# choderalab/openmmtools

Hardware: AMD Instinct MI355X
Metric: REMD iterations/s (propagate+u_kl+mix), 24-replica AlanineDipeptideExplicit per GPU (higher is better)
Workload: dtype f32

## Files before the change

### openmmtools_amd/csrc/forces.hip

```cpp
#include "remd_internal.h"
#include "rng.h"
#include <cmath>
#include <algorithm>
#include <set>
#include <cstdlib>
#include <cstdio>

#define EP_EXT      0
#define EP_BOND     1
#define EP_ANGLE    2
#define EP_TORSION  3
#define EP_EXCEPT   4
#define EP_EXCLCORR 5
#define EP_PME      6
#define EP_CONST    7
#define EP_NB0      8

#include "pair_math.h"
#include "listed_terms.h"

#define MAX_EXCL_WORDS 8

struct nb_tables {
    nb_params p{};
    int method = NB_LJ_ONLY;
    bool has_alch = false;
    dev_array<float4> d_param;
    dev_array<unsigned long long> d_mask;
    int n_exc = 0; dev_array<int> d_exc_atoms; dev_array<float> d_exc_params;
    dev_array<int> d_exc_alch; dev_array<int> d_excl_alch;
    double lam_e_override = -1.0;
    double self_nn = 0, self_aa = 0, q_n = 0, q_a = 0;
    dev_array<double> d_probe; int probe_R = 0;
    int n_excl = 0; dev_array<int> d_excl_atoms; dev_array<float> d_excl_qq;
    dev_array<float> d_rep_lam;
    int rep_lam_R = 0;
    std::vector<double> state_lam_a, state_sc;
    dev_array<double> d_state_lam;
    dev_array<double> d_alch_ukl;
    dev_array<int> d_own;
    int alch_R = 0, alch_K = 0;
    double disp_coeff = 0.0;
    double self_energy = 0.0;
    double net_charge_term = 0.0;
    std::vector<double> charge;
    std::vector<char> is_alch;
    int n_groups = 0; dev_array<int> d_grp_first; dev_array<int> d_grp_size;
    dev_array<int> d_order;
    dev_array<float4> d_spos;
    dev_array<float4> d_sposi;
    dev_array<float4> d_lj_sposi;
    dev_array<float4> d_sparam;
    dev_array<unsigned long long> d_smask;
    dev_array<float4> d_tile_c; dev_array<float4> d_tile_h;
    dev_array<float4> d_partial;
    dev_array<float4> d_cl_c; dev_array<float4> d_cl_h;
    int cl_cap = 0; bool clusters = true;
    bool lj_split = false; int NL = 0, NLpad = 0, lj_words = 1, lj_cap = 0;
    dev_array<int> d_lj_ord;
    dev_array<unsigned long long> d_lj_mask;
    dev_array<int> d_lj_order; dev_array<float4> d_lj_spos; dev_array<float4> d_lj_sparam; dev_array<unsigned long long> d_lj_smask;
    dev_array<float4> d_lj_tile_c; dev_array<float4> d_lj_tile_h; dev_array<float4> d_lj_cl_c; dev_array<float4> d_lj_cl_h;
    int sci_split = 12;
    dev_array<unsigned int> d_sci_list; dev_array<int> d_sci_count; dev_array<unsigned long long> d_excl; int excl_W = 0;
    dev_array<long long> d_sforce; dev_array<long long> d_lj_sforce;
    dev_array<unsigned int> d_lj_sci_list; dev_array<int> d_lj_sci_count; dev_array<unsigned long long> d_lj_excl; int lj_excl_W = 0;
    int sort_R = 0; int evals_since_sort = 1 << 30; int resort_interval = 40; bool sorting = true;
    std::vector<float> rep_lam_host;
    dev_array<unsigned int> d_queue;
    struct tune_seg { int cand; hipEvent_t a, b; };
    int nb_prio = 0;
    std::vector<tune_seg> tune_segs; int tune_state = 0 , tune_left = 0, tune_next = 0;
    int nb_grid = 0;
    int sort_hbits = 0;
    dev_array<float4> d_ctab; bool use_table = false;
    dev_array<unsigned int> d_pair_done; unsigned int pair_done_target = 0;
    dev_array<int> d_tile_of_rank;
    dev_array<int> d_sort_scratch;
    ~nb_tables() { for (auto& sg : tune_segs) { if (sg.a) hipEventDestroy(sg.a); if (sg.b) hipEventDestroy(sg.b); } }
};
void remd_table_deleter::operator()(nb_tables* t) const { delete t; }

__global__ void remd_spin_wait_kernel(const unsigned int* flag, unsigned int seq, unsigned int* spin_out)
{
    if (threadIdx.x == 0) {
        long long n = 0;
        while ((int)(__hip_atomic_load(flag, __ATOMIC_RELAXED, __HIP_MEMORY_SCOPE_AGENT) - seq) < 0) {
            if ((n & 255) == 255 && __hip_atomic_load(spin_out, __ATOMIC_RELAXED, __HIP_MEMORY_SCOPE_AGENT) != 0u) break;
            __builtin_amdgcn_s_sleep(4);
            if (++n > (1ll << 25)) { atomicCAS(spin_out, 0u, 1u); break; }
        }
    }
    __builtin_amdgcn_fence(__ATOMIC_ACQUIRE, "agent");
}
void remd_launch_join_wait(remd_ctx* h)
{
    if (h->fold_pending) {
        hipEventRecord(h->ev_join, h->stream2);
        hipStreamWaitEvent(h->stream, h->ev_join, 0);
        h->fold_pending = false;
    }
    if (!h->join_deferred) return;
    hipLaunchKernelGGL(remd_spin_wait_kernel, dim3(1), dim3(64), 0, h->stream, h->d_sync + 1, h->join_deferred, h->d_sync + 2);
    h->join_deferred = 0;
}
__global__ void remd_signal_kernel(unsigned int* flag, unsigned int seq)
{
    if (threadIdx.x == 0) __hip_atomic_store(flag, seq, __ATOMIC_RELEASE, __HIP_MEMORY_SCOPE_AGENT);
}

__device__ __forceinline__ double wave_sum(double e)
{
    for (int off = 32; off > 0; off >>= 1) e += __shfl_xor(e, off);
    return e;
}

__device__ __forceinline__ double block_sum_256(double e, double* s_part)
{
    e = wave_sum(e);
    if ((threadIdx.x & 63) == 0) s_part[threadIdx.x >> 6] = e;
    __syncthreads();
    return s_part[0] + s_part[1] + s_part[2] + s_part[3];
}

template <bool ENERGY>
__global__ __launch_bounds__(64)
void ext_force_kernel(int n_ext, const int* __restrict__ ext_atoms, float K, float x0, double U0,
                      int Npad, const float4* __restrict__ pos, long long* __restrict__ force,
                      double* __restrict__ epart, int n_epart)
{
    const int r = blockIdx.x;
    double e = 0.0;
    for (int t = threadIdx.x; t < n_ext; t += 64) {
        const int i = ext_atoms[t];
        const float4 p = pos[(size_t)r * Npad + i];
        const float dx = p.x - x0;
        add_force(force + (size_t)r * 3 * Npad, Npad, i, -K * dx, -K * p.y, -K * p.z);
        if (ENERGY) e += 0.5 * (double)K * ((double)dx * dx + (double)p.y * p.y + (double)p.z * p.z) + U0;
    }
    if (ENERGY) {
        e = wave_sum(e);
        if (threadIdx.x == 0) epart[(size_t)r * n_epart + EP_EXT] = e;
    }
}

template <bool ENERGY>
__global__ __launch_bounds__(256)
void bond_kernel(int n, const int* __restrict__ atoms, const float* __restrict__ params, int Npad,
                 const float4* __restrict__ pos, long long* __restrict__ force, double* __restrict__ epart, int n_epart)
{
    __shared__ double s_part[4];
    const int r = blockIdx.x;
    const float4* P = pos + (size_t)r * Npad;
    long long* F = force + (size_t)r * 3 * Npad;
    double e = 0.0;
    for (int t = threadIdx.x; t < n; t += 256) {
        const int i = atoms[2 * t], j = atoms[2 * t + 1];
        const float r0 = params[2 * t], k = params[2 * t + 1];
        const float3 d = sub3(ld3(P, j), ld3(P, i));
        const float len = sqrtf(dotf(d, d));
        const float dl = len - r0;
        const float fs = k * dl / len;
        add_force(F, Npad, i, fs * d.x, fs * d.y, fs * d.z);
        add_force(F, Npad, j, -fs * d.x, -fs * d.y, -fs * d.z);
        if (ENERGY) e += 0.5 * (double)k * (double)dl * (double)dl;
    }
    if (ENERGY) { e = block_sum_256(e, s_part); if (threadIdx.x == 0) epart[(size_t)r * n_epart + EP_BOND] = e; }
}

template <bool ENERGY>
__global__ __launch_bounds__(256)
void angle_kernel(int n, const int* __restrict__ atoms, const float* __restrict__ params, int Npad,
                  const float4* __restrict__ pos, long long* __restrict__ force, double* __restrict__ epart, int n_epart)
{
    __shared__ double s_part[4];
    const int r = blockIdx.x;
    const float4* P = pos + (size_t)r * Npad;
    long long* F = force + (size_t)r * 3 * Npad;
    double e = 0.0;
    for (int t = threadIdx.x; t < n; t += 256) {
        const int a = atoms[3 * t], b = atoms[3 * t + 1], c = atoms[3 * t + 2];
        const float th0 = params[2 * t], k = params[2 * t + 1];
// ... 79 lines not shown
    unsigned k = 0u;
    for (int b = bits - 1; b >= 0; --b) {
#pragma unroll
        for (int i = 0; i < 3; ++i) k = (k << 1) | ((X[i] >> b) & 1u);
    }
    return k;
}

template <typename KEY>
__device__ __forceinline__
void sort_groups_body(int G, int N, int Npad, const int* __restrict__ grp_first, const int* __restrict__ grp_size,
                      const float4* __restrict__ pos, const float* __restrict__ box, int* __restrict__ order,
                      KEY* key, int* r_first, int* r_size, int* r_off, int* s_part, int hbits)
{
    const int r = blockIdx.x, tid = threadIdx.x;
    const float Lx = box[4 * r], Ly = box[4 * r + 1], Lz = box[4 * r + 2];
    const int nc = 1 << hbits;
    constexpr int GBITS = sizeof(KEY) == 8 ? 32 : 13;
    for (int g = tid; g < G; g += 1024) {
        const float4 x = pos[(size_t)r * Npad + grp_first[g]];
        float fx = x.x / Lx, fy = x.y / Ly, fz = x.z / Lz;
        fx -= floorf(fx); fy -= floorf(fy); fz -= floorf(fz);
        const unsigned cx = min(nc - 1, (int)(fx * nc)), cy = min(nc - 1, (int)(fy * nc)), cz = min(nc - 1, (int)(fz * nc));
        key[g] = ((KEY)hilbert3(cx, cy, cz, hbits) << GBITS) | (KEY)(unsigned)g;
    }
    __syncthreads();
    for (int g = tid; g < G; g += 1024) {
        const KEY k = key[g];
        int rank = 0;
        for (int o = 0; o < G; ++o) rank += (key[o] < k) ? 1 : 0;
        r_first[rank] = grp_first[g];
        r_size[rank] = grp_size[g];
    }
    __syncthreads();
    const int per = (G + 1023) / 1024;
    const int b = min(G, tid * per), e = min(G, b + per);
    int sum = 0;
    for (int k = b; k < e; ++k) sum += r_size[k];
    s_part[tid] = sum;
    __syncthreads();
    for (int off = 1; off < 1024; off <<= 1) {
        const int v = (tid >= off) ? s_part[tid - off] : 0;
        __syncthreads();
        s_part[tid] += v;
        __syncthreads();
    }
    int run = (tid > 0) ? s_part[tid - 1] : 0;
    for (int k = b; k < e; ++k) { r_off[k] = run; run += r_size[k]; }
    __syncthreads();
    int* O = order + (size_t)r * Npad;
    for (int k = tid; k < G; k += 1024) {
        const int st = r_off[k], f = r_first[k], n = r_size[k];
        for (int a = 0; a < n; ++a) O[st + a] = f + a;
    }
    for (int k = N + tid; k < Npad; k += 1024) O[k] = -1;
}

__global__ __launch_bounds__(1024)
void sort_groups_kernel(int G, int N, int Npad, const int* __restrict__ grp_first, const int* __restrict__ grp_size,
                        const float4* __restrict__ pos, const float* __restrict__ box, int* __restrict__ order, int hbits)
{
    extern __shared__ __attribute__((aligned(16))) char smem[];
    unsigned* key = reinterpret_cast<unsigned*>(smem);
    int* r_first = reinterpret_cast<int*>(key + G);
    __shared__ int s_part[1024];
    sort_groups_body<unsigned>(G, N, Npad, grp_first, grp_size, pos, box, order, key, r_first, r_first + G, r_first + 2 * G, s_part, hbits);
}

__global__ __launch_bounds__(1024)
void sort_groups_large_kernel(int G, int N, int Npad, const int* __restrict__ grp_first, const int* __restrict__ grp_size,
                              const float4* __restrict__ pos, const float* __restrict__ box, int* __restrict__ order,
                              int* __restrict__ scratch, int hbits)
{
    __shared__ int s_part[1024];
    int* base = scratch + (size_t)blockIdx.x * 5 * G;
    unsigned long long* key = reinterpret_cast<unsigned long long*>(base);
    int* r_first = base + 2 * G;
    sort_groups_body<unsigned long long>(G, N, Npad, grp_first, grp_size, pos, box, order, key, r_first, r_first + G, r_first + 2 * G, s_part, hbits);
}

__global__ __launch_bounds__(256)
void gather_params_kernel(int Npad, int words, const int* __restrict__ order, const float4* __restrict__ param,
                          const unsigned long long* __restrict__ mask, float4* __restrict__ sparam,
                          unsigned long long* __restrict__ smask)
{
    const int k = blockIdx.x * blockDim.x + threadIdx.x, r = blockIdx.y;
    if (k >= Npad) return;
    const int o = order[(size_t)r * Npad + k];
    sparam[(size_t)r * Npad + k] = (o >= 0) ? param[o] : make_float4(0.f, 0.f, 0.f, 0.f);
    for (int w = 0; w < words; ++w)
        smask[((size_t)r * Npad + k) * words + w] = (o >= 0) ? mask[(size_t)o * words + w] : 0ull;
}

__global__ __launch_bounds__(1024)
void compact_lj_kernel(int N, int Npad, int NL, int NLpad, int words, const int* __restrict__ order, const int* __restrict__ lj_ord,
                       const float4* __restrict__ param, const unsigned long long* __restrict__ lj_mask,
                       int* __restrict__ lj_order, float4* __restrict__ lj_sparam, unsigned long long* __restrict__ lj_smask)
{
    __shared__ int s_part[1024];
    const int r = blockIdx.x, tid = threadIdx.x;
    const int* O = order + (size_t)r * Npad;
    const int per = (N + 1023) / 1024;
    const int b = min(N, tid * per), e = min(N, b + per);
    int cnt = 0;
    for (int k = b; k < e; ++k) cnt += (lj_ord[O[k]] >= 0) ? 1 : 0;
    s_part[tid] = cnt;
    __syncthreads();
    for (int off = 1; off < 1024; off <<= 1) {
        const int v = (tid >= off) ? s_part[tid - off] : 0;
        __syncthreads();
        s_part[tid] += v;
        __syncthreads();
    }
    int slot = (tid > 0) ? s_part[tid - 1] : 0;
    for (int k = b; k < e; ++k) {
        const int a = O[k];
        const int ord = lj_ord[a];
        if (ord >= 0) {
            lj_order[(size_t)r * NLpad + slot] = a;
            lj_sparam[(size_t)r * NLpad + slot] = param[a];
            for (int w = 0; w < words; ++w) lj_smask[((size_t)r * NLpad + slot) * words + w] = lj_mask[(size_t)ord * words + w];
            ++slot;
        }
    }
    for (int k = NL + tid; k < NLpad; k += 1024) {
        lj_order[(size_t)r * NLpad + k] = -1;
        lj_sparam[(size_t)r * NLpad + k] = make_float4(0.f, 0.f, 0.f, 0.f);
        for (int w = 0; w < words; ++w) lj_smask[((size_t)r * NLpad + k) * words + w] = 0ull;
    }
}

__device__ __forceinline__
void gather_positions_body(int tile, int nt, int r, int lane, int Npad, int Npad_pos, const int* __restrict__ order,
                           const float4* __restrict__ pos, const float* __restrict__ box, float4* __restrict__ spos,
                           float4* __restrict__ tile_c, float4* __restrict__ tile_h, float4* __restrict__ cl_c,
                           float4* __restrict__ cl_h, const float4* __restrict__ sparam = nullptr, float4* __restrict__ sposi = nullptr)
{
    const int k = tile * 64 + lane;
    const int o = order[(size_t)r * Npad + k];
    float4 x = (o >= 0) ? pos[(size_t)r * Npad_pos + o] : make_float4(0.f, 0.f, 0.f, 0.f);
    if (sparam) x.w = sparam[(size_t)r * Npad + k].x;
    spos[(size_t)r * Npad + k] = x;
    const float Lx = box[4 * r], Ly = box[4 * r + 1], Lz = box[4 * r + 2];
    if (sposi) {
        auto frac = [](float v, float L) { float f = v / L; f -= floorf(f); return (unsigned int)(f * 4294967296.f); };
        const unsigned int fx = frac(x.x, Lx), fy = frac(x.y, Ly), fz = frac(x.z, Lz);
        sposi[(size_t)r * Npad + k] = make_float4(__uint_as_float(fx), __uint_as_float(fy), __uint_as_float(fz), x.w);
    }
    const float x0 = __shfl(x.x, 0), y0 = __shfl(x.y, 0), z0 = __shfl(x.z, 0);
    float dx = x.x - x0, dy = x.y - y0, dz = x.z - z0;
    dx -= Lx * rintf(dx / Lx); dy -= Ly * rintf(dy / Ly); dz -= Lz * rintf(dz / Lz);
    if (o < 0) { dx = dy = dz = 0.f; }
    float lox = dx, hix = dx, loy = dy, hiy = dy, loz = dz, hiz = dz;
    for (int off = 32; off > 0; off >>= 1) {
        lox = fminf(lox, __shfl_xor(lox, off)); hix = fmaxf(hix, __shfl_xor(hix, off));
        loy = fminf(loy, __shfl_xor(loy, off)); hiy = fmaxf(hiy, __shfl_xor(hiy, off));
        loz = fminf(loz, __shfl_xor(loz, off)); hiz = fmaxf(hiz, __shfl_xor(hiz, off));
    }
    if (lane == 0) {
        tile_c[(size_t)r * nt + tile] = make_float4(x0 + 0.5f * (lox + hix), y0 + 0.5f * (loy + hiy), z0 + 0.5f * (loz + hiz), 0.f);
        tile_h[(size_t)r * nt + tile] = make_float4(0.5f * (hix - lox), 0.5f * (hiy - loy), 0.5f * (hiz - loz), 0.f);
    }
    if (cl_c) {
        const int g0 = lane & ~7;
        const float cx0 = __shfl(x.x, g0), cy0 = __shfl(x.y, g0), cz0 = __shfl(x.z, g0);
        const int o0 = __shfl(o, g0);
        float ex = x.x - cx0, ey = x.y - cy0, ez = x.z - cz0;
        ex -= Lx * rintf(ex / Lx); ey -= Ly * rintf(ey / Ly); ez -= Lz * rintf(ez / Lz);
        if (o < 0) { ex = ey = ez = 0.f; }
        float ax = ex, bx2 = ex, ay = ey, by2 = ey, az = ez, bz2 = ez;
        for (int off = 4; off > 0; off >>= 1) {
            ax = fminf(ax, __shfl_xor(ax, off)); bx2 = fmaxf(bx2, __shfl_xor(bx2, off));
            ay = fminf(ay, __shfl_xor(ay, off)); by2 = fmaxf(by2, __shfl_xor(by2, off));
            az = fminf(az, __shfl_xor(az, off)); bz2 = fmaxf(bz2, __shfl_xor(bz2, off));
        }
        if ((lane & 7) == 0) {
            const int ncl = nt * 8;
            const int c = tile * 8 + (lane >> 3);
            cl_c[(size_t)r * ncl + c] = (o0 >= 0) ? make_float4(cx0 + 0.5f * (ax + bx2), cy0 + 0.5f * (ay + by2), cz0 + 0.5f * (az + bz2), 0.f)
                                                  : make_float4(0.f, 0.f, 0.f, 0.f);
            cl_h[(size_t)r * ncl + c] = (o0 >= 0) ? make_float4(0.5f * (bx2 - ax), 0.5f * (by2 - ay), 0.5f * (bz2 - az), 0.f)
                                                  : make_float4(-1e9f, -1e9f, -1e9f, 0.f);
        }
    }
}

__global__ __launch_bounds__(64)
void gather_positions_kernel(int Npad, int Npad_pos, const int* __restrict__ order, const float4* __restrict__ pos,
                             const float* __restrict__ box, float4* __restrict__ spos, float4* __restrict__ tile_c,
                             float4* __restrict__ tile_h, float4* __restrict__ cl_c, float4* __restrict__ cl_h)
{
    gather_positions_body(blockIdx.x, gridDim.x, blockIdx.y, threadIdx.x, Npad, Npad_pos, order, pos, box, spos, tile_c, tile_h, cl_c, cl_h);
}

struct gather_args { int Npad; const int* order; float4* spos; float4* tile_c; float4* tile_h; float4* cl_c; float4* cl_h; const float4* sparam; float4* sposi; };
__global__ __launch_bounds__(64)
void gather_positions2_kernel(int nt_a, gather_args a, gather_args b, int Npad_pos, const float4* __restrict__ pos,
                              const float* __restrict__ box)
{
    const bool second = (int)blockIdx.x >= nt_a;
    const gather_args& g = second ? b : a;
    gather_positions_body(second ? blockIdx.x - nt_a : blockIdx.x, second ? gridDim.x - nt_a : nt_a, blockIdx.y, threadIdx.x, g.Npad, Npad_pos,
                          g.order, pos, box, g.spos, g.tile_c, g.tile_h, g.cl_c, g.cl_h, g.sparam, g.sposi);
}


__device__ __forceinline__
void scatter_sorted_forces_body(int Npad_a, const int* __restrict__ order_a, long long* __restrict__ sforce_a,
                                int Npad_b, const int* __restrict__ order_b, long long* __restrict__ sforce_b,
                                long long* __restrict__ force, int Npad_force, int k, int r)
{
    const bool second = k >= Npad_a;
    if (second) k -= Npad_a;
    const int Npad_s = second ? Npad_b : Npad_a;
    if (k >= Npad_s) return;
    long long* S = (second ? sforce_b : sforce_a) + (size_t)r * 3 * Npad_s;
    const int o = (second ? order_b : order_a)[(size_t)r * Npad_s + k];
    unsigned long long* U = reinterpret_cast<unsigned long long*>(force + (size_t)r * 3 * Npad_force);
#pragma unroll
    for (int c = 0; c < 3; ++c) {
        const long long v = S[(size_t)c * Npad_s + k];
        if (v != 0) { S[(size_t)c * Npad_s + k] = 0; if (o >= 0) atomicAdd(&U[(size_t)c * Npad_force + o], (unsigned long long)v); }
    }
}

__global__ __launch_bounds__(256)
void scatter_sorted_forces_kernel(int Npad_a, const int* __restrict__ order_a, long long* __restrict__ sforce_a,
                                  int Npad_b, const int* __restrict__ order_b, long long* __restrict__ sforce_b,
                                  long long* __restrict__ force, int Npad_force, unsigned int* __restrict__ done = nullptr)
{
    scatter_sorted_forces_body(Npad_a, order_a, sforce_a, Npad_b, order_b, sforce_b, force, Npad_force, blockIdx.x * 256 + threadIdx.x, blockIdx.y);
    if (done) {
        asm volatile("s_waitcnt vmcnt(0)" ::: "memory");
        __syncthreads();
        if (threadIdx.x == 0) __hip_atomic_fetch_add(done + 16 * blockIdx.y, 1u, __ATOMIC_RELAXED, __HIP_MEMORY_SCOPE_AGENT);
    }
}

#define SCI_LANE_II(lane) ((lane) & 7)
#define SCI_LANE_JJ(lane) ((lane) >> 3)
#define SCI_LANE_OF(ii, jj) ((jj) * 8 + (ii))

__global__ __launch_bounds__(64)
void build_excl_kernel(int Npad, int ncl, int W, int words, const unsigned long long* __restrict__ smask,
                       unsigned long long* __restrict__ excl)
{
    const int ic = blockIdx.x, r = blockIdx.y, lane = threadIdx.x;
    const int ii = SCI_LANE_II(lane), jj = SCI_LANE_JJ(lane);
    const int half = 32 * words;
    const int i = ic * 8 + ii;
    for (int dj = 0; dj < W; ++dj) {
        const int j = (ic + dj) * 8 + jj;
        const int d = j - i + half;
        bool ex = (dj == 0 && jj <= ii);
        if (d >= 0 && d < 2 * half) ex = ex || ((smask[((size_t)r * Npad + i) * words + (d >> 6)] >> (d & 63)) & 1ull);
        const unsigned long long m = __ballot(ex);
        if (lane == 0) excl[((size_t)r * ncl + ic) * W + dj] = m;
    }
}

__device__ __forceinline__
void build_sci_list_body(int T, int r, int lane, int ncl, int cap, float rc2, const float4* __restrict__ cl_c,
                         const float4* __restrict__ cl_h, const float4* __restrict__ tile_c, const float4* __restrict__ tile_h,
                         const float* __restrict__ box, unsigned int* __restrict__ list, int* __restrict__ count)
{
    __shared__ int s_tiles[64];
    __shared__ float4 s_ci[8], s_hi[8];
    const int ntile = ncl >> 3;
    const float Lx = box[4 * r], Ly = box[4 * r + 1], Lz = box[4 * r + 2];
    const float iLx = 1.f / Lx, iLy = 1.f / Ly, iLz = 1.f / Lz;
    if (lane < 8) { s_ci[lane] = cl_c[(size_t)r * ncl + T * 8 + lane]; s_hi[lane] = cl_h[(size_t)r * ncl + T * 8 + lane]; }
    const float4 ct = tile_c[(size_t)r * ntile + T], ht = tile_h[(size_t)r * ntile + T];
    auto near = [&](const float4 ci, const float4 hi, const float4 cj, const float4 hj) {
        float bx = cj.x - ci.x, by = cj.y - ci.y, bz = cj.z - ci.z;
        bx -= Lx * rintf(bx * iLx); by -= Ly * rintf(by * iLy); bz -= Lz * rintf(bz * iLz);
        bx = fmaxf(0.f, fabsf(bx) - hi.x - hj.x); by = fmaxf(0.f, fabsf(by) - hi.y - hj.y); bz = fmaxf(0.f, fabsf(bz) - hi.z - hj.z);
        return (hi.x >= 0.f) && (bx * bx + by * by + bz * bz <= rc2);
    };
    unsigned int* L = list + ((size_t)r * ntile + T) * cap;
    int n = 0;
    for (int tbase = T; tbase < ntile; tbase += 64) {
        const int jt = tbase + lane;
        const bool thit = (jt < ntile) && near(ct, ht, tile_c[(size_t)r * ntile + jt], tile_h[(size_t)r * ntile + jt]);
        const unsigned long long tm = __ballot(thit);
        const int nhit = __popcll(tm);
        __syncthreads();
        if (thit) s_tiles[__popcll(tm & ((1ull << lane) - 1ull))] = jt;
        __syncthreads();
        for (int q = 0; q < nhit; q += 8) {
            const int g = q + (lane >> 3);
            unsigned int imask = 0u;
            int jc = 0;
            if (g < nhit) {
                jc = s_tiles[g] * 8 + (lane & 7);
                const float4 cj = cl_c[(size_t)r * ncl + jc], hj = cl_h[(size_t)r * ncl + jc];
#pragma unroll
                for (int s = 0; s < 8; ++s)
                    if (jc >= T * 8 + s && near(s_ci[s], s_hi[s], cj, hj)) imask |= 1u << s;
            }
            const unsigned long long m = __ballot(imask != 0u);
            if (imask != 0u) {
                const int slot = n + __popcll(m & ((1ull << lane) - 1ull));
                if (slot < cap) L[slot] = (unsigned int)jc | (imask << 16);
            }
            n += __popcll(m);
        }
    }
    if (lane == 0) count[(size_t)r * ntile + T] = n;
}

__global__ __launch_bounds__(256)
void rank_tiles_kernel(int ntile, const int* __restrict__ count, int* __restrict__ tile_of_rank)
{
    const int r = blockIdx.y;
    const int* c = count + (size_t)r * ntile;
    for (int t = blockIdx.x * 256 + threadIdx.x; t < ntile; t += gridDim.x * 256) {
        const int mine = c[t];
        int rank = 0;
        for (int q = 0; q < ntile; ++q) { const int o = c[q]; rank += (o > mine || (o == mine && q < t)) ? 1 : 0; }
// ... 187 lines not shown
                fr = keep_where(in, fr);
                const sci_v2f dxy = { dx, dy }, fr2 = { fr, fr };
                fixy[s] = __builtin_elementwise_fma(dxy, fr2, fixy[s]);
                fjxy = __builtin_elementwise_fma(-dxy, fr2, fjxy);
                fiz[s] = fmaf(dz, fr, fiz[s]);
                fjz = fmaf(-dz, fr, fjz);
                if (ENERGY) e += ((in >> lane) & 1ull) ? (double)ee : 0.0;
            }
            fjx = fjxy.x; fjy = fjxy.y;
            if (touched) {
                asm("s_nop 1\n\t"
                    "v_add_f32_dpp %0, %0, %0 quad_perm:[1,0,3,2] row_mask:0xf bank_mask:0xf\n\t"
                    "v_add_f32_dpp %1, %1, %1 quad_perm:[1,0,3,2] row_mask:0xf bank_mask:0xf\n\t"
                    "v_add_f32_dpp %2, %2, %2 quad_perm:[1,0,3,2] row_mask:0xf bank_mask:0xf\n\t"
                    "v_add_f32_dpp %0, %0, %0 quad_perm:[2,3,0,1] row_mask:0xf bank_mask:0xf\n\t"
                    "v_add_f32_dpp %1, %1, %1 quad_perm:[2,3,0,1] row_mask:0xf bank_mask:0xf\n\t"
                    "v_add_f32_dpp %2, %2, %2 quad_perm:[2,3,0,1] row_mask:0xf bank_mask:0xf\n\t"
                    "v_add_f32_dpp %0, %0, %0 row_half_mirror row_mask:0xf bank_mask:0xf\n\t"
                    "v_add_f32_dpp %1, %1, %1 row_half_mirror row_mask:0xf bank_mask:0xf\n\t"
                    "v_add_f32_dpp %2, %2, %2 row_half_mirror row_mask:0xf bank_mask:0xf"
                    : "+v"(fjx), "+v"(fjy), "+v"(fjz));
            }
            const int eb = k & 7;
            if (ii == eb) { qfx = fjx; qfy = fjy; qfz = fjz; qj = j; }
            if (eb == 7 || k + 1 == cnt) {
                if (ii <= eb) add_force(force + (size_t)r * 3 * Npad_force, Npad_force, qj, qfx, qfy, qfz);
            }
        }
    }
    auto reduce_scatter = [&](float (&v)[8]) {
        float a[4], b[2];
#pragma unroll
        for (int q = 0; q < 4; ++q) {
            const float send = (jj & 4) ? v[q] : v[q + 4], keep = (jj & 4) ? v[q + 4] : v[q];
            a[q] = keep + __shfl_xor(send, 32);
        }
#pragma unroll
        for (int q = 0; q < 2; ++q) {
            const float send = (jj & 2) ? a[q] : a[q + 2], keep = (jj & 2) ? a[q + 2] : a[q];
            b[q] = keep + __shfl_xor(send, 16);
        }
        const float send = (jj & 1) ? b[0] : b[1], keep = (jj & 1) ? b[1] : b[0];
        return keep + __shfl_xor(send, 8);
    };
    float fix[8], fiy[8];
#pragma unroll
    for (int s = 0; s < 8; ++s) { fix[s] = fixy[s].x; fiy[s] = fixy[s].y; }
    float fx = reduce_scatter(fix), fy = reduce_scatter(fiy), fz = reduce_scatter(fiz);
    if (NW > 1) {
        __shared__ float s_f[NW][3][64];
        s_f[wv][0][lane] = fx; s_f[wv][1][lane] = fy; s_f[wv][2][lane] = fz;
        __syncthreads();
        if (wv == 0) {
            fx = s_f[0][0][lane]; fy = s_f[0][1][lane]; fz = s_f[0][2][lane];
#pragma unroll
            for (int w = 1; w < NW; ++w) { fx += s_f[w][0][lane]; fy += s_f[w][1][lane]; fz += s_f[w][2][lane]; }
        }
    }
    if (wv == 0) add_force(force + (size_t)r * 3 * Npad_force, Npad_force, (T * 8 + jj) * 8 + ii, fx, fy, fz);
    if (ENERGY) {
        e = wave_sum(e);
        if (lane == 0) epart[(size_t)r * n_epart + EP_NB0 + ep_off + T * nsplit + zsl] = e;
    }
}

#define SCI_RELAXED(M) (M == NB_RF || M == NB_EWALD || (M == NB_LJ_ONLY && ALCH))
extern __shared__ __attribute__((aligned(16))) float4 s_ctab[];
__device__ __forceinline__ void stage_coulomb_table(const nb_params& p, const float4* __restrict__ ctab_g, int nthreads)
{
    for (int k = threadIdx.x; k < p.ctab_n; k += nthreads) s_ctab[k] = ctab_g[k];
    __syncthreads();
}

template <int METHOD, bool ENERGY, bool ALCH, int NW, bool TABLE>
__global__ __launch_bounds__(64 * NW) __attribute__((amdgpu_waves_per_eu(SCI_RELAXED(METHOD) ? 2 : 4, SCI_RELAXED(METHOD) ? 3 : 4)))
void nonbonded_sci_kernel(nb_params p, sci_args a, const float* __restrict__ box, const float* __restrict__ rep_lam,
                          double* __restrict__ epart, int n_epart, int R, const float4* __restrict__ ctab_g)
{
    constexpr bool TAB = TABLE && !ENERGY && SCI_EWALD(METHOD);
    if (TAB) stage_coulomb_table(p, ctab_g, 64 * NW);
    nonbonded_sci_body<METHOD, ENERGY, ALCH, NW, TAB>(p, a, blockIdx.x, box, rep_lam, epart, n_epart, R, s_ctab - p.ctab_key0);
}

template <int METHOD_A, int METHOD_B, bool ENERGY, bool ALCH, int NW, bool TABLE>
__global__ __launch_bounds__(64 * NW)
__attribute__((amdgpu_waves_per_eu((SCI_RELAXED(METHOD_A) || SCI_RELAXED(METHOD_B)) ? 2 : 4, (SCI_RELAXED(METHOD_A) || SCI_RELAXED(METHOD_B)) ? 3 : 4)))
void nonbonded_sci2_kernel(nb_params p, sci_args a, sci_args b, int n_items_a, int n_items, unsigned int* queue, const float* __restrict__ box,
                           const float* __restrict__ rep_lam, double* __restrict__ epart, int n_epart, int R, const float4* __restrict__ ctab_g)
{
    constexpr bool TAB = TABLE && !ENERGY && SCI_EWALD(METHOD_A);
    if (p.prio) __builtin_amdgcn_s_setprio(3);
    if (!queue) {
        if ((int)blockIdx.x < n_items_a) {
            if (TAB) stage_coulomb_table(p, ctab_g, 64 * NW);
            nonbonded_sci_body<METHOD_A, ENERGY, ALCH, NW, TAB>(p, a, blockIdx.x, box, rep_lam, epart, n_epart, R, s_ctab - p.ctab_key0);
        }
        else nonbonded_sci_body<METHOD_B, ENERGY, ALCH, NW, false, true>(p, b, blockIdx.x - n_items_a, box, rep_lam, epart, n_epart, R);
        return;
    }
    if (TAB) stage_coulomb_table(p, ctab_g, 64 * NW);
    __shared__ int s_item;
    for (;;) {
        if (threadIdx.x == 0) s_item = (int)atomicAdd(&queue[0], 1u);
        __syncthreads();
        const int item = s_item;
        if (item >= n_items_a) break;
        nonbonded_sci_body<METHOD_A, ENERGY, ALCH, NW, TAB>(p, a, item, box, rep_lam, epart, n_epart, R, s_ctab - p.ctab_key0);
        __syncthreads();
    }
    __syncthreads();
    for (;;) {
        if (threadIdx.x == 0) s_item = (int)atomicAdd(&queue[1], 1u);
        __syncthreads();
        const int item = s_item;
        if (item >= n_items - n_items_a) break;
        nonbonded_sci_body<METHOD_B, ENERGY, ALCH, NW, false, true>(p, b, item, box, rep_lam, epart, n_epart, R);
        __syncthreads();
    }
    if (threadIdx.x == 0 && atomicAdd(&queue[2], 1u) == gridDim.x - 1) { queue[0] = 0u; queue[1] = 0u; queue[2] = 0u; }
}

#define NB_CHUNK 128
#define NB_WAVES 4
template <int METHOD, bool ENERGY, bool ALCH>
__global__ __launch_bounds__(64 * NB_WAVES)
void nonbonded_kernel(nb_params p, int N, int Npad, const float4* __restrict__ pos,
                      const float4* __restrict__ param_all, const unsigned long long* __restrict__ mask_all,
                      const int* __restrict__ order, const float4* __restrict__ tile_c, const float4* __restrict__ tile_h,
                      const float* __restrict__ box, const float* __restrict__ rep_lam,
                      float4* __restrict__ partial, double* __restrict__ epart, int n_epart, int ntile)
{
    __shared__ float4 s_pos[NB_CHUNK];
    __shared__ float4 s_prm[NB_CHUNK];
    const int tid = threadIdx.x;
    const int lane = tid & 63, wave = tid >> 6;
    const int itile = blockIdx.x * NB_WAVES + wave;
    const int i0 = itile * 64;
    const int i = i0 + lane;
    const int js = blockIdx.y;
    const int r = blockIdx.z;
    const float4* __restrict__ P = pos + (size_t)r * Npad;
    const float4* __restrict__ param = order ? param_all + (size_t)r * Npad : param_all;
    const unsigned long long* __restrict__ mask = order ? mask_all + (size_t)r * Npad * p.excl_words : mask_all;
    const float Lx = box[4 * r], Ly = box[4 * r + 1], Lz = box[4 * r + 2];
    const float iLx = 1.f / Lx, iLy = 1.f / Ly, iLz = 1.f / Lz;
    float lam_a = 1.f, sc = 0.f, lam_e = 1.f;
    if (ALCH) { lam_a = rep_lam[4 * r]; sc = rep_lam[4 * r + 1]; lam_e = rep_lam[4 * r + 2]; }
    const bool active = (itile < ntile) && (i < N);
    const float4 xi = P[active ? i : 0];
    float4 pi = param[active ? i : 0];
    if (ALCH && pi.w != 0.f) pi.x *= lam_e;
    unsigned long long mk[MAX_EXCL_WORDS];
#pragma unroll
    for (int w = 0; w < MAX_EXCL_WORDS; ++w) mk[w] = (w < p.excl_words) ? mask[(size_t)(active ? i : 0) * p.excl_words + w] : 0ull;
    const int half = 32 * p.excl_words;

    const int tps = (ntile + p.n_jsplit - 1) / p.n_jsplit;
    const int t0 = js * tps, t1 = min(ntile, t0 + tps);
    const int jbeg = t0 * 64, jend = min(t1 * 64, N);
    float4 ci = make_float4(0.f, 0.f, 0.f, 0.f), hi = ci;
    const bool cull = order != nullptr && itile < ntile;
    if (cull) { ci = tile_c[(size_t)r * ntile + itile]; hi = tile_h[(size_t)r * ntile + itile]; }
    float fx = 0.f, fy = 0.f, fz = 0.f;
    double e = 0.0;
    const float rcut2 = SCI_EWALD(METHOD) ? p.rcc2 : p.rc2;
    for (int cb = jbeg; cb < jend; cb += NB_CHUNK) {
        __syncthreads();
        {
            const int jj = min(cb + (tid & (NB_CHUNK - 1)), jend - 1);
            if (tid < NB_CHUNK) s_pos[tid] = P[jj]; else s_prm[tid - NB_CHUNK] = param[jj];
        }
        __syncthreads();
        const int cn = min(NB_CHUNK, jend - cb);
        for (int tb = 0; tb < cn; tb += 64) {
            const int jb = cb + tb;
            const int tn = min(64, cn - tb);
            const bool near = (jb + 63 >= i0 - half) && (jb <= i0 + 63 + half);
            if (cull) {
                const int jt = jb >> 6;
                const float4 cj = tile_c[(size_t)r * ntile + jt], hj = tile_h[(size_t)r * ntile + jt];
                float bx = cj.x - ci.x, by = cj.y - ci.y, bz = cj.z - ci.z;
                bx -= Lx * rintf(bx * iLx); by -= Ly * rintf(by * iLy); bz -= Lz * rintf(bz * iLz);
                bx = fmaxf(0.f, fabsf(bx) - hi.x - hj.x); by = fmaxf(0.f, fabsf(by) - hi.y - hj.y); bz = fmaxf(0.f, fabsf(bz) - hi.z - hj.z);
                if (bx * bx + by * by + bz * bz > rcut2) continue;
            }
#pragma unroll 4
            for (int u = 0; u < tn; ++u) {
                const int j = jb + u;
                const float4 xj = s_pos[tb + u];
                float4 pj = s_prm[tb + u];
                float dx = xj.x - xi.x, dy = xj.y - xi.y, dz = xj.z - xi.z;
                dx -= Lx * rintf(dx * iLx); dy -= Ly * rintf(dy * iLy); dz -= Lz * rintf(dz * iLz);
                const float r2 = dx * dx + dy * dy + dz * dz;
                bool in = active && (r2 < rcut2);
                if (near) {
                    const int d = j - i + half;
                    if (d >= 0 && d < 2 * half) in = in && !((mk[d >> 6] >> (d & 63)) & 1ull);
                }
                if (in) {
// ... 426 lines not shown
        for (int i = 0; i < N; ++i) if (d->epsilon[i] != 0.0) ord[i] = NL++;
        t.lj_split = any_charge && NL > 0 && NL * 10 <= N * 6;
        if (t.lj_split) {
            t.NL = NL; t.NLpad = (NL + 63) / 64 * 64;
            int maxd_lj = 0;
            for (int e = 0; e < d->n_exceptions; ++e) {
                const int a = ord[d->exception_atoms[2 * e]], b2 = ord[d->exception_atoms[2 * e + 1]];
                if (a >= 0 && b2 >= 0) maxd_lj = std::max(maxd_lj, std::abs(a - b2));
            }
            t.lj_words = std::max(1, (maxd_lj + 32) / 32);
            if (t.lj_words > MAX_EXCL_WORDS) t.lj_split = false;
        }
        if (t.lj_split) {
            std::vector<unsigned long long> lm((size_t)t.NLpad * t.lj_words, 0ull);
            auto setb = [&](int a, int b2) { const int dd = b2 - a + 32 * t.lj_words; lm[(size_t)a * t.lj_words + (dd >> 6)] |= 1ull << (dd & 63); };
            for (int a = 0; a < t.NL; ++a) setb(a, a);
            for (int e = 0; e < d->n_exceptions; ++e) {
                const int a = ord[d->exception_atoms[2 * e]], b2 = ord[d->exception_atoms[2 * e + 1]];
                if (a >= 0 && b2 >= 0) { setb(a, b2); setb(b2, a); }
            }
            if ((rc = t.d_lj_ord.upload(h, ord)) || (rc = t.d_lj_mask.upload(h, lm))) return rc;
        }
    }

    t.disp_coeff = 0.0;
    if (d->use_dispersion_correction) {
        std::vector<double> sg(d->sigma, d->sigma + N), ep(d->epsilon, d->epsilon + N);
        for (int i = 0; i < N; ++i) if (t.is_alch[i]) ep[i] = 0.0;
        t.disp_coeff = dispersion_coefficient(N, sg, ep, d->cutoff, p.rs >= 0 ? d->switch_distance : -1.0);
    }
    t.self_energy = 0.0; t.net_charge_term = 0.0; t.self_nn = t.self_aa = t.q_n = t.q_a = 0.0;
    if (t.method == NB_EWALD) {
        double q2n = 0, q2a = 0;
        for (int i = 0; i < N; ++i) {
            if (t.is_alch[i]) { q2a += d->charge[i] * d->charge[i]; t.q_a += d->charge[i]; }
            else { q2n += d->charge[i] * d->charge[i]; t.q_n += d->charge[i]; }
        }
        const double pref = -REMD_ONE_4PI_EPS0 * d->ewald_alpha / sqrt(M_PI);
        t.self_nn = pref * q2n; t.self_aa = pref * q2a;
        t.self_energy = t.self_nn + t.self_aa;
        t.net_charge_term = -REMD_ONE_4PI_EPS0 * M_PI / (2.0 * d->ewald_alpha * d->ewald_alpha);
    }
    return 0;
}

static int update_replica_lambdas(remd_ctx* h, nb_tables& t)
{
    if (!t.has_alch) return 0;
    if (t.rep_lam_R != h->R) { t.d_rep_lam.reset(); REMD_TRY(t.d_rep_lam.alloc(h, 4 * h->R)); t.rep_lam_R = h->R; t.rep_lam_host.clear(); }
    std::vector<float> rl(4 * (size_t)h->R, 0.f);
    for (int r = 0; r < h->R; ++r) {
        const int64_t k = h->labels.empty() ? 0 : h->labels[h->r_begin + r];
        const double ls = h->lam_s.empty() ? 1.0 : h->lam_s[k];
        const double le = t.lam_e_override >= 0.0 ? t.lam_e_override : (h->lam_e.empty() ? 1.0 : h->lam_e[k]);
        rl[4 * r] = (float)pow(ls, h->sc_a);
        rl[4 * r + 1] = (float)(h->sc_alpha * pow(1.0 - ls, h->sc_b));
        rl[4 * r + 2] = (float)le;
    }
    if (rl == t.rep_lam_host) return 0;
    REMD_CHECK(h, hipMemcpyAsync(t.d_rep_lam, rl.data(), sizeof(float) * rl.size(), hipMemcpyHostToDevice, h->stream));
    REMD_CHECK(h, hipStreamSynchronize(h->stream));
    t.rep_lam_host = rl;
    return 0;
}

static void launch_list_build(remd_ctx* h, nb_tables& t, bool lj)
{
    const int ncl = lj ? t.NLpad / 8 : ((h->N + 63) / 64) * 8;
    hipLaunchKernelGGL(build_sci_list_kernel, dim3(ncl / 8, h->R), dim3(64), 0, h->stream, ncl, lj ? t.lj_cap : t.cl_cap,
                       (!lj && t.method == NB_EWALD) ? t.p.rcc2 : t.p.rc2,
                       lj ? t.d_lj_cl_c : t.d_cl_c, lj ? t.d_lj_cl_h : t.d_cl_h, lj ? t.d_lj_tile_c : t.d_tile_c, lj ? t.d_lj_tile_h : t.d_tile_h,
                       h->d_box, lj ? t.d_lj_sci_list : t.d_sci_list, lj ? t.d_lj_sci_count : t.d_sci_count);
}

static int ensure_sorted(remd_ctx* h, nb_tables& t)
{
    if (!t.sorting || t.n_groups <= 0) return 0;
    const int ntile = (h->N + 63) / 64;
    const bool cl = t.clusters && ntile * 8 < 65536;
    if (t.sort_R != h->R) {
        t.d_order.reset(); t.d_spos.reset(); t.d_sparam.reset(); t.d_smask.reset(); t.d_tile_c.reset(); t.d_tile_h.reset();
        const size_t n = (size_t)h->R * h->Npad;
        REMD_TRY(t.d_order.alloc(h, n));
        REMD_TRY(t.d_spos.alloc(h, n));
        t.d_sposi.reset();
        REMD_TRY(t.d_sposi.alloc(h, n));
        REMD_TRY(t.d_sparam.alloc(h, n));
        REMD_TRY(t.d_smask.alloc(h, n * t.p.excl_words));
        REMD_TRY(t.d_tile_c.alloc(h, (size_t)h->R * ntile));
        REMD_TRY(t.d_tile_h.alloc(h, (size_t)h->R * ntile));
        t.d_pair_done.reset();
        REMD_TRY(t.d_pair_done.alloc(h, 16 * h->R));
        REMD_CHECK(h, hipMemsetAsync(t.d_pair_done, 0, sizeof(unsigned int) * 16 * h->R, h->stream));
        t.pair_done_target = 0;
        t.d_cl_c.reset(); t.d_cl_h.reset();
        t.d_sci_list.reset(); t.d_sci_count.reset(); t.d_excl.reset(); t.d_sforce.reset(); t.d_lj_sforce.reset();
        t.d_lj_sci_list.reset(); t.d_lj_sci_count.reset(); t.d_lj_excl.reset();
        const int ncl = ntile * 8;
        t.cl_cap = std::min(ncl, 4096);
        if (cl) {
            REMD_TRY(t.d_cl_c.alloc(h, (size_t)h->R * ncl));
            REMD_TRY(t.d_cl_h.alloc(h, (size_t)h->R * ncl));
            t.excl_W = 4 * t.p.excl_words + 1;
            REMD_TRY(t.d_sci_list.alloc(h, (size_t)h->R * ntile * t.cl_cap));
            REMD_TRY(t.d_sci_count.alloc(h, (size_t)h->R * ntile));
            t.d_tile_of_rank.reset();
            REMD_TRY(t.d_tile_of_rank.alloc(h, (size_t)h->R * ntile));
            REMD_TRY(t.d_excl.alloc(h, (size_t)h->R * ncl * t.excl_W));
            REMD_TRY(t.d_sforce.alloc(h, n * 3));
            REMD_CHECK(h, hipMemsetAsync(t.d_sforce, 0, sizeof(long long) * n * 3, h->stream));
            if (!t.d_queue) {
                REMD_TRY(t.d_queue.alloc(h, 4));
                REMD_CHECK(h, hipMemsetAsync(t.d_queue, 0, 4 * sizeof(unsigned int), h->stream));
            }
        }
        if (cl && t.lj_split) {
            t.d_lj_order.reset(); t.d_lj_spos.reset(); t.d_lj_sparam.reset(); t.d_lj_smask.reset(); t.d_lj_tile_c.reset(); t.d_lj_tile_h.reset();
            t.d_lj_cl_c.reset(); t.d_lj_cl_h.reset();
            const size_t nl = (size_t)h->R * t.NLpad;
            const int ncl_lj = t.NLpad / 8;
            t.lj_cap = std::min(ncl_lj, 4096);
            REMD_TRY(t.d_lj_order.alloc(h, nl));
            REMD_TRY(t.d_lj_spos.alloc(h, nl));
            t.d_lj_sposi.reset();
            REMD_TRY(t.d_lj_sposi.alloc(h, nl));
            REMD_TRY(t.d_lj_sparam.alloc(h, nl));
            REMD_TRY(t.d_lj_smask.alloc(h, nl * t.lj_words));
            REMD_TRY(t.d_lj_tile_c.alloc(h, (size_t)h->R * (t.NLpad / 64)));
            REMD_TRY(t.d_lj_tile_h.alloc(h, (size_t)h->R * (t.NLpad / 64)));
            REMD_TRY(t.d_lj_cl_c.alloc(h, (size_t)h->R * ncl_lj));
            REMD_TRY(t.d_lj_cl_h.alloc(h, (size_t)h->R * ncl_lj));
            t.lj_excl_W = 4 * t.lj_words + 1;
            REMD_TRY(t.d_lj_sci_list.alloc(h, (size_t)h->R * (ncl_lj / 8) * t.lj_cap));
            REMD_TRY(t.d_lj_sci_count.alloc(h, (size_t)h->R * (ncl_lj / 8)));
            REMD_TRY(t.d_lj_excl.alloc(h, (size_t)h->R * ncl_lj * t.lj_excl_W));
            REMD_TRY(t.d_lj_sforce.alloc(h, nl * 3));
            REMD_CHECK(h, hipMemsetAsync(t.d_lj_sforce, 0, sizeof(long long) * nl * 3, h->stream));
        }
        t.sort_R = h->R; t.evals_since_sort = 1 << 30;
    }
    const bool split = cl && t.lj_split;
    if (t.evals_since_sort >= t.resort_interval) {
        remd_prof_scope ps(h, "nb_sort");
        if (t.sort_hbits == 0) {
            double lmax = 0.0;
            for (int k = 0; k < 3 && (size_t)k < h->box_host.size(); ++k) lmax = std::max(lmax, h->box_host[k]);
            t.sort_hbits = lmax > 0.0 ? std::max(1, std::min(6, (int)lround(log2(lmax / 0.11)))) : 4;
        }
        if (t.n_groups < 8192) {
            const size_t lds = sizeof(int) * 4 * (size_t)t.n_groups;
            hipLaunchKernelGGL(sort_groups_kernel, dim3(h->R), dim3(1024), lds, h->stream, t.n_groups, h->N, h->Npad, t.d_grp_first,
                               t.d_grp_size, h->d_pos, h->d_box, t.d_order, t.sort_hbits);
        } else {
            const size_t need = (size_t)h->R * 5 * t.n_groups;
            REMD_TRY(t.d_sort_scratch.grow(h, need));
            hipLaunchKernelGGL(sort_groups_large_kernel, dim3(h->R), dim3(1024), 0, h->stream, t.n_groups, h->N, h->Npad, t.d_grp_first,
                               t.d_grp_size, h->d_pos, h->d_box, t.d_order, t.d_sort_scratch, t.sort_hbits);
        }
        hipLaunchKernelGGL(gather_params_kernel, dim3((h->Npad + 255) / 256, h->R), dim3(256), 0, h->stream, h->Npad, t.p.excl_words,
                           t.d_order, t.d_param, t.d_mask, t.d_sparam, t.d_smask);
        if (split)
            hipLaunchKernelGGL(compact_lj_kernel, dim3(h->R), dim3(1024), 0, h->stream, h->N, h->Npad, t.NL, t.NLpad, t.lj_words, t.d_order,
                               t.d_lj_ord, t.d_param, t.d_lj_mask, t.d_lj_order, t.d_lj_sparam, t.d_lj_smask);
        if (cl) {
            hipLaunchKernelGGL(build_excl_kernel, dim3(ntile * 8, h->R), dim3(64), 0, h->stream, h->Npad, ntile * 8, t.excl_W, t.p.excl_words,
                               t.d_smask, t.d_excl);
            if (split)
                hipLaunchKernelGGL(build_excl_kernel, dim3(t.NLpad / 8, h->R), dim3(64), 0, h->stream, t.NLpad, t.NLpad / 8, t.lj_excl_W,
                                   t.lj_words, t.d_lj_smask, t.d_lj_excl);
        }
        t.evals_since_sort = 0;
    }
    t.evals_since_sort++;
    remd_prof_scope ps(h, "nb_gather");
    if (split) {
        const int ntile_lj = t.NLpad / 64;
        gather_args ga{h->Npad, t.d_order, t.d_spos, t.d_tile_c, t.d_tile_h, t.d_cl_c, t.d_cl_h, t.d_sparam, t.d_sposi};
        gather_args gb{t.NLpad, t.d_lj_order, t.d_lj_spos, t.d_lj_tile_c, t.d_lj_tile_h, t.d_lj_cl_c, t.d_lj_cl_h, nullptr, t.d_lj_sposi};
        sci_list_args la{ntile * 8, t.cl_cap, t.d_cl_c, t.d_cl_h, t.d_tile_c, t.d_tile_h, t.d_sci_list, t.d_sci_count};
        sci_list_args lb{t.NLpad / 8, t.lj_cap, t.d_lj_cl_c, t.d_lj_cl_h, t.d_lj_tile_c, t.d_lj_tile_h, t.d_lj_sci_list, t.d_lj_sci_count};
        const float rc2_main = t.method == NB_EWALD ? t.p.rcc2 : t.p.rc2;
        hipLaunchKernelGGL(gather_positions2_kernel, dim3(ntile + ntile_lj, h->R), dim3(64), 0, h->stream, ntile, ga, gb, h->Npad, h->d_pos, h->d_box);
        hipLaunchKernelGGL(build_sci_list2_kernel, dim3(ntile + ntile_lj, h->R), dim3(64), 0, h->stream, ntile, la, lb, rc2_main, t.p.rc2, h->d_box);
        if (t.evals_since_sort == 1 && t.d_tile_of_rank && ntile <= 2048)
            hipLaunchKernelGGL(rank_tiles_kernel, dim3((ntile + 255) / 256, h->R), dim3(256), 0, h->stream, ntile, t.d_sci_count, t.d_tile_of_rank);
    } else {
        hipLaunchKernelGGL(gather_positions_kernel, dim3(ntile, h->R), dim3(64), 0, h->stream, h->Npad, h->Npad, t.d_order, h->d_pos, h->d_box,
                           t.d_spos, t.d_tile_c, t.d_tile_h, cl ? t.d_cl_c : (float4*)nullptr, cl ? t.d_cl_h : (float4*)nullptr);
        if (cl) launch_list_build(h, t, false);
    }
    const bool debug = h->sw.debug;
    if (cl && t.evals_since_sort == 1 && (t.cl_cap < ntile * 8 || debug)) {
        std::vector<int> cnt((size_t)h->R * ntile);
        REMD_CHECK(h, hipMemcpyAsync(cnt.data(), t.d_sci_count, sizeof(int) * cnt.size(), hipMemcpyDeviceToHost, h->stream));
        REMD_CHECK(h, hipStreamSynchronize(h->stream));
        int mx = 0; for (int c : cnt) mx = std::max(mx, c);
        if (debug) {
            std::vector<unsigned int> ll((size_t)ntile * t.cl_cap);
            hipMemcpy(ll.data(), t.d_sci_list, sizeof(unsigned int) * ll.size(), hipMemcpyDeviceToHost);
            double ne = 0, nb = 0;
            for (int T = 0; T < ntile; ++T) for (int k = 0; k < std::min(cnt[T], t.cl_cap); ++k) { ne += 1; nb += __builtin_popcount(ll[(size_t)T * t.cl_cap + k] >> 16); }
            fprintf(stderr, "[remd] sci list (replica 0): %d tiles, %.1f entries per tile (max %d, cap %d), %.2f i clusters per entry\n",
                    ntile, ne / ntile, mx, t.cl_cap, nb / std::max(1.0, ne));
        }
        if (mx > t.cl_cap) t.clusters = false;
    }
    return 0;
}

template <int METHOD, bool ENERGY>
static int launch_nb(remd_ctx* h, nb_tables& t)
{
    const int ntile = (h->N + 63) / 64;
    if (t.sorting && t.clusters && t.d_order && t.d_sci_list && t.n_groups > 0 && ntile * 8 < 65536) {
        const int ncl = ntile * 8;
        const float* rl = t.has_alch ? t.d_rep_lam : (const float*)nullptr;
        const bool split = t.lj_split && t.d_lj_sci_list && (METHOD == NB_EWALD || METHOD == NB_RF);
        constexpr int MAIN = (METHOD == NB_EWALD) ? NB_EWALD_NOLJ : (METHOD == NB_RF) ? NB_RF_NOLJ : METHOD;
        const int ssplit = std::max(SCI_NW, std::min(16, t.sci_split / SCI_NW * SCI_NW));
        const bool ranked = (ntile >= 64 || h->parent != nullptr) && ntile <= 2048 && t.lj_split && t.d_lj_sci_list && t.d_tile_of_rank && (METHOD == NB_EWALD || METHOD == NB_RF);
        sci_args sa{h->N, h->Npad, ncl, t.cl_cap, t.excl_W, h->Npad, 0, ssplit, t.d_spos, t.d_sparam, t.d_excl, t.d_sci_list, t.d_sci_count, t.d_sforce,
                    t.d_sposi, ranked ? t.d_tile_of_rank : (const int*)nullptr};
        const int items_a = ntile * h->R * (ssplit / SCI_NW);
        if (split) {
            sci_args sb{t.NL, t.NLpad, t.NLpad / 8, t.lj_cap, t.lj_excl_W, t.NLpad, ncl * 4, ssplit, t.d_lj_spos, t.d_lj_sparam, t.d_lj_excl,
                        t.d_lj_sci_list, t.d_lj_sci_count, t.d_lj_sforce, t.d_lj_sposi, nullptr};
            const int items = items_a + (t.NLpad / 64) * h->R * (ssplit / SCI_NW);
            const int persist_grid = h->sw.nb_persist_grid >= 0 ? h->sw.nb_persist_grid : t.nb_grid;
            const int grid = (h->pme_concurrent && persist_grid > 0) ? std::min(items, persist_grid) : items;
            const bool fold = h->fold_pending && !ENERGY && t.d_pair_done;
            if (h->fold_pending && !fold) h->fold_pending = false;
            const bool tab = t.use_table && !ENERGY && SCI_EWALD(MAIN);
            const size_t tab_lds = tab ? sizeof(float4) * (size_t)t.p.ctab_n : 0;
#define LAUNCH_SCI2(ALCHF, TABF) hipLaunchKernelGGL((nonbonded_sci2_kernel<MAIN, NB_LJ_ONLY, ENERGY, ALCHF, SCI_NW, TABF>), dim3(grid), dim3(64 * SCI_NW), \
            tab_lds, h->stream, t.p, sa, sb, items_a, items, grid < items ? t.d_queue : (unsigned int*)nullptr, h->d_box, rl, h->d_epart, h->n_epart, h->R, \
            (const float4*)t.d_ctab)
            if (t.has_alch) { if (tab) LAUNCH_SCI2(true, true); else LAUNCH_SCI2(true, false); }
            else { if (tab) LAUNCH_SCI2(false, true); else LAUNCH_SCI2(false, false); }
#undef LAUNCH_SCI2
            const dim3 sgrid((h->Npad + t.NLpad + 255) / 256, h->R);
            if (fold) {
                t.pair_done_target += sgrid.x;
                h->fold.done = t.d_pair_done; h->fold.target = t.pair_done_target;
            }
            hipLaunchKernelGGL(scatter_sorted_forces_kernel, sgrid, dim3(256), 0, h->stream, h->Npad,
                               t.d_order, t.d_sforce, t.NLpad, t.d_lj_order, t.d_lj_sforce, h->d_force, h->Npad, fold ? t.d_pair_done : (unsigned int*)nullptr);
            return 0;
        }
        const bool tab1 = t.use_table && !ENERGY && SCI_EWALD(METHOD);
        const size_t tab1_lds = tab1 ? sizeof(float4) * (size_t)t.p.ctab_n : 0;
#define LAUNCH_SCI(ALCHF, TABF) hipLaunchKernelGGL((nonbonded_sci_kernel<METHOD, ENERGY, ALCHF, SCI_NW, TABF>), dim3(items_a), dim3(64 * SCI_NW), tab1_lds, \
            h->stream, t.p, sa, h->d_box, rl, h->d_epart, h->n_epart, h->R, (const float4*)t.d_ctab)
        if (t.has_alch) { if (tab1) LAUNCH_SCI(true, true); else LAUNCH_SCI(true, false); }
        else { if (tab1) LAUNCH_SCI(false, true); else LAUNCH_SCI(false, false); }
#undef LAUNCH_SCI
        hipLaunchKernelGGL(scatter_sorted_forces_kernel, dim3((h->Npad + 255) / 256, h->R), dim3(256), 0, h->stream, h->Npad, t.d_order,
                           t.d_sforce, 0, (const int*)nullptr, (long long*)nullptr, h->d_force, h->Npad);
        return 0;
    }
    dim3 grid((ntile + NB_WAVES - 1) / NB_WAVES, t.p.n_jsplit, h->R);
    const size_t need = (size_t)h->R * t.p.n_jsplit * h->Npad;
    REMD_TRY(t.d_partial.grow(h, need));
    const bool sorted = t.sorting && t.d_order && t.n_groups > 0;
    const float4* P = sorted ? t.d_spos : h->d_pos;
    const float4* prm = sorted ? t.d_sparam : t.d_param;
    const unsigned long long* mk = sorted ? t.d_smask : t.d_mask;
    const int* ord = sorted ? t.d_order : nullptr;
    if (t.has_alch)
        hipLaunchKernelGGL((nonbonded_kernel<METHOD, ENERGY, true>), grid, dim3(64 * NB_WAVES), 0, h->stream, t.p, h->N, h->Npad, P,
                           prm, mk, ord, t.d_tile_c, t.d_tile_h, h->d_box, t.d_rep_lam, t.d_partial, h->d_epart, h->n_epart, ntile);
    else
        hipLaunchKernelGGL((nonbonded_kernel<METHOD, ENERGY, false>), grid, dim3(64 * NB_WAVES), 0, h->stream, t.p, h->N, h->Npad, P,
                           prm, mk, ord, t.d_tile_c, t.d_tile_h, h->d_box, (const float*)nullptr, t.d_partial, h->d_epart, h->n_epart, ntile);
    hipLaunchKernelGGL(nb_reduce_kernel, dim3((h->N + 255) / 256, h->R), dim3(256), 0, h->stream, h->N, h->Npad, t.p.n_jsplit,
                       t.d_partial, h->d_force);
    return 0;
}

void remd_nb_reset_accumulators(remd_ctx* h)
{
    nb_tables* t = h->nb.get();
    h->fold_pending = false;
    if (!t || h->R <= 0) return;
    if (t->d_sforce) hipMemsetAsync(t->d_sforce, 0, sizeof(long long) * 3 * (size_t)h->R * h->Npad, h->stream);
    if (t->d_lj_sforce) hipMemsetAsync(t->d_lj_sforce, 0, sizeof(long long) * 3 * (size_t)h->R * t->NLpad, h->stream);
}

int remd_nb_molecules(remd_ctx* h, const int** first, const int** size)
{
    nb_tables* it = h->nb.get();
    if (!it || it->n_groups <= 0) return 0;
    *first = it->d_grp_first; *size = it->d_grp_size;
    return it->n_groups;
}

const float* remd_nb_rep_lam(remd_ctx* h)
{
    if (h->regions_exact) {
        const float4* prm; const float* le;
        if (remd_regions_pme_tables(h, &prm, &le)) return le;
    }
    nb_tables* it = h->nb.get();
    return (it && it->has_alch) ? it->d_rep_lam : nullptr;
}
const float4* remd_nb_param(remd_ctx* h)
{
    if (h->regions_exact) {
        const float4* prm; const float* le;
        if (remd_regions_pme_tables(h, &prm, &le)) return prm;
    }
    return remd_table_of(h->nb).d_param;
}

int remd_nb_required_epart(remd_ctx* h)
{
    const int ntile = (h->Npad + 63) / 64;
    return EP_NB0 + ntile * 8 * 4 + 8 + ntile * 8 * 4 + 2;
}

#define TUNE_SEG 40
#define TUNE_NC 6
struct tune_cand { int grid, prio_pair; };
static const tune_cand g_tune_cands[TUNE_NC] = {{0, 1}, {0, 0}, {768, 0}, {640, 0}, {576, 0}, {512, 0}};
void remd_nb_tune_step(remd_ctx* h, int steps_left_in_call)
{
    nb_tables* tp = h->nb.get();
    if (!tp || h->nb_method == REMD_NB_NONE) return;
    nb_tables& t = *tp;
    if (h->sw.nb_persist_grid >= 0 || t.tune_state != 0 || !h->pme_concurrent || h->profiling == 2) return;
    if (t.tune_left == 0) {
        hipEvent_t boundary = nullptr;
        if (!t.tune_segs.empty() && !t.tune_segs.back().b) {
            hipEventCreate(&boundary); hipEventRecord(boundary, h->stream);
            t.tune_segs.back().b = boundary;
        }
        if (t.tune_next == 2 * TUNE_NC) { t.tune_state = 1; t.nb_grid = 0; return; }
        if (steps_left_in_call < TUNE_SEG) { t.nb_grid = 0; return; }
        nb_tables::tune_seg sg{t.tune_next % TUNE_NC, nullptr, nullptr};
        hipEventCreate(&sg.a); hipEventRecord(sg.a, h->stream);
        t.tune_segs.push_back(sg);
        t.nb_grid = g_tune_cands[sg.cand].grid; t.nb_prio = g_tune_cands[sg.cand].prio_pair;
        t.tune_next++;
        t.tune_left = TUNE_SEG;
    }
    t.tune_left--;
}
void remd_nb_tune_resolve(remd_ctx* h)
{
    nb_tables* tp = h->nb.get();
    if (!tp || tp->tune_state != 1) return;
    nb_tables& t = *tp;
    double ms[TUNE_NC] = {0};
    bool ok = true;
    for (auto& sg : t.tune_segs) {
        float e = 0.f;
        if (!sg.a || !sg.b || hipEventElapsedTime(&e, sg.a, sg.b) != hipSuccess) { ok = false; (void)hipGetLastError(); }
        ms[sg.cand] += e;
        if (sg.a) hipEventDestroy(sg.a);
        if (sg.b) hipEventDestroy(sg.b);
    }
    t.tune_segs.clear();
    int best = 0;
    for (int c = 1; c < TUNE_NC; ++c) if (ok && ms[c] < ms[best] * 0.995) best = c;
    t.nb_grid = ok ? g_tune_cands[best].grid : 0; t.nb_prio = ok ? g_tune_cands[best].prio_pair : 0;
    t.tune_state = 2;
    if (h->sw.nb_tune_verbose)
    {
        fprintf(stderr, "[remd] pair-kernel residency, ms per %d steps:", 2 * TUNE_SEG);
        for (int c = 0; c < TUNE_NC; ++c) fprintf(stderr, " %d%s: %.2f", g_tune_cands[c].grid, g_tune_cands[c].prio_pair ? "p" : "", ms[c]);
        fprintf(stderr, " -> %d workgroups\n", t.nb_grid);
    }
}
void remd_nb_invalidate_sort(remd_ctx* h)
{
    nb_tables* t = h->nb.get();
    if (t) t->evals_since_sort = 1 << 30;
}
int remd_nb_resident_info(remd_ctx* h, int* ok, int* method, int* has_alch, nb_params* p, const float4** param, const float** rep_lam)
{
    *ok = 0; *method = -1; *has_alch = 0; *param = nullptr; *rep_lam = nullptr;
    if (h->nb_method == REMD_NB_NONE) { *ok = h->nocutoff ? 0 : 1; return 0; }
    if (h->n_regions > 0) return 0;
    nb_tables* t = h->nb.get();
    if (!t || t->method != NB_LJ_ONLY || t->n_exc != 0 || t->n_excl != 0 || h->n_exceptions != 0) return 0;
    int rc = update_replica_lambdas(h, *t);
    if (rc) return rc;
    *ok = 1; *method = t->method; *has_alch = t->has_alch ? 1 : 0; *p = t->p; *param = t->d_param;
    *rep_lam = t->has_alch ? t->d_rep_lam : nullptr;
    return 0;
}

int remd_compute_forces(remd_ctx* h, bool with_energy, unsigned class_mask)
{
    if (with_energy && (class_mask & 63u) != 63u) return remd_fail(h, -1, "energies need every force class");
    const bool do_ext = (class_mask >> REMD_FG_EXTERNAL) & 1u, do_bond = (class_mask >> REMD_FG_BOND) & 1u;
    const bool do_angle = (class_mask >> REMD_FG_ANGLE) & 1u, do_torsion = (class_mask >> REMD_FG_TORSION) & 1u;
    const bool do_nb = (class_mask >> REMD_FG_NONBONDED) & 1u, do_recip = (class_mask >> REMD_FG_RECIPROCAL) & 1u;
    const bool do_rst = h->n_restraints > 0 && ((class_mask >> REMD_FG_RESTRAINT) & 1u);
    if (!h->force_zeroed)
        REMD_CHECK(h, hipMemsetAsync(h->d_force, 0, sizeof(long long) * 3 * (size_t)h->Npad * h->R, h->stream));
    h->force_zeroed = false;
    if (with_energy)
        REMD_CHECK(h, hipMemsetAsync(h->d_epart, 0, sizeof(double) * (size_t)h->n_epart * h->R, h->stream));
    const int R = h->R;
#define LAUNCH_E(kern, ...) do { if (with_energy) hipLaunchKernelGGL(kern<true>, __VA_ARGS__); else hipLaunchKernelGGL(kern<false>, __VA_ARGS__); } while (0)
    if (h->n_regions > 0 && do_nb) { int rcr = remd_regions_forces(h, with_energy, h->n_epart - 2); if (rcr) return rcr; }
    if (h->nocutoff && do_nb) { int rcn = remd_nocutoff_forces(h, with_energy, EP_NB0); if (rcn) return rcn; }
    if (h->gbsa && do_nb) { int rcg = remd_gbsa_forces(h, with_energy, EP_NB0 + 1); if (rcg) return rcg; }
    if (h->n_ext > 0 && do_ext) {
        remd_prof_scope ps(h, "ext_force");
        LAUNCH_E(ext_force_kernel, dim3(R), dim3(64), 0, h->stream, h->n_ext, h->d_ext_atoms, (float)h->ext_K, (float)h->ext_x0,
                 h->ext_U0, h->Npad, h->d_pos, h->d_force, h->d_epart, h->n_epart);
    }
    bool forked = false, swapped = false;
    struct unswap { remd_ctx* h; bool* on; ~unswap() { if (*on) std::swap(h->stream, h->stream2); } } guard{h, &swapped};
    auto listed_terms = [&](int& total) {
        listed_tables T{};
        T.n_bonds = do_bond ? h->n_bonds : 0; T.n_angles = do_angle ? h->n_angles : 0; T.n_torsions = do_torsion ? h->n_torsions : 0;
        T.bond_atoms = h->d_bond_atoms; T.bond_params = h->d_bond_params;
        T.angle_atoms = h->d_angle_atoms; T.angle_params = h->d_angle_params;
        T.torsion_atoms = h->d_torsion_atoms; T.torsion_params = h->d_torsion_params;
        nb_tables* it = h->nb.get();
        if (it && h->nb_method != REMD_NB_NONE && do_nb) {
            nb_tables& t = *it;
            T.n_exc = t.n_exc; T.exc_atoms = t.d_exc_atoms; T.exc_params = t.d_exc_params;
            T.n_excl = t.n_excl; T.excl_atoms = t.d_excl_atoms; T.excl_qq = t.d_excl_qq;
            T.alpha = t.p.alpha; T.two_alpha_sqrtpi = t.p.two_alpha_sqrtpi;
            T.exc_alch = t.d_exc_alch; T.excl_alch = t.d_excl_alch; T.rep_lam = t.has_alch ? t.d_rep_lam : nullptr;
        }
        total = T.n_bonds + T.n_angles + T.n_torsions + T.n_exc + T.n_excl;
        T.n_aterm = 0; T.aterm = nullptr;
        if (h->sw.listed_atoms && total > 0 && h->d_aterm && h->n_aterm > 0) { T.aterm = h->d_aterm; T.n_aterm = h->n_aterm; total = h->n_aterm; }
        return T;
    };
    bool listed_rode = false;
    if (h->nb_method != REMD_NB_NONE) {
        nb_tables& t0 = remd_table_of(h->nb);
        int rc0 = update_replica_lambdas(h, t0);
        if (rc0) return rc0;
        if (t0.method == NB_EWALD && h->sw.overlap && h->stream2 && do_nb && do_recip) {
            t0.p.prio = h->sw.nb_prio >= 0 ? h->sw.nb_prio : t0.nb_prio;
            h->mesh_prio_hi = !t0.p.prio;
            if (!h->sync_events) {
                h->fork_seq_pending = ++h->sync_seq;
                hipLaunchKernelGGL(remd_spin_wait_kernel, dim3(1), dim3(64), 0, h->stream2, h->d_sync, h->sync_seq, h->d_sync + 2);
            } else {
                hipEventRecord(h->ev_fork, h->stream);
                hipStreamWaitEvent(h->stream2, h->ev_fork, 0);
            }
            h->mesh_listed_total = 0;
            if (h->sw.listed_main && h->sw.listed_ride && !with_energy && !h->sync_events && t0.p.prio != 0) {
                int total = 0;
                h->mesh_listed = listed_terms(total);
                h->mesh_listed_total = total;
                listed_rode = total > 0;
            }
            rc0 = remd_pme_forces(h, with_energy, h->stream, 1);
            if (rc0) return rc0;
            std::swap(h->stream, h->stream2);
            swapped = true; forked = true;
        }
    }
    h->pme_concurrent = forked;
    if (!forked) { h->mesh_prio_hi = true; if (h->nb_method != REMD_NB_NONE) remd_table_of(h->nb).p.prio = 0; }
    const bool merged = !with_energy;
    if (!merged && h->n_bonds > 0) {
        remd_prof_scope ps(h, "bonded");
        LAUNCH_E(bond_kernel, dim3(R), dim3(256), 0, h->stream, h->n_bonds, h->d_bond_atoms, h->d_bond_params, h->Npad,
                 h->d_pos, h->d_force, h->d_epart, h->n_epart);
    }
    if (!merged && h->n_angles > 0) {
        remd_prof_scope ps(h, "bonded");
        LAUNCH_E(angle_kernel, dim3(R), dim3(256), 0, h->stream, h->n_angles, h->d_angle_atoms, h->d_angle_params, h->Npad,
                 h->d_pos, h->d_force, h->d_epart, h->n_epart);
    }
    if (!merged && h->n_torsions > 0) {
        remd_prof_scope ps(h, "bonded");
        LAUNCH_E(torsion_kernel, dim3(R), dim3(256), 0, h->stream, h->n_torsions, h->d_torsion_atoms, h->d_torsion_params, h->Npad,
                 h->d_pos, h->d_force, h->d_epart, h->n_epart);
    }
    if (!merged && do_rst) { int rcr = remd_restraints_forces(h, with_energy, h->n_epart - 1, h->stream); if (rcr) return rcr; }
    const bool listed_main = h->sw.listed_main && forked && !with_energy && !h->sync_events && h->nb_method != REMD_NB_NONE && remd_table_of(h->nb).p.prio != 0;
    int rc_rst = 0;
    auto launch_listed = [&](hipStream_t lst) {
        if (do_rst && !rc_rst) rc_rst = remd_restraints_forces(h, with_energy, h->n_epart - 1, lst);
        if (listed_rode) return;
        int total = 0;
        const listed_tables T = listed_terms(total);
        if (total > 0) {
            remd_prof_scope ps(h, "bonded");
            hipLaunchKernelGGL(listed_forces_kernel, dim3((total + 255) / 256, R), dim3(256), 0, lst, T, h->Npad, h->d_pos,
                               h->d_box, h->d_force);
        }
    };
    if (h->nb_method == REMD_NB_NONE) {
        if (merged) launch_listed(h->stream);
    } else {
        nb_tables& t = remd_table_of(h->nb);
        int rc = do_nb ? ensure_sorted(h, t) : 0;
        if (rc) return rc;
        if (merged && listed_main) launch_listed(h->stream2);
        h->fold_pending = h->sw.nb_fold && listed_main && merged && h->defer_join_ok && do_nb && (class_mask & 63u) == 63u && t.sorting && t.clusters &&
                          t.lj_split && t.d_lj_sci_list && t.d_sci_list && h->profiling != 2;
        h->fold.done = nullptr;
        if (do_nb) {
            remd_prof_scope ps(h, "nonbonded");
            if (with_energy) {
                if (t.method == NB_LJ_ONLY) rc = launch_nb<NB_LJ_ONLY, true>(h, t);
                else if (t.method == NB_RF) rc = launch_nb<NB_RF, true>(h, t);
                else rc = launch_nb<NB_EWALD, true>(h, t);
            } else {
                if (t.method == NB_LJ_ONLY) rc = launch_nb<NB_LJ_ONLY, false>(h, t);
                else if (t.method == NB_RF) rc = launch_nb<NB_RF, false>(h, t);
                else rc = launch_nb<NB_EWALD, false>(h, t);
            }
            if (rc) return rc;
        }
        h->fold_pending = h->fold_pending && h->fold.done != nullptr;
        if (merged && !listed_main) launch_listed(h->stream);
        if (!merged && t.n_exc > 0) {
            remd_prof_scope ps(h, "exceptions");
            LAUNCH_E(exception_kernel, dim3(R), dim3(256), 0, h->stream, t.n_exc, t.d_exc_atoms, t.d_exc_params, t.d_exc_alch,
                     t.has_alch ? t.d_rep_lam : (const float*)nullptr, h->Npad,
                     h->d_pos, h->d_box, h->d_force, h->d_epart, h->n_epart);
        }
        if (!merged && t.n_excl > 0) {
            remd_prof_scope ps(h, "exceptions");
            LAUNCH_E(ewald_exclusion_kernel, dim3(R), dim3(256), 0, h->stream, t.n_excl, t.d_excl_atoms, t.d_excl_qq, t.d_excl_alch,
                     t.has_alch ? t.d_rep_lam : (const float*)nullptr, t.p.alpha,
                     t.p.two_alpha_sqrtpi, h->Npad, h->d_pos, h->d_box, h->d_force, h->d_epart, h->n_epart);
        }
        if (t.method == NB_EWALD) {
            if (forked) {
                if (h->fold_pending) {
                    std::swap(h->stream, h->stream2); swapped = false;
                } else if (!h->sync_events) {
                    hipLaunchKernelGGL(remd_signal_kernel, dim3(1), dim3(64), 0, h->stream, h->d_sync + 1, h->sync_seq);
                    std::swap(h->stream, h->stream2); swapped = false;
                    if (h->defer_join_ok && !with_energy) h->join_deferred = h->sync_seq;
                    else hipLaunchKernelGGL(remd_spin_wait_kernel, dim3(1), dim3(64), 0, h->stream, h->d_sync + 1, h->sync_seq, h->d_sync + 2);
                } else {
                    hipEventRecord(h->ev_join, h->stream);
                    std::swap(h->stream, h->stream2); swapped = false;
                    hipStreamWaitEvent(h->stream, h->ev_join, 0);
                }
                rc = remd_pme_forces(h, with_energy, h->stream, 2); if (rc) return rc;
            }
            else if (do_recip) { rc = remd_pme_forces(h, with_energy, h->stream); if (rc) return rc; }
        }
        if (with_energy)
            hipLaunchKernelGGL(const_energy_kernel, dim3((R + 63) / 64), dim3(64), 0, h->stream, R, t.disp_coeff, t.self_nn, t.self_aa,
                               t.q_n, t.q_a, t.net_charge_term, t.has_alch ? t.d_rep_lam : (const float*)nullptr, h->d_box,
                               h->d_epart, h->n_epart);
    }
#undef LAUNCH_E
    if (rc_rst) return rc_rst;
    if (with_energy)
        hipLaunchKernelGGL(reduce_energy_kernel, dim3(R), dim3(64), 0, h->stream, h->n_epart, h->d_epart, h->d_potential);
    REMD_CHECK(h, hipGetLastError());
    h->forces_valid = true;
    return 0;
}

__global__ void assemble_ukl_poly_kernel(int R, int K, const double* __restrict__ probe ,
                                         const double* __restrict__ beta, const double* __restrict__ econst,
                                         const double* __restrict__ lam_e, const double* __restrict__ alch, const int* __restrict__ own,
                                         const double* __restrict__ pressure , const float* __restrict__ box,
                                         double econst_vref, double* __restrict__ ukl_rows, double* __restrict__ potential)
{
    const int t = blockIdx.x * blockDim.x + threadIdx.x;
    if (t >= R * K) return;
    const int r = t / K, l = t % K;
    const double P0 = probe[r], Ph = probe[R + r], P1 = probe[2 * R + r];
    const double c = 2.0 * (P1 - P0) - 4.0 * (Ph - P0);
    const double b = (P1 - P0) - c;
    const double le = lam_e[l];
    const double V = (double)box[4 * r] * (double)box[4 * r + 1] * (double)box[4 * r + 2];
    if (l == own[r]) potential[r] = P0 + b * le + c * le * le;
    double U = P0 + b * le + c * le * le + econst[l] * ((econst_vref > 0.0 && V > 0.0) ? econst_vref / V : 1.0);
    if (alch) U += alch[t] - alch[(size_t)r * K + own[r]];
    if (pressure) U += pressure[l] * V;
    ukl_rows[t] = beta[l] * U;
}

__global__ void assemble_ukl_quad_kernel(int R, int K, int n, const double* __restrict__ probe ,
                                         const double* __restrict__ beta, const double* __restrict__ econst,
                                         const float* __restrict__ state_le , const double* __restrict__ alch, const int* __restrict__ own,
                                         const double* __restrict__ pressure , const float* __restrict__ box,
                                         double econst_vref, double* __restrict__ ukl_rows, double* __restrict__ potential)
{
    const int t = blockIdx.x * blockDim.x + threadIdx.x;
    if (t >= R * K) return;
    const int r = t / K, l = t % K;
    const double c0 = probe[r];
    double lin[4], a[4], b[4], le[4];
    for (int x = 0; x < n; ++x) {
        const double Ph = probe[(size_t)(1 + 2 * x) * R + r] - c0, P1 = probe[(size_t)(2 + 2 * x) * R + r] - c0;
        a[x] = 2.0 * P1 - 4.0 * Ph; b[x] = P1 - a[x]; lin[x] = P1;
        le[x] = (double)state_le[4 * l + x];
    }
    double U = c0;
    for (int x = 0; x < n; ++x) U += b[x] * le[x] + a[x] * le[x] * le[x];
    int p = 1 + 2 * n;
    for (int x = 0; x < n; ++x) for (int y = x + 1; y < n; ++y, ++p)
        U += (probe[(size_t)p * R + r] - c0 - lin[x] - lin[y]) * le[x] * le[y];
    const double V = (double)box[4 * r] * (double)box[4 * r + 1] * (double)box[4 * r + 2];
    if (l == own[r]) potential[r] = U;
    U += econst[l] * ((econst_vref > 0.0 && V > 0.0) ? econst_vref / V : 1.0);
    if (alch) U += alch[t] - alch[(size_t)r * K + own[r]];
    if (pressure) U += pressure[l] * V;
    ukl_rows[t] = beta[l] * U;
}

static int assemble_ukl_rows(remd_ctx* h, double* d_rows)
{
    const int n = h->R * h->K;
    const double* alch = nullptr;
    nb_tables* it = h->nb.get();
    bool poly = false;
    const int* d_own_states = nullptr;
    if (h->n_regions > 0 && (h->nb_method != REMD_NB_NONE || h->nocutoff)) {
        nb_tables& t = remd_table_of(h->nb);
        it = &t;
        if (t.alch_R != h->R || t.alch_K != h->K) {
            t.d_alch_ukl.reset(); t.d_state_lam.reset(); t.d_own.reset();
            REMD_TRY(t.d_alch_ukl.alloc(h, (size_t)n));
            t.alch_R = h->R; t.alch_K = h->K;
// ... 89 lines not shown
```

### openmmtools_amd/csrc/integrate.hip

```cpp
#include "remd_internal.h"
#include "rng.h"
#include <set>
#include "pair_math.h"
#include "listed_terms.h"
#include "nocutoff_pair.h"

#define UNIT_FREE   0
#define UNIT_SETTLE 1
#define UNIT_SHAKE  2
#define MAX_TOK 24
#define CHAIN_BIN_COLS 256

struct chain_prog {
    int n;
    char tok[MAX_TOK];
    int o_index[MAX_TOK];
    long long step[MAX_TOK];
    float hV, hR;
    float hVg[4];
    const long long* Fg[4];
    float a, b;
    int nO;
    int accumulate_momentum;
    int cmm_w, cmm_r;
// ... 243 lines not shown
        } else if (tok == 'V' || (tok >= '0' && tok <= '3')) {
            const long long* Ft = tok == 'V' ? F : prog.Fg[tok - '0'] + (size_t)r * 3 * Npad;
            const float hv = tok == 'V' ? prog.hV : prog.hVg[tok - '0'];
#pragma unroll
            for (int k = 0; k < NAT; ++k) {
                const float s = hv * im[k] * (1.0f / 4294967296.0f);
                v[k].x += s * (float)Ft[idx[k]];
                v[k].y += s * (float)Ft[Npad + idx[k]];
                v[k].z += s * (float)Ft[2 * Npad + idx[k]];
            }
#ifdef CHAIN_STAMPS
            if (S.stamps && t == 0) { asm volatile("s_waitcnt vmcnt(0) lgkmcnt(0)" ::: "memory"); const unsigned long long now = wall_clock64(); atomicAdd(&S.stamps[1 + 22], now - S.t_last); S.t_last = now; }
#endif
            constrain_v<TYPE, NAT>(sc, im, tol, v, x);
        } else if (tok == 'R') {
            if (TYPE == UNIT_FREE) {
#pragma unroll
                for (int k = 0; k < NAT; ++k) x[k] = x[k] + v[k] * prog.hR;
            } else {
                float3 p0[NAT], p1[NAT], q[NAT];
#pragma unroll
                for (int k = 0; k < NAT; ++k) {
                    p0[k] = x[k] - x[0];
                    p1[k] = p0[k] + v[k] * prog.hR;
                    q[k] = p1[k];
                }
                if (TYPE == UNIT_SETTLE) settle_positions(sc, p0, p1);
                else S.shake_it = max(S.shake_it, shake_positions<NAT>(im, dist, tol, p0, p1));
                const float ih = frcp(prog.hR);
                const float3 org = x[0];
#pragma unroll
                for (int k = 0; k < NAT; ++k) {
                    v[k] = v[k] + (p1[k] - q[k]) * ih;
                    x[k] = org + p1[k];
                }
                constrain_v<TYPE, NAT>(sc, im, tol, v, x);
            }
        } else if (tok == 'O') {
            const uint64_t cnt = (uint64_t)prog.step[t] * (uint64_t)prog.nO + (uint64_t)prog.o_index[t];
#pragma unroll
            for (int k = 0; k < NAT; ++k) {
                const float3 xi = gaussian3(seed, REMD_STREAM_OU, (uint32_t)idx[k], rg, cnt);
                const float sig = prog.b * fsqrt(kT * im[k]);
                v[k].x = prog.a * v[k].x + sig * xi.x;
                v[k].y = prog.a * v[k].y + sig * xi.y;
                v[k].z = prog.a * v[k].z + sig * xi.z;
            }
            constrain_v<TYPE, NAT>(sc, im, tol, v, x);
        } else if (tok == 'C') {
            float sx, sy, sz;
            if (S.have_cm) { sx = S.cmx; sy = S.cmy; sz = S.cmz; }
            else {
                sx = (float)__hip_atomic_load(&cmm_r[0], __ATOMIC_RELAXED, __HIP_MEMORY_SCOPE_AGENT) * (1.0f / 4294967296.0f) * inv_total_mass;
                sy = (float)__hip_atomic_load(&cmm_r[1], __ATOMIC_RELAXED, __HIP_MEMORY_SCOPE_AGENT) * (1.0f / 4294967296.0f) * inv_total_mass;
                sz = (float)__hip_atomic_load(&cmm_r[2], __ATOMIC_RELAXED, __HIP_MEMORY_SCOPE_AGENT) * (1.0f / 4294967296.0f) * inv_total_mass;
            }
#pragma unroll
            for (int k = 0; k < NAT; ++k) { v[k].x -= sx; v[k].y -= sy; v[k].z -= sz; }
        }
#ifdef CHAIN_STAMPS
        if (S.stamps) { const unsigned long long now = wall_clock64(); atomicAdd(&S.stamps[1 + min(t, 33)], now - S.t_last); S.t_last = now; }
#endif
        if ((prog.measure & 1) && tok == 'O') S.heat += unit_ke() - ke0;
        if ((prog.measure & 2) && (is_v || tok == 'R')) S.shadow += unit_ke() - ke0;
    }
    float3 mom = f3(0, 0, 0);
    if (!last) return mom;
#pragma unroll
    for (int k = 0; k < NAT; ++k) {
        P[idx[k]] = make_float4(x[k].x, x[k].y, x[k].z, 0.f);
        V[idx[k]] = make_float4(v[k].x, v[k].y, v[k].z, 0.f);
        mom = mom + v[k] * frcp(im[k]);
        if (prog.zero_force) { Fw[idx[k]] = 0; Fw[Npad + idx[k]] = 0; Fw[2 * Npad + idx[k]] = 0; }
        if (bins.count) {
            float u; int kx;
            remd_pme_scaled1(x[k].x, bins.box[4 * r], bins.nx, u, kx);
            if (kx >= bins.nx) kx -= bins.nx;
            const int slot = atomicAdd(&bins.count[(size_t)r * bins.nx + kx], 1);
            if (slot < bins.cap) {
                const size_t e = ((size_t)r * bins.nx + kx) * bins.cap + slot;
                bins.atoms[e] = make_float4(x[k].x, x[k].y, x[k].z, __int_as_float(idx[k]));
                if (bins.q) bins.q[e] = bins.param[idx[k]].x;
            } else atomicCAS(bins.err, 0u, 2u);
        }
#ifdef CHAIN_STAMPS
        if (S.stamps) { asm volatile("s_waitcnt vmcnt(0) lgkmcnt(0)" ::: "memory"); const unsigned long long now = wall_clock64(); atomicAdd(&S.stamps[1 + 24 + k], now - S.t_last); S.t_last = now; }
#endif
    }
#ifdef CHAIN_STAMPS
    if (S.stamps) { const unsigned long long now = wall_clock64(); atomicAdd(&S.stamps[35], now - S.t_last); S.t_last = now; }
#endif
    return mom;
}

__device__ __forceinline__ void integrate_chain_body(chain_prog prog, int n_units, const int4* __restrict__ unit_atoms,
                            const unsigned char* __restrict__ unit_type, const float* __restrict__ shake_dist,
                            settle_const sc, float tol,
                            int Npad, float4* __restrict__ pos, float4* __restrict__ vel,
                            long long* force, const float* __restrict__ invmass,
                            const int64_t* __restrict__ labels, const double* __restrict__ beta,
                            int r_begin, uint64_t seed, long long* __restrict__ cmm, float inv_total_mass,
                            unsigned int* join_flag, unsigned int join_seq, remd_chain_bins bins,
                            unsigned long long* chain_slots, unsigned int* chain_sync_err,
                            unsigned long long* own_time, long long* __restrict__ work, float4* __restrict__ xold, float4* __restrict__ vold,
                            remd_fold_args fold, const unsigned int* __restrict__ noise_id)
{
    const int uidx = blockIdx.x * blockDim.x + threadIdx.x;
    const int r = blockIdx.y;
    int4 a4 = make_int4(-1, -1, -1, -1);
    int type = UNIT_FREE;
    float dist[3] = { 0.f, 0.f, 0.f };
    float kT = 0.f;
    uint32_t rg = 0u;
    unit_regs S;
    S.have_cm = 0; S.shake_it = 0;
    {
        if (uidx < n_units) {
            a4 = unit_atoms[uidx]; type = (int)unit_type[uidx];
            dist[0] = shake_dist[uidx * 3]; dist[1] = shake_dist[uidx * 3 + 1]; dist[2] = shake_dist[uidx * 3 + 2];
        }
        kT = frcp((float)beta[labels[r_begin + r]]);
        rg = noise_id ? noise_id[r] : (uint32_t)(r_begin + r);
        const int e_idx[4] = { a4.x, a4.y, a4.z, a4.w };
        const float4* Pe = pos + (size_t)r * Npad;
        const float4* Ve = vel + (size_t)r * Npad;
#pragma unroll
        for (int k = 0; k < 4; ++k) {
            if (e_idx[k] >= 0) {
                const float4 p = Pe[e_idx[k]], w = Ve[e_idx[k]];
                S.x[k] = f3(p.x, p.y, p.z); S.v[k] = f3(w.x, w.y, w.z); S.im[k] = invmass[e_idx[k]];
            }
        }
    }
    if (fold.done) {
        if (threadIdx.x == 0) {
            const unsigned int* word = fold.done + 16 * blockIdx.y;
            long long n = 0;
            while ((int)(__hip_atomic_load(word, __ATOMIC_RELAXED, __HIP_MEMORY_SCOPE_AGENT) - fold.target) < 0) {
                if ((n & 255) == 255 && __hip_atomic_load(chain_sync_err, __ATOMIC_RELAXED, __HIP_MEMORY_SCOPE_AGENT) != 0u) break;
                __builtin_amdgcn_s_sleep(2);
                if (++n > (1ll << 25)) { atomicCAS(chain_sync_err, 0u, 1u); break; }
            }
        }
        __syncthreads();
        __builtin_amdgcn_fence(__ATOMIC_ACQUIRE, "agent");
    }
    if (join_flag) {
        if (threadIdx.x == 0) {
            long long n = 0;
            while ((int)(__hip_atomic_load(join_flag, __ATOMIC_RELAXED, __HIP_MEMORY_SCOPE_AGENT) - join_seq) < 0) {
                if ((n & 255) == 255 && __hip_atomic_load(join_flag + 1, __ATOMIC_RELAXED, __HIP_MEMORY_SCOPE_AGENT) != 0u) break;
                __builtin_amdgcn_s_sleep(2);
                if (++n > (1ll << 25)) { atomicCAS(join_flag + 1, 0u, 1u); break; }
            }
        }
        __syncthreads();
        __builtin_amdgcn_fence(__ATOMIC_ACQUIRE, "agent");
    }
    const unsigned long long own_t0 = own_time ? wall_clock64() : 0ull;
    float3 mom = f3(0, 0, 0);
    const int cmm_r_eff = prog.cmm_r, cmm_w_eff = prog.cmm_w;
    if (uidx == 0 && cmm_r_eff >= 0) {
        long long* o = cmm + ((size_t)(1 - cmm_r_eff) * gridDim.y + r) * 4;
        o[0] = 0; o[1] = 0; o[2] = 0;
    }
    const bool active = a4.x >= 0;
    if (!active) type = UNIT_FREE;
    const int idx[4] = { a4.x, a4.y, a4.z, a4.w };
    float4* P = pos + (size_t)r * Npad;
    float4* V = vel + (size_t)r * Npad;
    const long long* F = force + (size_t)r * 3 * Npad;
    long long* Fw = force + (size_t)r * 3 * Npad;
    const long long* cr = cmm + ((size_t)max(cmm_r_eff, 0) * gridDim.y + r) * 4;
#ifdef CHAIN_STAMPS
    S.stamps = (own_time && blockIdx.x == 0 && blockIdx.y == 0 && threadIdx.x == 0) ? own_time + 2 : nullptr;
    S.t_last = own_t0;
#endif
    const bool wg_bins = bins.count != nullptr && bins.nx <= CHAIN_BIN_COLS;
    remd_chain_bins unit_bins = bins;
    if (wg_bins) unit_bins.count = nullptr;
#ifdef CHAIN_STAMPS
    if (S.stamps) { asm volatile("s_waitcnt vmcnt(0) lgkmcnt(0)" ::: "memory"); const unsigned long long now = wall_clock64(); atomicAdd(&S.stamps[1 + 20], now - S.t_last); S.t_last = now; }
#endif
    for (int t0 = 0;;) {
        int t1 = t0;
        while (t1 < prog.n && chain_tok(prog, t1) != 'M') ++t1;
        const bool first = t0 == 0, last = t1 == prog.n;
        if (active) {
#define RUN(TY, NA) mom = run_unit<TY, NA>(prog, idx, dist, sc, tol, Npad, P, V, F, Fw, invmass, kT, rg, seed, cr, inv_total_mass, unit_bins, r, S, t0, t1, first, last, xold ? xold + (size_t)r * Npad : nullptr, vold ? vold + (size_t)r * Npad : nullptr)
            if (type == UNIT_SETTLE) RUN(UNIT_SETTLE, 3);
            else if (type == UNIT_FREE) { if (a4.y < 0) RUN(UNIT_FREE, 1); else RUN(UNIT_FREE, 4); }
            else if (a4.z < 0) RUN(UNIT_SHAKE, 2);
            else if (a4.w < 0) RUN(UNIT_SHAKE, 3);
            else RUN(UNIT_SHAKE, 4);
#undef RUN
        }
        if (last) break;
        {
            __shared__ long long s_pm[4][3];
            __shared__ unsigned long long s_tot[3];
            float3 pm = f3(0, 0, 0);
            if (active) {
#pragma unroll
                for (int k = 0; k < 4; ++k) if (idx[k] >= 0) pm = pm + S.v[k] * frcp(S.im[k]);
            }
            for (int off = 32; off > 0; off >>= 1) {
                pm.x += __shfl_xor(pm.x, off); pm.y += __shfl_xor(pm.y, off); pm.z += __shfl_xor(pm.z, off);
            }
            if ((threadIdx.x & 63) == 0) {
                long long* w = s_pm[threadIdx.x >> 6];
                w[0] = (long long)((double)pm.x * 4294967296.0); w[1] = (long long)((double)pm.y * 4294967296.0); w[2] = (long long)((double)pm.z * 4294967296.0);
            }
            if (threadIdx.x < 3) s_tot[threadIdx.x] = 0ull;
            __syncthreads();
            const unsigned long long tag = (unsigned long long)(prog.m_epoch & 0xffffu);
            unsigned long long* slots = chain_slots + ((size_t)(prog.m_epoch & 1u) * gridDim.y + r) * gridDim.x * 3;
            if (threadIdx.x < 3) {
                const long long t = s_pm[0][threadIdx.x] + s_pm[1][threadIdx.x] + s_pm[2][threadIdx.x] + s_pm[3][threadIdx.x];
                if (t >= (1ll << 46) || t < -(1ll << 46)) atomicCAS(chain_sync_err, 0u, 7u);
                __hip_atomic_store(&slots[blockIdx.x * 3 + threadIdx.x], ((unsigned long long)t << 16) | tag, __ATOMIC_RELAXED, __HIP_MEMORY_SCOPE_AGENT);
            }
            const int n_words = 3 * (int)gridDim.x;
            if (threadIdx.x < 255 && (int)threadIdx.x < n_words) {
                long long part = 0;
                for (int q = threadIdx.x; q < n_words; q += 255) {
                    unsigned long long w;
                    long long n = 0;
                    while (((w = __hip_atomic_load(&slots[q], __ATOMIC_RELAXED, __HIP_MEMORY_SCOPE_AGENT)) & 0xffffull) != tag) {
                        if ((n & 255) == 255 && __hip_atomic_load(chain_sync_err, __ATOMIC_RELAXED, __HIP_MEMORY_SCOPE_AGENT) != 0u) break;
                        __builtin_amdgcn_s_sleep(1);
                        if (++n > (1ll << 25)) { atomicCAS(chain_sync_err, 0u, 3u); break; }
                    }
                    part += (long long)w >> 16;
                }
                atomicAdd(&s_tot[threadIdx.x % 3], (unsigned long long)part);
            }
            __syncthreads();
            S.cmx = (float)(long long)s_tot[0] * (1.0f / 4294967296.0f) * inv_total_mass;
            S.cmy = (float)(long long)s_tot[1] * (1.0f / 4294967296.0f) * inv_total_mass;
            S.cmz = (float)(long long)s_tot[2] * (1.0f / 4294967296.0f) * inv_total_mass;
            S.have_cm = 1;
            __syncthreads();
#ifdef CHAIN_STAMPS
            if (S.stamps) { const unsigned long long now = wall_clock64(); atomicAdd(&S.stamps[1 + min(t1, 33)], now - S.t_last); S.t_last = now; }
#endif
        }
        t0 = t1 + 1;
    }
    if (wg_bins) {
        __shared__ int s_bin_cnt[CHAIN_BIN_COLS], s_bin_base[CHAIN_BIN_COLS];
        for (int c = threadIdx.x; c < bins.nx; c += blockDim.x) s_bin_cnt[c] = 0;
        __syncthreads();
        int col[4] = { 0, 0, 0, 0 }, rank[4] = { 0, 0, 0, 0 };
        if (active) {
#pragma unroll
            for (int k = 0; k < 4; ++k) {
                if (idx[k] >= 0) {
                    float u; int kx;
                    remd_pme_scaled1(S.x[k].x, bins.box[4 * r], bins.nx, u, kx);
                    if (kx >= bins.nx) kx -= bins.nx;
                    col[k] = kx; rank[k] = atomicAdd(&s_bin_cnt[kx], 1);
                }
            }
        }
        __syncthreads();
        for (int c = threadIdx.x; c < bins.nx; c += blockDim.x) {
            const int n = s_bin_cnt[c];
            if (n > 0) s_bin_base[c] = atomicAdd(&bins.count[(size_t)r * bins.nx + c], n);
        }
        __syncthreads();
        if (active) {
#pragma unroll
            for (int k = 0; k < 4; ++k) {
                if (idx[k] >= 0) {
                    const int slot = s_bin_base[col[k]] + rank[k];
                    if (slot < bins.cap) {
                        const size_t e = ((size_t)r * bins.nx + col[k]) * bins.cap + slot;
                        bins.atoms[e] = make_float4(S.x[k].x, S.x[k].y, S.x[k].z, __int_as_float(idx[k]));
                        if (bins.q) bins.q[e] = bins.param[idx[k]].x;
                    } else atomicCAS(bins.err, 0u, 2u);
                }
            }
        }
#ifdef CHAIN_STAMPS
        if (S.stamps) { const unsigned long long now = wall_clock64(); atomicAdd(&S.stamps[1 + 27], now - S.t_last); S.t_last = now; }
#endif
    }
    if (prog.accumulate_momentum) {
        for (int off = 32; off > 0; off >>= 1) {
            mom.x += __shfl_xor(mom.x, off); mom.y += __shfl_xor(mom.y, off); mom.z += __shfl_xor(mom.z, off);
        }
        if ((threadIdx.x & 63) == 0) {
            unsigned long long* c = reinterpret_cast<unsigned long long*>(cmm + ((size_t)cmm_w_eff * gridDim.y + r) * 4);
            atomicAdd(&c[0], (unsigned long long)(long long)((double)mom.x * 4294967296.0));
            atomicAdd(&c[1], (unsigned long long)(long long)((double)mom.y * 4294967296.0));
            atomicAdd(&c[2], (unsigned long long)(long long)((double)mom.z * 4294967296.0));
        }
    }
    if (prog.measure && work) {
        float hq = active ? S.heat : 0.f, sw = active ? S.shadow : 0.f;
        for (int off = 32; off > 0; off >>= 1) { hq += __shfl_xor(hq, off); sw += __shfl_xor(sw, off); }
        if ((threadIdx.x & 63) == 0) {
            unsigned long long* w = reinterpret_cast<unsigned long long*>(work + 4 * (size_t)r);
            if (prog.measure & 1) atomicAdd(&w[0], (unsigned long long)(long long)((double)hq * 16777216.0));
            if (prog.measure & 2) atomicAdd(&w[1], (unsigned long long)(long long)((double)sw * 16777216.0));
        }
    }
    if (type == UNIT_SHAKE && S.shake_it > 0 &&
        (unsigned int)S.shake_it > __hip_atomic_load(chain_sync_err + 1, __ATOMIC_RELAXED, __HIP_MEMORY_SCOPE_AGENT))
        atomicMax(chain_sync_err + 1, (unsigned int)S.shake_it);
    if (own_time && blockIdx.x == 0 && blockIdx.y == 0 && threadIdx.x == 0) {
        atomicAdd(&own_time[0], wall_clock64() - own_t0);
        atomicAdd(&own_time[1], 1ull);
    }
}

__global__ __launch_bounds__(256)
void integrate_chain_kernel(chain_prog prog, int n_units, const int4* __restrict__ unit_atoms, const unsigned char* __restrict__ unit_type,
                            const float* __restrict__ shake_dist, settle_const sc, float tol, int Npad, float4* __restrict__ pos,
                            float4* __restrict__ vel, long long* force, const float* __restrict__ invmass, const int64_t* __restrict__ labels,
                            const double* __restrict__ beta, int r_begin, uint64_t seed, long long* __restrict__ cmm, float inv_total_mass,
                            unsigned int* join_flag, unsigned int join_seq, remd_chain_bins bins, unsigned long long* chain_slots,
                            unsigned int* chain_sync_err, unsigned long long* own_time, long long* __restrict__ work, float4* __restrict__ xold,
                            float4* __restrict__ vold, remd_fold_args fold, const unsigned int* __restrict__ noise_id)
{
    integrate_chain_body(prog, n_units, unit_atoms, unit_type, shake_dist, sc, tol, Npad, pos, vel, force, invmass, labels, beta, r_begin, seed,
                         cmm, inv_total_mass, join_flag, join_seq, bins, chain_slots, chain_sync_err, own_time, work, xold, vold, fold, noise_id);
}

template <int TYPE, int NAT>
__device__ __forceinline__ void assign_unit(const int* idx, const settle_const& sc, float tol, const float4* __restrict__ P,
                                            float4* __restrict__ V, const float* __restrict__ invmass, float kT, uint32_t rg,
                                            uint64_t seed, int64_t iteration)
{
    float3 x[NAT], v[NAT];
    float im[NAT];
#pragma unroll
    for (int k = 0; k < NAT; ++k) {
        const float4 p = P[idx[k]];
        x[k] = f3(p.x, p.y, p.z);
        im[k] = invmass[idx[k]];
        const float3 xi = gaussian3(seed, REMD_STREAM_VELOCITY, (uint32_t)idx[k], rg, (uint64_t)iteration);
        const float sig = fsqrt(kT * im[k]);
        v[k] = xi * sig;
    }
    constrain_v<TYPE, NAT>(sc, im, tol, v, x);
#pragma unroll
    for (int k = 0; k < NAT; ++k) V[idx[k]] = make_float4(v[k].x, v[k].y, v[k].z, 0.f);
}

__global__ __launch_bounds__(256)
void assign_velocities_kernel(int n_units, const int4* __restrict__ unit_atoms,
                              const unsigned char* __restrict__ unit_type, settle_const sc, float tol,
                              int Npad, const float4* __restrict__ pos, float4* __restrict__ vel,
                              const float* __restrict__ invmass, const int64_t* __restrict__ labels,
                              const double* __restrict__ beta, int r_begin, uint64_t seed, int64_t iteration,
                              const unsigned int* __restrict__ noise_id)
{
    const int uidx = blockIdx.x * blockDim.x + threadIdx.x;
    const int r = blockIdx.y;
    if (uidx >= n_units) return;
    const int4 a4 = unit_atoms[uidx];
    if (a4.x < 0) return;
// ... 79 lines not shown
            dist.push_back(0); dist.push_back(0); dist.push_back(0);
        }
        for (; q < fr.size(); ++q) {
            atoms.push_back(make_int4(fr[q], -1, -1, -1)); type.push_back(UNIT_FREE);
            dist.push_back(0); dist.push_back(0); dist.push_back(0);
        }
    }
    ut.n_units = (int)atoms.size();
    REMD_TRY(ut.d_atoms.upload(h, atoms));
    REMD_TRY(ut.d_type.upload(h, type));
    REMD_TRY(ut.d_dist.upload(h, dist));
    h->n_settle = d->n_settle; h->n_shake = d->n_shake;
    int n_con = 3 * d->n_settle;
    for (int s = 0; s < d->n_shake; ++s) for (int k = 1; k < 4; ++k) if (d->shake_atoms[4 * s + k] >= 0) n_con++;
    h->n_dof = 3 * N - n_con - (d->cmm_frequency > 0 ? 3 : 0);
    if (d->n_settle > 0) {
        const int* a = d->settle_atoms;
        const double mO = d->mass[a[0]], mH = d->mass[a[1]];
        const double rc = 0.5 * d->settle_dHH;
        const double t = sqrt(d->settle_dOH * d->settle_dOH - rc * rc);
        const double ra = 2.0 * mH * t / (mO + 2.0 * mH);
        ut.sc.mO = (float)mO; ut.sc.mH = (float)mH; ut.sc.ra = (float)ra; ut.sc.rb = (float)(t - ra);
        ut.sc.rc = (float)rc; ut.sc.dOH = (float)d->settle_dOH; ut.sc.dHH = (float)d->settle_dHH;
    }
    return 0;
}

int remd_parse_splitting(remd_ctx* h, const char* splitting, std::vector<char>& tokens, int& nV, int& nR, int& nO, int* nVg)
{
    tokens.clear(); nV = nR = nO = 0;
    std::string s(splitting ? splitting : "");
    std::vector<int> vgroup;
    size_t i = 0;
    while (i < s.size()) {
        while (i < s.size() && s[i] == ' ') ++i;
        if (i >= s.size()) break;
        size_t j = i; while (j < s.size() && s[j] != ' ') ++j;
        std::string tok = s.substr(i, j - i);
        for (auto& c : tok) c = (char)toupper(c);
        if (tok[0] == 'V' && tok.find_first_not_of("0123456789", 1) == std::string::npos) {
            int g = -1;
            if (tok.size() > 1) {
                if (tok.size() > 3) return remd_fail(h, -3, "force group of '" + tok + "' out of range");
                g = atoi(tok.c_str() + 1);
                if (g > 31) return remd_fail(h, -3, "OpenMM only allows up to 32 force groups (integrators.py:1346-1347)");
            }
            tokens.push_back('V'); vgroup.push_back(g); nV++;
        }
        else if (tok == "R") { tokens.push_back('R'); nR++; }
        else if (tok == "O") { tokens.push_back('O'); nO++; }
        else if (tok == "{" || tok == "}") tokens.push_back(tok[0]);
        else return remd_fail(h, -3, "unsupported splitting token '" + tok + "' (supported: V V<group> R O { })");
        i = j;
    }
    {
        std::set<int> groups;
        for (int g : vgroup) if (g >= 0) groups.insert(g);
        int counts[4] = {0, 0, 0, 0};
        if (groups.size() > 1) {
            if (!nVg) return remd_fail(h, -3, "multiple-time-step splittings are set with remd_set_integrator");
            size_t v = 0;
            for (auto& c : tokens) if (c == 'V') {
                const int g = vgroup[v++];
                if (g < 0) return remd_fail(h, -3, "a multiple-time-step splitting must name the force group of every V (integrators.py:1527-1529)");
                if (g > 3) return remd_fail(h, -3, "force groups above 3 are not supported in multiple-time-step splittings");
                c = (char)('0' + g); counts[g]++;
            }
        }
        if (nVg) for (int g = 0; g < 4; ++g) nVg[g] = counts[g];
    }
    if (tokens.empty()) return remd_fail(h, -3, "empty splitting string");
    if (nR == 0 || nV == 0) return remd_fail(h, -3, "splitting needs at least one R and one V (integrators.py:1376-1385)");
    int depth = 0;
    for (char c : tokens) {
        if (c == '{') { if (++depth > 1) return remd_fail(h, -3, "nested '{' in the splitting string"); }
        else if (c == '}') { if (--depth < 0) return remd_fail(h, -3, "'}' without '{' in the splitting string"); }
        else if (c == 'O' && depth > 0) return remd_fail(h, -3, "O substeps cannot be Metropolized (integrators.py:1387-1401)");
    }
    if (depth != 0) return remd_fail(h, -3, "'{' without '}' in the splitting string");
    return 0;
}

remd_chain_bins remd_pme_chain_bins(remd_ctx* h);
static void launch_chain(remd_ctx* h, const unit_tables& ut, const chain_prog& prog, bool bin_for_pme = false)
{
    const bool chain_bins = h->sw.pme_chainbin >= 0 ? h->sw.pme_chainbin != 0
                                                    : (h->parent == nullptr || (long long)((ut.n_units + 255) / 256) * h->R > 1024);
    const remd_chain_bins bins = (bin_for_pme && chain_bins) ? remd_pme_chain_bins(h) : remd_chain_bins();
    remd_prof_scope ps(h, "integrate_chain");
    dim3 grid((ut.n_units + 255) / 256, h->R);
    hipLaunchKernelGGL(integrate_chain_kernel, grid, dim3(256), 0, h->stream, prog, ut.n_units, ut.d_atoms, ut.d_type,
                       ut.d_dist, ut.sc, (float)fmax(h->constraint_tol, REMD_CONSTRAINT_TOL_FLOOR), h->Npad, h->d_pos, h->d_vel, h->d_force,
                       h->d_invmass, h->d_labels, h->d_beta, h->r_begin, h->seed, h->d_cmm,
                       (float)(h->total_mass > 0 ? 1.0 / h->total_mass : 0.0),
                       h->join_deferred ? h->d_sync + 1 : (unsigned int*)nullptr, h->join_deferred, bins, h->d_chain_sync, h->d_sync + 2,
                       (h->profiling == 2 || (h->profiling == 1 && h->prof_filter.find("integrate_chain") != std::string::npos)) ? h->d_chain_own : (unsigned long long*)nullptr,
                       h->d_work, h->d_xold, h->d_vold, h->fold_pending ? h->fold : remd_fold_args(), h->d_noise_id);
    h->join_deferred = 0; h->fold_pending = false;
    if (bins.count) h->cbins_ready = true;
}

#define WORK_SCALE 16777216.0
__global__ void work_pe_kernel(int R, const double* __restrict__ U, double* __restrict__ pe_prev, long long* __restrict__ work, int accumulate)
{
    const int r = blockIdx.x * blockDim.x + threadIdx.x;
    if (r >= R) return;
    if (accumulate) work[4 * r + 1] += (long long)((U[r] - pe_prev[r]) * WORK_SCALE);
    pe_prev[r] = U[r];
}
__global__ void metropolis_kernel(int R, int r_begin, uint64_t seed, long long gstep, int brace, const int64_t* __restrict__ labels,
                                  const double* __restrict__ beta, long long* __restrict__ work, int* __restrict__ accept,
                                  const unsigned int* __restrict__ noise_id)
{
    const int r = blockIdx.x * blockDim.x + threadIdx.x;
    if (r >= R) return;
    const double sw = (double)work[4 * r + 1] / WORK_SCALE;
    const philox4 w = remd_philox(seed, REMD_STREAM_METROPOLIS, (uint32_t)brace, noise_id ? noise_id[r] : (uint32_t)(r_begin + r), (uint64_t)gstep);
    const double u = remd_u53(w.w[2], w.w[3]);
    const int acc = (exp(-sw * beta[labels[r_begin + r]]) - u >= 0.0) ? 1 : 0;
    accept[r] = acc;
    work[4 * r + 2] += 1;
    if (!acc) work[4 * r + 3] += 1;
    work[4 * r + 1] = 0;
}
__global__ __launch_bounds__(256)
void metropolis_restore_kernel(int N, int Npad, const int* __restrict__ accept, float4* __restrict__ pos, float4* __restrict__ vel,
                               const float4* __restrict__ xold, const float4* __restrict__ vold)
{
    const int i = blockIdx.x * blockDim.x + threadIdx.x, r = blockIdx.y;
    if (i >= N || accept[r]) return;
    const size_t o = (size_t)r * Npad + i;
    pos[o] = xold[o];
    const float4 v = vold[o];
    vel[o] = make_float4(-v.x, -v.y, -v.z, 0.f);
}
int remd_work_buffers(remd_ctx* h)
{
    if (h->d_work.size() == 4 * (size_t)h->R) return 0;
    REMD_TRY(h->d_work.alloc(h, 4 * (size_t)h->R));
    REMD_TRY(h->d_pe_prev.alloc(h, h->R));
    REMD_TRY(h->d_xold.alloc(h, (size_t)h->R * h->Npad));
    REMD_TRY(h->d_vold.alloc(h, (size_t)h->R * h->Npad));
    REMD_TRY(h->d_accept.alloc(h, h->R));
    REMD_CHECK(h, hipMemsetAsync(h->d_work, 0, sizeof(long long) * 4 * h->R, h->stream));
    return 0;
}

struct resident_prog {
    int n; char tok[MAX_TOK]; int o_index[MAX_TOK];
    float hV, hR, a, b; int nO;
    int n_steps, cmm_frequency; long long gstep0, first_step;
};
struct resident_sys {
    int N, Npad, method, alch, n_ext, list_cap;
    nb_params p;
    float skin, ext_K, ext_x0, inv_total_mass;
    const float4* param; const float* rep_lam; const int* ext_atoms; const float* invmass; const float* box;
    const int64_t* labels; const double* beta; int r_begin; uint64_t seed; const unsigned int* noise_id;
    unsigned int* err;
};

#ifndef RES_UNROLL
#define RES_UNROLL 2
#endif
#define RES_FSCALE 8192.f

template <bool ALCH>
__device__ __forceinline__ float resident_pair(const nb_params& p, float r2, float4 pi, float4 pj, float lam_a, float sc)
{
    const float inv_r = __builtin_amdgcn_rsqf(r2), r = r2 * inv_r;
    const float sig = pi.y + pj.y, eps4 = pi.z * pj.z;
    const bool soft = ALCH && ((pi.w != pj.w) || pi.w > 1.5f);
    const float lam = soft ? lam_a : 1.f, s0 = soft ? sc : 0.f;
    const float is2 = __builtin_amdgcn_rcpf(sig * sig);
    const float q2 = r2 * is2, t = q2 * q2 * q2;
    const float x = __builtin_amdgcn_rcpf(s0 + t);
    float U = lam * eps4 * x * (x - 1.f);
    float dUdr = lam * eps4 * (2.f * x - 1.f) * (-x * x * 6.f * t * inv_r);
    const float xs = fminf(fmaxf((r - p.rs) * p.inv_sw, 0.f), 1.f);
    const float Sw = 1.f + xs * xs * xs * (-10.f + xs * (15.f - 6.f * xs));
// ... 984 lines not shown
```

### openmmtools_amd/csrc/pme.hip

```cpp
#include "remd_internal.h"
#include "listed_terms.h"
#include "pme_pow2.h"
#include <cmath>
#include <vector>
#include <type_traits>

#ifndef PME_PRIO
#define PME_PRIO 3
#endif
#define PME_ORDER 5
#define FFT_B 8
#define FFT_T 32
#define PME_FIXED_SCALE 68719476736.0

struct fft_sched { const uint2* tab; int off[8]; };

struct pme_state {
    bool prio_hi = true;
    int n[4] = {0, 0, 0, 0};
    int R = 0;
    size_t npts = 0;
    bool ready = false;
    dev_array<float2> d_grid;
    hipStream_t stream = nullptr;
    int nzc = 0; size_t nspec = 0; size_t xy_lds = 0; bool xy_fused = false; int xy_threads = 512;
    int xy_pow2 = 0;
    dev_array<int> d_col_count; dev_array<int> d_col_start; dev_array<int> d_cursor; dev_array<int> d_atom_col; dev_array<int> d_col_atoms;
    dev_array<float2> d_tw[4];
    dev_array<float> d_bmod[3];
    int nrad[4] = {0, 0, 0, 0}; int radix[4][8];
    int xs_sw = 0;
    int ys_sh = 0;
    dev_array<float> d_infl; int infl_version = -1;
    int infl_rep = 0;
    bool z_half = false;
    dev_array<double> d_energy;
    int n_eblk = 0;
    fft_sched sch_x, sch_y, sch_z;
    dev_array<uint2> d_sched[3];
    int sch_nl = 0, sch_zt = 0;
    dev_array<float> d_cbin_q;
    dev_array<unsigned long long> d_fbin; size_t fbin_P = 0;
    dev_array<int> d_cbin_count; dev_array<float4> d_cbin_atoms; int cbin_cap = 0, cbin_parity = 0; bool cbin_use = false;
};

__device__ __forceinline__ float2 cmul(float2 a, float2 b) { return make_float2(a.x * b.x - a.y * b.y, a.x * b.y + a.y * b.x); }
__device__ __forceinline__ float2 cadd(float2 a, float2 b) { return make_float2(a.x + b.x, a.y + b.y); }
__device__ __forceinline__ float2 csub(float2 a, float2 b) { return make_float2(a.x - b.x, a.y - b.y); }

struct fft_plan { int n; int nrad; int radix[8]; unsigned mnb[8]; unsigned mNs[8]; int prio;  };
__host__ __device__ __forceinline__ unsigned fft_magic(unsigned d) { return (unsigned)((0x100000000ull + d - 1) / d); }
__device__ __forceinline__ int fft_div(int x, unsigned magic, int d) { return d == 1 ? x : (int)__umulhi((unsigned)x, magic); }

template <int SIGN>
__device__ __forceinline__ void bfly2(float2* v) { const float2 a = v[0], b = v[1]; v[0] = cadd(a, b); v[1] = csub(a, b); }
template <int SIGN>
__device__ __forceinline__ void bfly3(float2* v)
{
    const float c = -0.5f, s = SIGN * 0.86602540378443865f;
    const float2 t1 = cadd(v[1], v[2]);
    const float2 t2 = make_float2(v[0].x + c * t1.x, v[0].y + c * t1.y);
    const float2 d = csub(v[1], v[2]);
    const float2 t3 = make_float2(-s * d.y, s * d.x);
    v[0] = cadd(v[0], t1); v[1] = cadd(t2, t3); v[2] = csub(t2, t3);
}
template <int SIGN>
__device__ __forceinline__ void bfly4(float2* v)
{
    const float2 a = cadd(v[0], v[2]), b = csub(v[0], v[2]), c = cadd(v[1], v[3]), d = csub(v[1], v[3]);
    const float2 id = make_float2(-SIGN * d.y, SIGN * d.x);
    v[0] = cadd(a, c); v[2] = csub(a, c); v[1] = cadd(b, id); v[3] = csub(b, id);
}
template <int SIGN>
__device__ __forceinline__ void bfly8(float2* v)
{
    float2 e[4] = { v[0], v[2], v[4], v[6] }, o[4] = { v[1], v[3], v[5], v[7] };
    bfly4<SIGN>(e); bfly4<SIGN>(o);
    const float h = 0.70710678118654752f;
    const float2 o1 = make_float2((o[1].x - SIGN * o[1].y) * h, (o[1].y + SIGN * o[1].x) * h);
    const float2 o2 = make_float2(-SIGN * o[2].y, SIGN * o[2].x);
    const float2 o3 = make_float2((-o[3].x - SIGN * o[3].y) * h, (-o[3].y + SIGN * o[3].x) * h);
    v[0] = cadd(e[0], o[0]); v[4] = csub(e[0], o[0]);
    v[1] = cadd(e[1], o1);   v[5] = csub(e[1], o1);
    v[2] = cadd(e[2], o2);   v[6] = csub(e[2], o2);
    v[3] = cadd(e[3], o3);   v[7] = csub(e[3], o3);
}
template <int SIGN>
__device__ __forceinline__ void bfly5(float2* v)
{
    const float c1 = 0.30901699437494745f, c2 = -0.80901699437494745f;
    const float s1 = SIGN * 0.95105651629515353f, s2 = SIGN * 0.58778525229247314f;
    const float2 a1 = cadd(v[1], v[4]), a2 = cadd(v[2], v[3]), b1 = csub(v[1], v[4]), b2 = csub(v[2], v[3]);
    const float2 x0 = v[0];
    v[0] = make_float2(x0.x + a1.x + a2.x, x0.y + a1.y + a2.y);
    const float2 p1 = make_float2(x0.x + c1 * a1.x + c2 * a2.x, x0.y + c1 * a1.y + c2 * a2.y);
    const float2 p2 = make_float2(x0.x + c2 * a1.x + c1 * a2.x, x0.y + c2 * a1.y + c1 * a2.y);
    const float2 q1 = make_float2(s1 * b1.x + s2 * b2.x, s1 * b1.y + s2 * b2.y);
    const float2 q2 = make_float2(s2 * b1.x - s1 * b2.x, s2 * b1.y - s1 * b2.y);
    v[1] = make_float2(p1.x - q1.y, p1.y + q1.x); v[4] = make_float2(p1.x + q1.y, p1.y - q1.x);
    v[2] = make_float2(p2.x - q2.y, p2.y + q2.x); v[3] = make_float2(p2.x + q2.y, p2.y - q2.x);
}

template <int SIGN>
__device__ float2* fft_lines_lds(const fft_plan& pl, float2* src, float2* dst, int nlines, int ls, int es,
                                 const float2* __restrict__ tw, int tid, int nthreads, bool lines_fastest = false)
{
    const int n = pl.n;
    const unsigned mlines = fft_magic((unsigned)nlines);
    int Ns = 1;
    for (int s = 0; s < pl.nrad; ++s) {
        const int Rx = pl.radix[s];
        const int nb = n / Rx;
        const int total = nlines * nb;
        const int tstride = n / (Ns * Rx);
        const unsigned mnb = pl.mnb[s], mNs = pl.mNs[s];
        for (int idx = tid; idx < total; idx += nthreads) {
            int l, j;
            if (ls == 1 || lines_fastest) { j = fft_div(idx, mlines, nlines); l = idx - j * nlines; }
            else { l = fft_div(idx, mnb, nb); j = idx - l * nb; }
            const int jq = fft_div(j, mNs, Ns);
            const int k = j - jq * Ns;
            const int tstep = k * tstride;
            const float2* S = src + l * ls;
            float2 v[8];
#pragma unroll
// ... 79 lines not shown
        Ns *= Rx;
    }
}

#define PME_MESH_SCALE 16777216.0f

__device__ __forceinline__ void bspline5(float f, float* w, float* d)
{
    float a[5] = { f, 1.f - f, 0.f, 0.f, 0.f };
#pragma unroll
    for (int m = 3; m <= 4; ++m) {
        const float div = 1.f / (m - 1);
#pragma unroll
        for (int j = 4; j >= 0; --j) if (j < m) {
            const float prev = (j > 0) ? a[j - 1] : 0.f;
            const float cur = (j < m - 1) ? a[j] : 0.f;
            a[j] = div * ((f + j) * cur + (m - f - j) * prev);
        }
    }
#pragma unroll
    for (int j = 0; j < 5; ++j) {
        const float prev = (j > 0) ? a[j - 1] : 0.f;
        const float cur = (j < 4) ? a[j] : 0.f;
        d[j] = cur - prev;
        w[j] = 0.25f * ((f + j) * cur + (5.f - f - j) * prev);
    }
}

__device__ __forceinline__ void pme_scaled(const float4 x, const float* __restrict__ box4, int nx, int ny, int nz,
                                           float& ux, float& uy, float& uz, int& kx, int& ky, int& kz)
{
    remd_pme_scaled1(x.x, box4[0], nx, ux, kx);
    remd_pme_scaled1(x.y, box4[1], ny, uy, ky);
    remd_pme_scaled1(x.z, box4[2], nz, uz, kz);
}

struct pme_cand { int n[5]; int base[5]; int ntot; };
__device__ __forceinline__ pme_cand pme_candidates(const int* __restrict__ cs, int x, int nx, int cap)
{
    pme_cand c;
    if (cap > 0) {
        c.ntot = 0;
#pragma unroll
        for (int b = 0; b < 5; ++b) {
            int kx = x + b; if (kx >= nx) kx -= nx;
            c.n[b] = min(cs[kx], cap); c.base[b] = kx * cap; c.ntot += c.n[b];
        }
    } else {
        const int xe = x + 5;
        const int beg0 = cs[x], end0 = cs[xe <= nx ? xe : nx];
        const int beg1 = cs[0], end1 = (xe <= nx) ? beg1 : cs[xe - nx];
        c.n[0] = end0 - beg0; c.base[0] = beg0; c.n[1] = end1 - beg1; c.base[1] = beg1;
        c.n[2] = c.n[3] = c.n[4] = 0; c.base[2] = c.base[3] = c.base[4] = 0;
        c.ntot = c.n[0] + c.n[1];
    }
    return c;
}
__device__ __forceinline__ int pme_cand_atom(const pme_cand& c, const int* __restrict__ ca, int t, bool capped,
                                             const float4* __restrict__ P, float4& xi, const float* __restrict__ cq,
                                             const float4* __restrict__ param, const float* __restrict__ rep_lam, int r, float& q, int* flat = nullptr)
{
    int base = c.base[0];
#pragma unroll
    for (int b = 0; b < 4; ++b) if (t >= c.n[b]) { t -= c.n[b]; base = c.base[b + 1]; } else break;
    if (flat) *flat = base + t;
    int i;
    if (capped) {
        xi = reinterpret_cast<const float4*>(ca)[base + t];
        i = __float_as_int(xi.w);
        if (cq) { q = cq[base + t]; return i; }
    } else {
        i = ca[base + t];
        xi = P[i];
    }
    const float4 pr = param[i];
    q = pr.x;
    if (rep_lam && pr.w != 0.f) q *= rep_lam[4 * r + (pr.w >= 8.f ? (int)pr.w - 8 : 2)];
    return i;
}

__global__ __launch_bounds__(1024)
void pme_bin_kernel(int N, int Npad, int nx, int ny, int nz, const float4* __restrict__ pos, const float* __restrict__ box,
                    int* __restrict__ bin_start , int* __restrict__ bin_atoms ,
                    unsigned int* fork_flag, unsigned int fork_seq)
{
    if (fork_flag && blockIdx.x == 0 && threadIdx.x == 0) __hip_atomic_store(fork_flag, fork_seq, __ATOMIC_RELEASE, __HIP_MEMORY_SCOPE_AGENT);
    __builtin_amdgcn_s_setprio(PME_PRIO);
    __shared__ int s_cnt[257], s_start[257], s_cur[256];
    const int r = blockIdx.x, tid = threadIdx.x;
    for (int k = tid; k <= nx; k += 1024) s_cnt[k] = 0;
    __syncthreads();
    for (int i = tid; i < N; i += 1024) {
        float ux, uy, uz; int kx, ky, kz;
        pme_scaled(pos[(size_t)r * Npad + i], box + 4 * r, nx, ny, nz, ux, uy, uz, kx, ky, kz);
        if (kx >= nx) kx -= nx;
        atomicAdd(&s_cnt[kx], 1);
    }
    __syncthreads();
    if (tid == 0) {
        int run = 0;
        for (int k = 0; k < nx; ++k) { s_start[k] = run; s_cur[k] = run; run += s_cnt[k]; }
        s_start[nx] = run;
    }
    __syncthreads();
    for (int i = tid; i < N; i += 1024) {
        float ux, uy, uz; int kx, ky, kz;
        pme_scaled(pos[(size_t)r * Npad + i], box + 4 * r, nx, ny, nz, ux, uy, uz, kx, ky, kz);
        if (kx >= nx) kx -= nx;
        const int slot = atomicAdd(&s_cur[kx], 1);
        bin_atoms[(size_t)r * Npad + slot] = i;
    }
    for (int k = tid; k <= nx; k += 1024) bin_start[(size_t)r * (nx + 1) + k] = s_start[k];
}

#define Z_PPT 12

template <int Z_THREADS, bool HALF>
__global__ __launch_bounds__(Z_THREADS)
void pme_spread_zfwd_kernel(fft_plan pl, fft_sched sc, int nl, int nx, int ny, int Npad, const float4* __restrict__ pos,
                            const float4* __restrict__ param, const float* __restrict__ box, const float* __restrict__ rep_lam,
                            const int* __restrict__ col_start, const int* __restrict__ col_atoms,
                            float2* __restrict__ spec, const float2* tw, const float2* tw_half,
                            int bin_cap, int* __restrict__ zero_count, unsigned int* fork_flag, unsigned int fork_seq,
                            const float* __restrict__ bin_q, listed_tables LT, int n_mesh_blocks, long long* __restrict__ force)
{
    if ((int)blockIdx.x >= n_mesh_blocks) {
        listed_forces_body(LT, Npad, pos, box, force, ((int)blockIdx.x - n_mesh_blocks) * Z_THREADS + (int)threadIdx.x, blockIdx.y);
        return;
    }
    if (pl.prio) __builtin_amdgcn_s_setprio(PME_PRIO);
    extern __shared__ __attribute__((aligned(16))) char smem[];
    const int M = pl.n;
    const int nz = HALF ? 2 * M : M, nzc = nz / 2 + 1, PZ = HALF ? ((M + 1) | 1) : (nz | 1);
    float2* buf = reinterpret_cast<float2*>(smem);
    float2* s_tw = buf + nl * PZ;
    float2* s_twh = s_tw + nz;
    int* acc = reinterpret_cast<int*>(buf);
    const int r = blockIdx.y, tid = threadIdx.x;
    const int nbpr = (ny + nl - 1) / nl;
    const int x = blockIdx.x / nbpr, y0 = (blockIdx.x - x * nbpr) * nl;
    for (int idx = tid; idx < nl * nz; idx += Z_THREADS) acc[idx] = 0;
    for (int idx = tid; idx < nz; idx += Z_THREADS) s_tw[idx] = tw[idx];
    if (HALF) for (int idx = tid; idx < M; idx += Z_THREADS) s_twh[idx] = tw_half[idx];
    __syncthreads();
    const int* cs = col_start + (size_t)r * (bin_cap > 0 ? nx : nx + 1);
    const int* ca = col_atoms + (size_t)r * (bin_cap > 0 ? (size_t)nx * bin_cap * 4 : (size_t)Npad);
    const float4* P = pos + (size_t)r * Npad;
    if (zero_count && blockIdx.x == 0) for (int k = tid; k < nx; k += Z_THREADS) zero_count[(size_t)r * nx + k] = 0;
    if (fork_flag && blockIdx.x == 0 && blockIdx.y == 0 && tid == 0)
        __hip_atomic_store(fork_flag, fork_seq, __ATOMIC_RELEASE, __HIP_MEMORY_SCOPE_AGENT);
    {
        const pme_cand cnd = pme_candidates(cs, x, nx, bin_cap);
        const int ntot = cnd.ntot;
        for (int t = tid; t < ntot; t += Z_THREADS) {
            float4 xi; float q;
            pme_cand_atom(cnd, ca, t, bin_cap > 0, P, xi, bin_q ? bin_q + (size_t)r * nx * bin_cap : (const float*)nullptr, param, rep_lam, r, q);
            if (q == 0.f) continue;
            float ux, uy, uz; int kx, ky, kz;
            pme_scaled(xi, box + 4 * r, nx, ny, nz, ux, uy, uz, kx, ky, kz);
            float wx[5], wy[5], wz[5], dx[5], dy[5], dz[5];
            bspline5(ux - kx, wx, dx); bspline5(uy - ky, wy, dy); bspline5(uz - kz, wz, dz);
            if (kx >= nx) kx -= nx; if (ky >= ny) ky -= ny; if (kz >= nz) kz -= nz;
            int a = kx - x; if (a < 0) a += nx;
            float wa = 0.f;
#pragma unroll
            for (int k = 0; k < 5; ++k) if (k == a) wa = wx[k];
            const float qa = q * wa * PME_MESH_SCALE;
#pragma unroll
            for (int b = 0; b < 5; ++b) {
                int iy = ky - b; if (iy < 0) iy += ny;
                const int lb = iy - y0;
                if (lb < 0 || lb >= nl) continue;
                const float qab = qa * wy[b];
#pragma unroll
                for (int c = 0; c < 5; ++c) {
                    int iz = kz - c; if (iz < 0) iz += nz;
                    atomicAdd(&acc[lb * nz + iz], __float2int_rn(qab * wz[c]));
                }
            }
        }
    }
    __syncthreads();
    const unsigned mM = fft_magic((unsigned)M);
    {
        float2 val[Z_PPT];
#pragma unroll
        for (int q = 0; q < Z_PPT; ++q) {
            const int idx = tid + q * Z_THREADS;
            val[q] = make_float2(0.f, 0.f);
            if (idx < nl * M) {
                if (HALF) { const int2 w = reinterpret_cast<const int2*>(acc)[idx]; val[q] = make_float2((float)w.x * (1.0f / PME_MESH_SCALE), (float)w.y * (1.0f / PME_MESH_SCALE)); }
                else val[q].x = (float)acc[idx] * (1.0f / PME_MESH_SCALE);
            }
// ... 615 lines not shown
    int e = 0;
    while (m % 2 == 0) { ++e; m /= 2; }
    const int st = (e + 2) / 3;
    for (int k = 0, left = e; k < st; ++k) { const int b = (left + (st - k) - 1) / (st - k); radix[nrad++] = 1 << b; left -= b; }
    while (m % 3 == 0) { radix[nrad++] = 3; m /= 3; }
    while (m % 5 == 0) { radix[nrad++] = 5; m /= 5; }
    return m == 1 && nrad <= 8;
}

static double bspline_M(int order, double u)
{
    if (order == 2) return (u < 0 || u > 2) ? 0.0 : 1.0 - fabs(u - 1.0);
    return u / (order - 1) * bspline_M(order - 1, u) + (order - u) / (order - 1) * bspline_M(order - 1, u - 1.0);
}

void remd_table_deleter::operator()(pme_state* s) const { delete s; }

static fft_plan make_plan(pme_state* s, int axis)
{
    fft_plan pl; pl.n = s->n[axis]; pl.nrad = s->nrad[axis]; pl.prio = s->prio_hi ? 1 : 0;
    int Ns = 1;
    for (int k = 0; k < 8; ++k) {
        pl.radix[k] = s->radix[axis][k];
        pl.mnb[k] = pl.mNs[k] = 0;
        if (k < pl.nrad) { pl.mnb[k] = fft_magic((unsigned)(pl.n / pl.radix[k])); pl.mNs[k] = fft_magic((unsigned)Ns); Ns *= pl.radix[k]; }
    }
    return pl;
}

static int build_sched(remd_ctx* h, pme_state* s, int axis, int nlines, int ls, int es, int nthreads, int ppt,
                       fft_sched* out, dev_array<uint2>& d_tab)
{
    const int n = s->n[axis];
    std::vector<uint2> tab;
    int Ns = 1;
    for (int st = 0; st < s->nrad[axis]; ++st) {
        const int Rx = s->radix[axis][st];
        const int NB = (ppt + Rx - 1) / Rx;
        const int nb = n / Rx, total = nlines * nb, tstride = n / (Ns * Rx);
        if ((long long)NB * nthreads < total) return remd_fail(h, -3, "PME FFT pass does not fit the workgroup registers");
        out->off[st] = (int)tab.size();
        const size_t base = tab.size();
        tab.resize(base + (size_t)NB * nthreads, make_uint2(0xffffffffu, 0u));
        if ((nlines - 1) * ls + (n - 1) * es > 0xffff) return remd_fail(h, -3, "PME plane too large for the FFT schedule");
        for (int b = 0; b < NB; ++b)
            for (int t = 0; t < nthreads; ++t) {
                const int idx = t + b * nthreads;
                if (idx >= total) continue;
                const int l = idx % nlines, j = idx / nlines;
                const int jq = j / Ns, k = j % Ns;
                const int src = l * ls + j * es, dst = l * ls + (jq * Ns * Rx + k) * es;
                tab[base + (size_t)b * nthreads + t] = make_uint2((unsigned)src | ((unsigned)dst << 16), (unsigned)(k * tstride));
            }
        Ns *= Rx;
    }
    REMD_TRY(d_tab.upload(h, tab));
    out->tab = d_tab;
    return 0;
}

static int pme_setup_impl(remd_ctx* h, bool full_complex)
{
    h->pme.reset(new pme_state());
    pme_state* s = h->pme.get();
    for (int k = 0; k < 3; ++k) {
        s->n[k] = h->grid[k];
        if (s->n[k] < 6 || s->n[k] > 256 || !factorize(s->n[k], s->radix[k], s->nrad[k]))
            return remd_fail(h, -3, "PME mesh sizes must be products of 2, 3, 5 between 6 and 256");
    }
    s->n[3] = s->n[2] / 2;
    s->z_half = (s->n[2] % 2 == 0) && s->n[3] >= 3 && factorize(s->n[3], s->radix[3], s->nrad[3]) &&
                true;
    s->R = h->R;
    s->npts = (size_t)s->n[0] * s->n[1] * s->n[2];
    s->nzc = s->n[2] / 2 + 1;
    s->nspec = (size_t)s->nzc * s->n[0] * s->n[1];
    if (full_complex) {
        REMD_TRY(s->d_grid.alloc(h, s->npts * s->R));
    } else {
        s->ready = true;
        REMD_TRY(s->d_grid.alloc(h, s->nspec * s->R));
        REMD_TRY(s->d_col_start.alloc(h, (size_t)(s->n[0] + 1) * s->R));
        REMD_TRY(s->d_col_atoms.alloc(h, (size_t)h->Npad * s->R));
        if (!full_complex && h->sw.pme_chainbin != 0) {
            s->cbin_cap = std::min(h->Npad, std::max(64, 4 * ((h->N + s->n[0] - 1) / s->n[0])));
            if (h->sw.pme_cbin_cap) s->cbin_cap = h->sw.pme_cbin_cap;
            REMD_TRY(s->d_cbin_count.alloc(h, 2 * (size_t)s->R * s->n[0]));
            REMD_CHECK(h, hipMemset(s->d_cbin_count, 0, sizeof(int) * 2 * (size_t)s->R * s->n[0]));
            REMD_TRY(s->d_cbin_atoms.alloc(h, (size_t)s->R * s->n[0] * s->cbin_cap));
            REMD_TRY(s->d_cbin_q.alloc(h, (size_t)s->R * s->n[0] * s->cbin_cap));
        }
    }
    if (s->z_half) {
        const int n = s->n[3];
        std::vector<float2> tw(n);
        for (int j = 0; j < n; ++j) tw[j] = make_float2((float)cos(2.0 * M_PI * j / n), (float)(-sin(2.0 * M_PI * j / n)));
        REMD_TRY(s->d_tw[3].alloc(h, n));
        REMD_CHECK(h, hipMemcpy(s->d_tw[3], tw.data(), sizeof(float2) * n, hipMemcpyHostToDevice));
    }
    for (int k = 0; k < 3; ++k) {
        const int n = s->n[k];
        std::vector<float2> tw(n);
        for (int j = 0; j < n; ++j) tw[j] = make_float2((float)cos(2.0 * M_PI * j / n), (float)(-sin(2.0 * M_PI * j / n)));
        REMD_TRY(s->d_tw[k].alloc(h, n));
        REMD_CHECK(h, hipMemcpy(s->d_tw[k], tw.data(), sizeof(float2) * n, hipMemcpyHostToDevice));
        std::vector<float> bm(n);
        for (int m = 0; m < n; ++m) {
            double re = 0, im = 0;
            for (int k2 = 0; k2 <= PME_ORDER - 2; ++k2) {
                const double w = bspline_M(PME_ORDER, k2 + 1.0), arg = 2.0 * M_PI * m * k2 / n;
                re += w * cos(arg); im += w * sin(arg);
            }
            bm[m] = (float)(re * re + im * im);
        }
        for (int m = 0; m < n; ++m)
            if (bm[m] < 1e-7f) bm[m] = 0.5f * (bm[(m + n - 1) % n] + bm[(m + 1) % n]);
        REMD_TRY(s->d_bmod[k].alloc(h, n));
        REMD_CHECK(h, hipMemcpy(s->d_bmod[k], bm.data(), sizeof(float) * n, hipMemcpyHostToDevice));
    }
    s->n_eblk = s->nzc;
    REMD_TRY(s->d_energy.alloc(h, (size_t)s->n_eblk * s->R));
    s->xy_lds = sizeof(float2) * ((size_t)s->n[0] * (s->n[1] | 1) + s->n[0] + s->n[1]) + 128;
    {
        const long long np = (long long)s->n[0] * s->n[1];
        long long best_cost = -1; int best_t = 0;
        const int xy_cands[4] = {512, 256, 768, 1024};
        for (int tc = 0; tc < 4; ++tc) {
            const int t = xy_cands[tc];
            long long cost = 0; bool ok = true;
            for (int ax = 0; ax < 2 && ok; ++ax)
                for (int st = 0; st < s->nrad[ax]; ++st) {
                    const int rx = s->radix[ax][st];
                    const long long slots = (np / rx + t - 1) / t;
                    if (slots > (XY_PPT + rx - 1) / rx) ok = false;
                    cost += slots * t * rx;
                }
            if (ok && (best_cost < 0 || cost < best_cost)) { best_cost = cost; best_t = t; }
        }
        s->xy_threads = best_t > 0 ? best_t : 1024;
        s->xy_fused = best_t > 0 && s->xy_lds <= 160 * 1024;
    }
    if (!s->xy_fused && !full_complex) {
        for (int c = 1; c <= s->n[1]; ++c)
            if (s->n[1] % c == 0 && (long long)s->n[0] * c <= (long long)XY_PPT * XS_THREADS && (size_t)s->n[0] * (c | 1) * 8 <= 40 * 1024) s->xs_sw = c;
        if (s->xs_sw > 0) {
            int rc = build_sched(h, s, 0, s->xs_sw, 1, s->xs_sw | 1, XS_THREADS, XY_PPT, &s->sch_x, s->d_sched[0]);
            if (rc) return rc;
            s->n_eblk = s->nzc * (s->n[1] / s->xs_sw);
            REMD_TRY(s->d_energy.alloc(h, (size_t)s->n_eblk * s->R));
            REMD_CHECK(h, hipFuncSetAttribute((const void*)pme_x_fused_kernel, hipFuncAttributeMaxDynamicSharedMemorySize, 64 * 1024));
            for (int c = 1; c <= s->n[0]; ++c)
                if (s->n[0] % c == 0 && (long long)s->n[1] * c <= (long long)XY_PPT * XS_THREADS && (size_t)c * (s->n[1] | 1) * 8 <= 40 * 1024) s->ys_sh = c;
            if (s->ys_sh > 0) {
                rc = build_sched(h, s, 1, s->ys_sh, s->n[1] | 1, 1, XS_THREADS, XY_PPT, &s->sch_y, s->d_sched[1]);
                if (rc) return rc;
                REMD_CHECK(h, hipFuncSetAttribute((const void*)pme_y_slab_kernel<-1>, hipFuncAttributeMaxDynamicSharedMemorySize, 64 * 1024));
                REMD_CHECK(h, hipFuncSetAttribute((const void*)pme_y_slab_kernel<+1>, hipFuncAttributeMaxDynamicSharedMemorySize, 64 * 1024));
            }
        }
    }
    if (s->xy_fused && !full_complex && s->n[0] == s->n[1] && (s->n[0] == 64 || s->n[0] == 128) &&
        (h->sw.pme_pow2 & 1)) {
        s->xy_pow2 = s->n[0];
        s->xy_threads = s->n[0] == 64 ? 512 : 1024;
        s->xy_lds = sizeof(float2) * ((size_t)s->n[0] * (s->n[0] + 8) + s->n[0]) + sizeof(double) * 16;
        REMD_CHECK(h, hipFuncSetAttribute((const void*)pme_xy_pow2_kernel<64, 8, false>, hipFuncAttributeMaxDynamicSharedMemorySize, 64 * 1024));
        REMD_CHECK(h, hipFuncSetAttribute((const void*)pme_xy_pow2_kernel<64, 8, true>, hipFuncAttributeMaxDynamicSharedMemorySize, 64 * 1024));
        REMD_CHECK(h, hipFuncSetAttribute((const void*)pme_xy_pow2_kernel<128, 16, false>, hipFuncAttributeMaxDynamicSharedMemorySize, 160 * 1024));
        REMD_CHECK(h, hipFuncSetAttribute((const void*)pme_xy_pow2_kernel<128, 16, true>, hipFuncAttributeMaxDynamicSharedMemorySize, 160 * 1024));
    }
    if (s->xy_fused && !full_complex && !s->xy_pow2) {
        REMD_CHECK(h, hipFuncSetAttribute((const void*)pme_xy_fused_kernel, hipFuncAttributeMaxDynamicSharedMemorySize, (int)s->xy_lds));
        const int PS = s->n[1] | 1;
        int rc = build_sched(h, s, 1, s->n[0], PS, 1, s->xy_threads, XY_PPT, &s->sch_y, s->d_sched[1]);
        if (!rc) rc = build_sched(h, s, 0, s->n[1], 1, PS, s->xy_threads, XY_PPT, &s->sch_x, s->d_sched[0]);
        if (rc) return rc;
    }
#define Z_LDS_ATTR(ZT, HF) \
    REMD_CHECK(h, hipFuncSetAttribute((const void*)pme_spread_zfwd_kernel<ZT, HF>, hipFuncAttributeMaxDynamicSharedMemorySize, 160 * 1024)); \
    REMD_CHECK(h, hipFuncSetAttribute((const void*)pme_zinv_gather_kernel<ZT, HF>, hipFuncAttributeMaxDynamicSharedMemorySize, 160 * 1024));
    Z_LDS_ATTR(512, false) Z_LDS_ATTR(256, false) Z_LDS_ATTR(512, true) Z_LDS_ATTR(256, true)
#undef Z_LDS_ATTR
    REMD_CHECK(h, hipDeviceSynchronize());
    return 0;
}

int remd_pme_setup(remd_ctx* h) { return pme_setup_impl(h, false); }

template <int SIGN>
static void launch_pass(remd_ctx* h, pme_state* s, float2* data, size_t rep_stride, int axis_n_index, int es, int lines,
                        int line_div, size_t hi, int contiguous)
{
    fft_plan pl = make_plan(s, axis_n_index);
    dim3 grid((lines + FFT_B - 1) / FFT_B, s->R);
    const size_t lds = sizeof(float2) * 2 * FFT_B * pl.n;
    hipLaunchKernelGGL((fft_pass_kernel<SIGN, 0>), grid, dim3(FFT_B * FFT_T), lds, s->stream ? s->stream : h->stream, pl, data, rep_stride, es, lines,
                       line_div, hi, contiguous, s->d_tw[axis_n_index]);
}

const float* remd_nb_rep_lam(remd_ctx* h);
const float4* remd_nb_param(remd_ctx* h);

int remd_pme_forces(remd_ctx* h, bool with_energy, hipStream_t st, int part)
{
    pme_state* s = h->pme.get();
    if (!s || s->R != h->R || !s->ready) { int rc = remd_pme_setup(h); if (rc) return rc; s = h->pme.get(); }
    s->stream = st;
    s->prio_hi = h->mesh_prio_hi;
    const int nx = s->n[0], ny = s->n[1], nz = s->n[2];
    const float* rep_lam = remd_nb_rep_lam(h);
    const float4* param = remd_nb_param(h);
    if (part & 1) {
    s->cbin_use = h->cbins_ready && s->d_cbin_count;
    h->cbins_ready = false;
    if (!s->cbin_use)
    {
        remd_prof_scope ps(h, "pme_bin", st);
        hipLaunchKernelGGL(pme_bin_kernel, dim3(h->R), dim3(1024), 0, st, h->N, h->Npad, nx, ny, nz, h->d_pos, h->d_box,
                           s->d_col_start, s->d_col_atoms, h->fork_seq_pending ? h->d_sync : (unsigned int*)nullptr, h->fork_seq_pending);
        h->fork_seq_pending = 0;
    }
    {
        remd_prof_scope ps(h, "pme_fft", st);
        const bool half = s->z_half;
        const int zaxis = half ? 3 : 2;
        const int M = s->n[zaxis], PZ = half ? ((M + 1) | 1) : (nz | 1);
        const int ZT = (long long)ny * M <= (long long)Z_PPT * 256 ? 256 : 512;
        int nl = 1;
        for (int c = 1; c <= ny; ++c) if (ny % c == 0 && c * M <= Z_PPT * ZT) nl = c;
        const size_t zlds = sizeof(float2) * ((size_t)nl * PZ + nz + (half ? M : 0));
        const dim3 zgrid(nx * ((ny + nl - 1) / nl), s->R);
        if (s->sch_nl != nl || s->sch_zt != ZT) {
            int rc = build_sched(h, s, zaxis, nl, PZ, 1, ZT, Z_PPT, &s->sch_z, s->d_sched[2]);
            if (rc) return rc;
            s->sch_nl = nl; s->sch_zt = ZT;
        }
#define LAUNCH_Z(KERN, ZTT, HF, ...) hipLaunchKernelGGL((KERN<ZTT, HF>), zgrid, dim3(ZTT), zlds, st, make_plan(s, zaxis), s->sch_z, nl, nx, ny, __VA_ARGS__)
#define DISPATCH_Z(KERN, ...) do { if (ZT == 256) { if (half) LAUNCH_Z(KERN, 256, true, __VA_ARGS__); else LAUNCH_Z(KERN, 256, false, __VA_ARGS__); } \
                                   else { if (half) LAUNCH_Z(KERN, 512, true, __VA_ARGS__); else LAUNCH_Z(KERN, 512, false, __VA_ARGS__); } } while (0)
        const int* bin_cs = s->cbin_use ? s->d_cbin_count + (size_t)s->cbin_parity * s->R * nx : s->d_col_start;
        const int* bin_ca = s->cbin_use ? reinterpret_cast<const int*>(s->d_cbin_atoms.get()) : s->d_col_atoms;
        const int bin_cap = s->cbin_use ? s->cbin_cap : 0;
        int* bin_zero = s->cbin_use ? s->d_cbin_count + (size_t)(1 - s->cbin_parity) * s->R * nx : (int*)nullptr;
        unsigned int* fflag = (s->cbin_use && h->fork_seq_pending) ? h->d_sync : (unsigned int*)nullptr;
        const unsigned int fseq = h->fork_seq_pending;
        if (s->cbin_use) { h->fork_seq_pending = 0; }
        const int n_mesh_blocks = (int)zgrid.x;
        const int n_listed_blocks = h->mesh_listed_total > 0 ? (h->mesh_listed_total + ZT - 1) / ZT : 0;
        const int zp2 = ((h->sw.pme_pow2 & 2) && half && (nz == 64 || nz == 128) && ny % 64 == 0 && nl == 64 && ZT == 64 * (nz / 16)) ? nz : 0;
        const size_t zlds2 = sizeof(float2) * (size_t)(nz / 2 + 1) * 64;
        if (zp2) {
            const dim3 zg(zgrid.x + n_listed_blocks, zgrid.y);
#define LAUNCH_ZF2(MMM, RR) hipLaunchKernelGGL((pme_spread_zfwd_pow2_kernel<MMM, RR>), zg, dim3(64 * RR), zlds2, st, nx, ny, h->Npad, h->d_pos, param, h->d_box, rep_lam, \
                       bin_cs, bin_ca, s->d_grid, s->d_tw[2], s->d_tw[3], bin_cap, bin_zero, fflag, fseq, \
                       (s->cbin_use && !rep_lam) ? s->d_cbin_q : (const float*)nullptr, h->mesh_listed, n_mesh_blocks, h->d_force, s->prio_hi ? 1 : 0)
            if (zp2 == 64) LAUNCH_ZF2(32, 4); else LAUNCH_ZF2(64, 8);
#undef LAUNCH_ZF2
        } else
        {
            const dim3 zgrid_keep = zgrid;
            const dim3 zgrid(zgrid_keep.x + n_listed_blocks, zgrid_keep.y);
            DISPATCH_Z(pme_spread_zfwd_kernel, h->Npad, h->d_pos, param, h->d_box, rep_lam, bin_cs, bin_ca, s->d_grid,
                       s->d_tw[2], s->d_tw[3], bin_cap, bin_zero, fflag, fseq, (s->cbin_use && !rep_lam) ? s->d_cbin_q : (const float*)nullptr,
                       h->mesh_listed, n_mesh_blocks, h->d_force);
        }
        h->mesh_listed_total = 0;
        if (s->xy_fused || s->xs_sw > 0) {
            if (!s->d_infl) REMD_TRY(s->d_infl.alloc(h, s->nspec * s->R));
            if (s->infl_version != h->box_version) {
                hipLaunchKernelGGL(pme_influence_table_kernel, dim3(s->nzc, h->box_uniform ? 1 : s->R), dim3(256), 0, st, nx, ny, nz, s->d_bmod[0], s->d_bmod[1],
                                   s->d_bmod[2], h->d_box, (float)h->ewald_alpha, s->d_infl, s->xy_pow2 == 64 ? 8 : s->xy_pow2 == 128 ? 16 : 0);
                s->infl_version = h->box_version;
                s->infl_rep = h->box_uniform ? 0 : s->nzc;
            }
        }
        if (s->xy_pow2) {
            remd_prof_scope pxy(h, "pme_xy", st);
#define LAUNCH_XY_P2(NN, RR, TT, WE) hipLaunchKernelGGL((pme_xy_pow2_kernel<NN, RR, WE>), dim3(s->nzc, s->R), dim3(TT), s->xy_lds, st, nz, s->d_grid, \
                                   s->d_tw[0], s->d_energy, s->n_eblk, s->d_infl, s->infl_rep, s->prio_hi ? 1 : 0)
            if (s->xy_pow2 == 64) { if (with_energy) LAUNCH_XY_P2(64, 8, 512, true); else LAUNCH_XY_P2(64, 8, 512, false); }
            else { if (with_energy) LAUNCH_XY_P2(128, 16, 1024, true); else LAUNCH_XY_P2(128, 16, 1024, false); }
#undef LAUNCH_XY_P2
        } else if (s->xy_fused) {
            remd_prof_scope pxy(h, "pme_xy", st);
            hipLaunchKernelGGL(pme_xy_fused_kernel, dim3(s->nzc, s->R), dim3(s->xy_threads), s->xy_lds, st, make_plan(s, 0), make_plan(s, 1),
                               s->sch_x, s->sch_y, nz, s->d_grid, s->d_tw[0], s->d_tw[1], s->d_bmod[0], s->d_bmod[1], s->d_bmod[2], h->d_box,
                               (float)h->ewald_alpha, with_energy ? 1 : 0, s->d_energy, s->n_eblk, s->d_infl, s->infl_rep);
        } else if (s->xs_sw > 0) {
            const size_t ylds = sizeof(float2) * ((size_t)s->ys_sh * (ny | 1) + ny + 2);
            if (s->ys_sh > 0)
                hipLaunchKernelGGL(pme_y_slab_kernel<-1>, dim3(s->nzc * (nx / s->ys_sh), s->R), dim3(XS_THREADS), ylds, st, make_plan(s, 1), s->sch_y,
                                   nx, nz, s->ys_sh, s->d_grid, s->d_tw[1]);
            else
                launch_pass<-1>(h, s, s->d_grid, s->nspec, 1, 1, s->nzc * nx, s->nzc * nx, 0, 1);
            const int PS = s->xs_sw | 1;
            const size_t lds = sizeof(float2) * ((size_t)nx * PS + nx + 2) + 64;
            hipLaunchKernelGGL(pme_x_fused_kernel, dim3(s->nzc * (ny / s->xs_sw), s->R), dim3(XS_THREADS), lds, st, make_plan(s, 0), s->sch_x,
                               ny, nz, s->xs_sw, s->d_grid, s->d_tw[0], with_energy ? 1 : 0, s->d_energy, s->n_eblk, s->d_infl, s->infl_rep);
            if (s->ys_sh > 0)
                hipLaunchKernelGGL(pme_y_slab_kernel<+1>, dim3(s->nzc * (nx / s->ys_sh), s->R), dim3(XS_THREADS), ylds, st, make_plan(s, 1), s->sch_y,
                                   nx, nz, s->ys_sh, s->d_grid, s->d_tw[1]);
            else
                launch_pass<+1>(h, s, s->d_grid, s->nspec, 1, 1, s->nzc * nx, s->nzc * nx, 0, 1);
        } else {
            launch_pass<-1>(h, s, s->d_grid, s->nspec, 1, 1, s->nzc * nx, s->nzc * nx, 0, 1);
            launch_pass<-1>(h, s, s->d_grid, s->nspec, 0, ny, s->nzc * ny, ny, (size_t)nx * ny, 0);
            hipLaunchKernelGGL(pme_influence_kernel, dim3(s->nzc, s->R), dim3(256), 0, st, nx, ny, nz, s->d_grid, s->d_bmod[0],
                               s->d_bmod[1], s->d_bmod[2], h->d_box, (float)h->ewald_alpha, with_energy ? 1 : 0, s->d_energy, s->n_eblk);
            launch_pass<+1>(h, s, s->d_grid, s->nspec, 0, ny, s->nzc * ny, ny, (size_t)nx * ny, 0);
            launch_pass<+1>(h, s, s->d_grid, s->nspec, 1, 1, s->nzc * nx, s->nzc * nx, 0, 1);
        }
        if (h->sw.pme_fbin && !s->d_fbin) {
            s->fbin_P = std::max((size_t)nx * (size_t)std::max(s->cbin_cap, 0), (size_t)h->Npad);
            REMD_TRY(s->d_fbin.alloc(h, 3 * s->fbin_P * s->R));
            REMD_CHECK(h, hipMemsetAsync(s->d_fbin, 0, sizeof(unsigned long long) * 3 * s->fbin_P * s->R, st));
        }
        unsigned long long* fbin = h->sw.pme_fbin ? s->d_fbin : (unsigned long long*)nullptr;
        {
        remd_prof_scope pzg(h, "pme_zinv_gather", st);
        if (zp2) {
#define LAUNCH_ZI2(MMM, RR) hipLaunchKernelGGL((pme_zinv_gather_pow2_kernel<MMM, RR>), zgrid, dim3(64 * RR), zlds2, st, nx, ny, s->d_grid, s->d_tw[2], s->d_tw[3], \
                       h->Npad, h->d_pos, param, h->d_box, rep_lam, bin_cs, bin_ca, h->d_force, bin_cap, \
                       (s->cbin_use && !rep_lam) ? s->d_cbin_q : (const float*)nullptr, s->prio_hi ? 1 : 0, fbin, s->fbin_P)
            if (zp2 == 64) LAUNCH_ZI2(32, 4); else LAUNCH_ZI2(64, 8);
#undef LAUNCH_ZI2
        } else
        DISPATCH_Z(pme_zinv_gather_kernel, s->d_grid, s->d_tw[2], s->d_tw[3], h->Npad, h->d_pos, param, h->d_box, rep_lam,
                   bin_cs, bin_ca, h->d_force, bin_cap, (s->cbin_use && !rep_lam) ? s->d_cbin_q : (const float*)nullptr, fbin, s->fbin_P);
        if (fbin) {
            const int npos = bin_cap > 0 ? nx * bin_cap : h->N;
            hipLaunchKernelGGL(pme_unbin_forces_kernel, dim3((npos + 255) / 256, s->R), dim3(256), 0, st, nx, bin_cap, h->N, h->Npad, s->fbin_P,
                               bin_cs, bin_ca, fbin, h->d_force);
        }
        if (s->cbin_use) s->cbin_parity ^= 1;
        }
#undef DISPATCH_Z
#undef LAUNCH_Z
    }
    }
    if (!(part & 2)) { REMD_CHECK(h, hipGetLastError()); return 0; }
    if (with_energy)
        hipLaunchKernelGGL(pme_energy_reduce_kernel, dim3(h->R), dim3(64), 0, st, s->n_eblk, s->d_energy, h->d_epart,
                           h->n_epart, 6 );
    REMD_CHECK(h, hipGetLastError());
    return 0;
}

remd_chain_bins remd_pme_chain_bins(remd_ctx* h)
{
    remd_chain_bins b;
    const pme_state* s = h->pme.get();
    if (!s || !s->d_cbin_count || s->R != h->R || !h->pme_concurrent || h->no_chain_bins) return b;
    b.nx = s->n[0]; b.cap = s->cbin_cap; b.count = s->d_cbin_count + (size_t)s->cbin_parity * s->R * s->n[0]; b.atoms = s->d_cbin_atoms;
    b.box = h->d_box; b.err = h->d_sync + 2;
    b.param = remd_nb_param(h);
    b.q = (b.param && !remd_nb_rep_lam(h)) ? s->d_cbin_q : nullptr;
    return b;
}

int remd_test_fft3d_impl(remd_ctx* h, int nx, int ny, int nz, float* data, int inverse)
{
    remd_table<pme_state> old = std::move(h->pme);
    const int oldgrid[3] = { h->grid[0], h->grid[1], h->grid[2] };
    const int oldR = h->R;
    h->grid[0] = nx; h->grid[1] = ny; h->grid[2] = nz; h->R = 1;
    int rc = pme_setup_impl(h, true);
    if (!rc) {
        pme_state* s = h->pme.get();
        hipMemcpy(s->d_grid, data, sizeof(float2) * s->npts, hipMemcpyHostToDevice);
        auto all = [&](auto tag) {
            constexpr int SG = decltype(tag)::value;
            launch_pass<SG>(h, s, s->d_grid, s->npts, 2, 1, nx * ny, nx * ny, 0, 1);
            launch_pass<SG>(h, s, s->d_grid, s->npts, 1, nz, nx * nz, nz, (size_t)ny * nz, 0);
            launch_pass<SG>(h, s, s->d_grid, s->npts, 0, ny * nz, ny * nz, ny * nz, 0, 0);
        };
        if (!inverse) all(std::integral_constant<int, -1>()); else all(std::integral_constant<int, +1>());
        hipStreamSynchronize(h->stream);
        hipMemcpy(data, s->d_grid, sizeof(float2) * s->npts, hipMemcpyDeviceToHost);
        if (hipGetLastError() != hipSuccess) rc = remd_fail(h, -2, "fft test launch failed");
    }
    h->pme = std::move(old); h->grid[0] = oldgrid[0]; h->grid[1] = oldgrid[1]; h->grid[2] = oldgrid[2]; h->R = oldR;
    return rc;
}
```

### openmmtools_amd/csrc/remd_internal.h

```cpp
#pragma once
#include <hip/hip_runtime.h>
#include <stdint.h>
#include <stdlib.h>
#include <algorithm>
#include <string>
#include <map>
#include <memory>
#include <vector>
#include "../../include/remd_hip.h"

#define REMD_KB 0.00831446261815324
#define REMD_ONE_4PI_EPS0 138.93545764438198

struct remd_error { int code; std::string msg; };

struct remd_ctx;
void remd_set_global_error(const std::string& s);
int remd_hip_fail(remd_ctx* h, const char* what, hipError_t e);

template <typename T>
struct dev_array {
    dev_array() = default;
    dev_array(const dev_array&) = delete;
    dev_array& operator=(const dev_array&) = delete;
    dev_array(dev_array&& o) noexcept : p_(o.p_), n_(o.n_) { o.p_ = nullptr; o.n_ = 0; }
    dev_array& operator=(dev_array&& o) noexcept { if (this != &o) { reset(); std::swap(p_, o.p_); std::swap(n_, o.n_); } return *this; }
    ~dev_array() { reset(); }
    operator T*() const { return p_; }
    T* get() const { return p_; }
    size_t size() const { return n_; }
    void reset() { if (p_) hipFree(p_); p_ = nullptr; n_ = 0; }
    int alloc(remd_ctx* h, size_t n)
    {
        reset();
        if (!n) return 0;
        const hipError_t e = hipMalloc(&p_, sizeof(T) * n);
        if (e != hipSuccess) { p_ = nullptr; return remd_hip_fail(h, "hipMalloc", e); }
        n_ = n;
        return 0;
    }
    int grow(remd_ctx* h, size_t n) { return n_ >= n && p_ ? 0 : alloc(h, n); }
    int upload(remd_ctx* h, const std::vector<T>& host)
    {
        if (int rc = alloc(h, host.size())) return rc;
        if (host.empty()) return 0;
        const hipError_t e = hipMemcpy(p_, host.data(), sizeof(T) * host.size(), hipMemcpyHostToDevice);
        return e == hipSuccess ? 0 : remd_hip_fail(h, "hipMemcpy", e);
    }
private:
    T* p_ = nullptr; size_t n_ = 0;
};

#define REMD_TRY(expr) do { const int _rc = (expr); if (_rc) return _rc; } while (0)

struct nb_tables; struct pme_state; struct unit_tables; struct gbsa_tables; struct nocutoff_tables; struct region_tables; struct rst_tables;
struct mix_pre_buffers;
struct remd_table_deleter {
    void operator()(nb_tables*) const; void operator()(pme_state*) const; void operator()(unit_tables*) const;
    void operator()(gbsa_tables*) const; void operator()(nocutoff_tables*) const; void operator()(region_tables*) const;
    void operator()(rst_tables*) const; void operator()(mix_pre_buffers*) const;
};
template <typename T> using remd_table = std::unique_ptr<T, remd_table_deleter>;
template <typename T> T& remd_table_of(remd_table<T>& t) { if (!t) t.reset(new T()); return *t; }

#define REMD_FORCE_SCALE 4294967296.0
#define REMD_CONSTRAINT_TOL_FLOOR 2e-7

__device__ __forceinline__ void remd_pme_scaled1(float x, float L, int n, float& u, int& k)
{
    float f = x / L;
    f -= floorf(f);
    u = f * n;
    k = (int)u;
}
struct remd_chain_bins { int nx = 0, cap = 0; int* count = nullptr; float4* atoms = nullptr; const float* box = nullptr; unsigned int* err = nullptr;
                         float* q = nullptr; const float4* param = nullptr; const float* rep_lam = nullptr; };

__device__ __forceinline__ unsigned long long remd_f2fix(float f)
{
    const float a = fabsf(f);
    const float hi_f = floorf(a);
    const unsigned int lo = (unsigned int)((a - hi_f) * 4294967296.f);
    const unsigned int hi = (unsigned int)(int)hi_f;
    const unsigned long long v = ((unsigned long long)hi << 32) | lo;
    return f < 0.f ? 0ull - v : v;
}

struct remd_fold_args {
    const unsigned int* done = nullptr; unsigned int target = 0;
};

struct listed_tables {
    int n_bonds, n_angles, n_torsions, n_exc, n_excl;
    const int *bond_atoms, *angle_atoms, *torsion_atoms, *exc_atoms, *excl_atoms;
    const float *bond_params, *angle_params, *torsion_params, *exc_params, *excl_qq;
    const int *exc_alch, *excl_alch; const float* rep_lam;
    float alpha, two_alpha_sqrtpi;
    int n_aterm; const unsigned int* aterm;
};

struct remd_profile_entry { int64_t n = 0; double ms = 0.0; };

struct remd_desc_store {
    remd_system_desc d{}; bool valid = false;
    std::vector<double> mass, bond_params, angle_params, torsion_params, charge, sigma, epsilon, exception_params, shake_dist;
    std::vector<int32_t> ext_atoms, bond_atoms, angle_atoms, torsion_atoms, exception_atoms, settle_atoms, shake_atoms, alch_atoms;
    void assign(const remd_system_desc* s)
    {
        d = *s;
        auto cpd = [](std::vector<double>& v, const double*& p, size_t n) { if (p && n) { v.assign(p, p + n); p = v.data(); } else { v.clear(); if (!n) p = nullptr; } };
        auto cpi = [](std::vector<int32_t>& v, const int32_t*& p, size_t n) { if (p && n) { v.assign(p, p + n); p = v.data(); } else { v.clear(); if (!n) p = nullptr; } };
        const size_t N = (size_t)d.n_atoms;
        cpd(mass, d.mass, N); cpi(ext_atoms, d.ext_atoms, (size_t)d.n_ext);
        cpi(bond_atoms, d.bond_atoms, 2 * (size_t)d.n_bonds); cpd(bond_params, d.bond_params, 2 * (size_t)d.n_bonds);
        cpi(angle_atoms, d.angle_atoms, 3 * (size_t)d.n_angles); cpd(angle_params, d.angle_params, 2 * (size_t)d.n_angles);
        cpi(torsion_atoms, d.torsion_atoms, 4 * (size_t)d.n_torsions); cpd(torsion_params, d.torsion_params, 3 * (size_t)d.n_torsions);
        cpd(charge, d.charge, N); cpd(sigma, d.sigma, N); cpd(epsilon, d.epsilon, N);
        cpi(exception_atoms, d.exception_atoms, 2 * (size_t)d.n_exceptions); cpd(exception_params, d.exception_params, 3 * (size_t)d.n_exceptions);
        cpi(settle_atoms, d.settle_atoms, 3 * (size_t)d.n_settle);
        cpi(shake_atoms, d.shake_atoms, 4 * (size_t)d.n_shake); cpd(shake_dist, d.shake_dist, 3 * (size_t)d.n_shake);
        cpi(alch_atoms, d.alch_atoms, (size_t)d.n_alch);
        valid = true;
    }
};

struct remd_switches {
    bool overlap = true;
    int phases = -1;
    bool resident = true;
    int resident_cap = 0;
    bool chain_merge = true;
    bool nb_tiles = false;
    int nb_persist_grid = -1;
    int nb_prio = -1;
    bool nb_fold = true;
    bool listed_atoms = true;
    bool listed_main = true;
    bool listed_ride = true;
    int pme_chainbin = -1;
    int pme_cbin_cap = 0;
    int pme_pow2 = 3;
    bool pme_fbin = true;
    bool gb_small = true;
    int mix_flow = -1;
    bool mix_pre = true;
    bool debug = false;
    bool nb_tune_verbose = false;
    bool many_verbose = false;
    int prof_every = 16;
};

struct remd_ctx {
    int device = 0;
    remd_switches sw;
    hipStream_t stream = nullptr; bool owns_stream = false;
    std::string err;
    uint64_t seed = 0;

    int N = 0;
    int Npad = 0;
    bool has_system = false;
    dev_array<float> d_invmass;
    dev_array<float> d_mass;
    double total_mass = 0.0;
    int n_ext = 0; dev_array<int> d_ext_atoms; double ext_K = 0, ext_x0 = 0, ext_U0 = 0;
    int n_bonds = 0, n_angles = 0, n_torsions = 0;
    dev_array<int> d_bond_atoms; dev_array<float> d_bond_params;
    dev_array<unsigned int> d_aterm; int n_aterm = 0;
    dev_array<int> d_angle_atoms; dev_array<float> d_angle_params;
    dev_array<int> d_torsion_atoms; dev_array<float> d_torsion_params;
    int nb_method = REMD_NB_NONE;
    int gbsa = 0;
// ... 15 lines not shown
    double self_energy = 0;
    int n_settle = 0; dev_array<int> d_settle_atoms; double settle_dOH = 0, settle_dHH = 0;
    int n_shake = 0;  dev_array<int> d_shake_atoms; dev_array<float> d_shake_dist;
    int n_groups = 0; dev_array<int> d_group_first;
    dev_array<int> d_free_atoms; int n_free = 0;
    int cmm_frequency = 0;
    int n_dof = 0;
    int n_alch = 0; dev_array<int> d_alch_atoms;
    double sc_alpha = 0.5, sc_a = 1, sc_b = 1, sc_c = 6;
    int n_regions = 0;
    int regions_exact = 0;
    long long states_version = 0;
    int n_restraints = 0, rst_group = 0;

    int K = 0;
    std::vector<double> beta, lam_s, lam_e, econst;
    dev_array<double> d_beta; dev_array<double> d_lam_s; dev_array<double> d_lam_e; dev_array<double> d_econst;

    std::string splitting = "V R O R V";
    std::vector<char> tokens;
    int nV = 0, nR = 0, nO = 0;
    int nVg[4] = {0, 0, 0, 0};
    int fgroup[6] = {0, 0, 0, 0, 0, 0};
    dev_array<long long> d_force_g[4];
    double dt = 0.001, gamma = 1.0, constraint_tol = 1e-8;
    int n_steps = 1; int reassign = 1;
    bool has_integrator = false;
    int measure_heat = 0, measure_shadow = 0;
    dev_array<long long> d_snap_work;
    dev_array<long long> d_work;
    dev_array<double> d_pe_prev;
    dev_array<float4> d_xold; dev_array<float4> d_vold; dev_array<int> d_accept;

    int R_global = 0, r_begin = 0, R = 0;
    dev_array<unsigned int> d_noise_id;
    dev_array<float4> d_pos;
    dev_array<float4> d_vel;
    int baro_frequency = 0; long long baro_steps = 0, baro_attempts = 0; std::vector<double> pressure_host;
    double econst_vref = 0.0;
    dev_array<double> d_pressure;
    dev_array<double> d_baro;
    dev_array<float> d_box_old; dev_array<float4> d_baro_x0; dev_array<long long> d_baro_f0; dev_array<double> d_baro_U0; dev_array<int> d_baro_acc;
    bool box_uniform = false;
    int box_version = 0;
    int n_restart_attempts = 0;
    dev_array<unsigned int> d_mix_log;
    bool mix_pre_launched = false, mix_no_pre = false;
    double mix_acc_rate = -1.0;
    dev_array<float4> d_snap_pos; dev_array<float4> d_snap_vel;
    dev_array<float4> d_fin_pos; dev_array<float4> d_fin_vel;
    dev_array<float> d_snap_box; dev_array<float> d_fin_box;
    dev_array<float4> d_pos_ref;
    dev_array<long long> d_force;
    dev_array<float> d_box;
    std::vector<double> box_host;
    dev_array<int64_t> d_labels;
    std::vector<int64_t> labels;
    dev_array<double> d_ukl;
    dev_array<double> d_potential;
    dev_array<double> d_epart; int n_epart = 0;
    dev_array<double> d_kinetic;
    dev_array<int> d_nan;
    dev_array<long long> d_cmm;
    bool forces_valid = false;
    bool force_zeroed = false;

    remd_table<pme_state> pme;
    remd_table<nb_tables> nb;
    remd_table<unit_tables> units;
    remd_table<nocutoff_tables> nc;
    remd_table<gbsa_tables> gb;
    remd_table<region_tables> reg;
    remd_table<rst_tables> rst;
    remd_table<mix_pre_buffers> mix_pre;

    dev_array<unsigned long long> d_nacc; dev_array<unsigned long long> d_nprop; int stats_K = 0;
    dev_array<double> d_logw; dev_array<double> d_logP; dev_array<double> d_ukl_tmp;

    hipEvent_t ev0 = nullptr, ev1 = nullptr;
    dev_array<unsigned int> d_sync; unsigned int sync_seq = 0; unsigned int fork_seq_pending = 0; bool sync_events = false;
    bool defer_join_ok = false; unsigned int join_deferred = 0;
    listed_tables mesh_listed{}; int mesh_listed_total = 0;
    remd_fold_args fold; bool fold_pending = false;
    bool mesh_prio_hi = true;
    bool no_device_waits = false, no_chain_bins = false, no_resident = false, no_chain_merge = false;
    bool lean_waits = false, no_chain_barrier = false;
    int phases_req = 0; int phases_last = 1;
    std::vector<remd_ctx*> phase; remd_ctx* parent = nullptr; int seen_parent_box = -1; long long ids_version = 0, seen_parent_ids = -1;
    long long config_version = 0, phase_config = -1;
    std::unique_ptr<remd_desc_store> sysdesc;
    std::vector<int64_t> noise_id_host;
    bool borrowed_stream2 = false;
    dev_array<unsigned long long> d_chain_own;
    dev_array<unsigned long long> d_chain_sync; unsigned int chain_sync_epoch = 0; long long chain_sync_key = -1;
    bool cbins_ready = false;
    hipStream_t stream2 = nullptr; hipEvent_t ev_fork = nullptr, ev_join = nullptr; bool pme_concurrent = false;
    void* comm = nullptr; int comm_rank = 0, comm_world = 1;
    std::vector<long long> comm_begin, comm_count;
    dev_array<long long> d_comm_part; bool comm_part_current = false;
    double t_prop = 0, t_energy = 0, t_mix = 0;
    int profiling = 0;
    std::string prof_filter = "nonbonded";
    std::map<const char*, long> prof_seen;
    struct pending_t { std::string name; hipEvent_t a, b; };
    std::vector<pending_t> prof_pending;
    std::map<std::string, remd_profile_entry> prof;

    remd_ctx() = default;
    remd_ctx(const remd_ctx&) = delete;
    remd_ctx& operator=(const remd_ctx&) = delete;
    ~remd_ctx();
};

#define REMD_CHECK(h, expr) do { hipError_t _e = (expr); if (_e != hipSuccess) { \
    (h)->err = std::string(#expr) + ": " + hipGetErrorString(_e); remd_set_global_error((h)->err); return -2; } } while (0)

void remd_set_global_error(const std::string& s);
int remd_fail(remd_ctx* h, int code, const std::string& msg);
void remd_comm_release(remd_ctx* h);

struct remd_prof_scope {
    remd_ctx* h; const char* name; hipEvent_t a = nullptr; bool on = false; hipStream_t st;
    remd_prof_scope(remd_ctx* h_, const char* n, hipStream_t stream = (hipStream_t)-1) : h(h_), name(n) {
        st = (stream == (hipStream_t)-1) ? h->stream : stream;
        on = h->profiling == 2;
        if (h->profiling == 1) {
            const std::string nm(n), &f = h->prof_filter;
            for (size_t b = 0; b <= f.size() && !on; ) {
                size_t e = f.find('|', b); if (e == std::string::npos) e = f.size();
                on = e > b && nm.compare(0, e - b, f, b, e - b) == 0;
                b = e + 1;
            }
            if (on) on = (h->prof_seen[n]++ % h->sw.prof_every) == 0;
        }
        if (on) { hipEventCreate(&a); hipEventRecord(a, st); }
    }
    ~remd_prof_scope() {
        if (on) {
            hipEvent_t b; hipEventCreate(&b); hipEventRecord(b, st);
            h->prof_pending.push_back({name, a, b});
        }
    }
};

int remd_mix_launch(remd_ctx* h, int scheme, int64_t iteration, int R, int K, int ld, const double* d_ukl,
                    int64_t* d_labels, unsigned long long* d_nacc, unsigned long long* d_nprop,
                    const double* d_logw, double* d_logP, int64_t n_attempts);

int remd_parse_splitting(remd_ctx* h, const char* splitting, std::vector<char>& tokens, int& nV, int& nR, int& nO, int* nVg = nullptr);
int remd_run_steps(remd_ctx* h, const std::vector<char>& tokens, int nV, int nR, int nO,
                   int64_t iteration, int64_t first_step, int n_steps);
int remd_run_steps_many(remd_ctx** hs, int n, int64_t iteration, int64_t first_step, int n_steps);
long long remd_chain_blocks(remd_ctx* h);
int remd_assign_velocities(remd_ctx* h, int64_t iteration);
int remd_kinetic_energy(remd_ctx* h);
int remd_work_buffers(remd_ctx* h);

int remd_barostat_attempt(remd_ctx* h);
int remd_barostat_buffers(remd_ctx* h);
int remd_nb_molecules(remd_ctx* h, const int** first, const int** size);
int remd_minimize_impl(remd_ctx* h, double tolerance, int max_iterations, int32_t* converged, int32_t* n_iterations);
void remd_nb_invalidate_sort(remd_ctx* h);
#define REMD_FG_EXTERNAL 0
#define REMD_FG_BOND 1
#define REMD_FG_ANGLE 2
#define REMD_FG_TORSION 3
// ... 28 lines not shown
```

Baseline: 14.59.

## Fold sorted-force scatter and PME unbin into integrator chain kernel

```diff
diff --git a/openmmtools_amd/csrc/forces.hip b/openmmtools_amd/csrc/forces.hip
--- a/openmmtools_amd/csrc/forces.hip
+++ b/openmmtools_amd/csrc/forces.hip
@@ -75,6 +75,7 @@
     int sort_hbits = 0;
     dev_array<float4> d_ctab; bool use_table = false;
     dev_array<unsigned int> d_pair_done; unsigned int pair_done_target = 0;
+    dev_array<int> d_slot_of; dev_array<int> d_lj_slot_of;
     dev_array<int> d_tile_of_rank;
     dev_array<int> d_sort_scratch;
     ~nb_tables() { for (auto& sg : tune_segs) { if (sg.a) hipEventDestroy(sg.a); if (sg.b) hipEventDestroy(sg.b); } }
@@ -93,11 +94,26 @@
     }
     __builtin_amdgcn_fence(__ATOMIC_ACQUIRE, "agent");
 }
+void remd_pme_fold_take(remd_ctx* h, remd_fold_args& fold);
+void remd_pme_unbin_pending(remd_ctx* h, hipStream_t st);
+void remd_pme_reset_fbin(remd_ctx* h);
+__global__ void scatter_sorted_forces_kernel(int Npad_a, const int* __restrict__ order_a, long long* __restrict__ sforce_a,
+                                             int Npad_b, const int* __restrict__ order_b, long long* __restrict__ sforce_b,
+                                             long long* __restrict__ force, int Npad_force);
+static void remd_fold_handover(remd_ctx* h, hipStream_t st)
+{
+    nb_tables* t = h->nb.get();
+    if (t && h->fold.sforce)
+        hipLaunchKernelGGL(scatter_sorted_forces_kernel, dim3((h->Npad + t->NLpad + 255) / 256, h->R), dim3(256), 0, st, h->Npad,
+                           t->d_order, t->d_sforce, t->NLpad, t->d_lj_order, t->d_lj_sforce, h->d_force, h->Npad);
+    remd_pme_unbin_pending(h, st);
+}
 void remd_launch_join_wait(remd_ctx* h)
 {
     if (h->fold_pending) {
         hipEventRecord(h->ev_join, h->stream2);
         hipStreamWaitEvent(h->stream, h->ev_join, 0);
+        remd_fold_handover(h, h->stream);
         h->fold_pending = false;
     }
     if (!h->join_deferred) return;
@@ -343,11 +359,12 @@
 __global__ __launch_bounds__(256)
 void gather_params_kernel(int Npad, int words, const int* __restrict__ order, const float4* __restrict__ param,
                           const unsigned long long* __restrict__ mask, float4* __restrict__ sparam,
-                          unsigned long long* __restrict__ smask)
+                          unsigned long long* __restrict__ smask, int* __restrict__ slot_of)
 {
     const int k = blockIdx.x * blockDim.x + threadIdx.x, r = blockIdx.y;
     if (k >= Npad) return;
     const int o = order[(size_t)r * Npad + k];
+    if (o >= 0) slot_of[(size_t)r * Npad + o] = k;
     sparam[(size_t)r * Npad + k] = (o >= 0) ? param[o] : make_float4(0.f, 0.f, 0.f, 0.f);
     for (int w = 0; w < words; ++w)
         smask[((size_t)r * Npad + k) * words + w] = (o >= 0) ? mask[(size_t)o * words + w] : 0ull;
@@ -356,11 +373,13 @@
 __global__ __launch_bounds__(1024)
 void compact_lj_kernel(int N, int Npad, int NL, int NLpad, int words, const int* __restrict__ order, const int* __restrict__ lj_ord,
                        const float4* __restrict__ param, const unsigned long long* __restrict__ lj_mask,
-                       int* __restrict__ lj_order, float4* __restrict__ lj_sparam, unsigned long long* __restrict__ lj_smask)
+                       int* __restrict__ lj_order, float4* __restrict__ lj_sparam, unsigned long long* __restrict__ lj_smask,
+                       int* __restrict__ lj_slot_of)
 {
     __shared__ int s_part[1024];
     const int r = blockIdx.x, tid = threadIdx.x;
     const int* O = order + (size_t)r * Npad;
+    for (int k = tid; k < Npad; k += 1024) lj_slot_of[(size_t)r * Npad + k] = -1;
     const int per = (N + 1023) / 1024;
     const int b = min(N, tid * per), e = min(N, b + per);
     int cnt = 0;
@@ -379,6 +398,7 @@
         const int ord = lj_ord[a];
         if (ord >= 0) {
             lj_order[(size_t)r * NLpad + slot] = a;
+            lj_slot_of[(size_t)r * Npad + a] = slot;
             lj_sparam[(size_t)r * NLpad + slot] = param[a];
             for (int w = 0; w < words; ++w) lj_smask[((size_t)r * NLpad + slot) * words + w] = lj_mask[(size_t)ord * words + w];
             ++slot;
@@ -488,14 +508,9 @@
 __global__ __launch_bounds__(256)
 void scatter_sorted_forces_kernel(int Npad_a, const int* __restrict__ order_a, long long* __restrict__ sforce_a,
                                   int Npad_b, const int* __restrict__ order_b, long long* __restrict__ sforce_b,
-                                  long long* __restrict__ force, int Npad_force, unsigned int* __restrict__ done = nullptr)
+                                  long long* __restrict__ force, int Npad_force)
 {
     scatter_sorted_forces_body(Npad_a, order_a, sforce_a, Npad_b, order_b, sforce_b, force, Npad_force, blockIdx.x * 256 + threadIdx.x, blockIdx.y);
-    if (done) {
-        asm volatile("s_waitcnt vmcnt(0)" ::: "memory");
-        __syncthreads();
-        if (threadIdx.x == 0) __hip_atomic_fetch_add(done + 16 * blockIdx.y, 1u, __ATOMIC_RELAXED, __HIP_MEMORY_SCOPE_AGENT);
-    }
 }
 
 #define SCI_LANE_II(lane) ((lane) & 7)
@@ -849,11 +864,26 @@
     nonbonded_sci_body<METHOD, ENERGY, ALCH, NW, TAB>(p, a, blockIdx.x, box, rep_lam, epart, n_epart, R, s_ctab - p.ctab_key0);
 }
 
+template <int NW>
+__device__ __forceinline__ int sci_item_replica(const sci_args& a, int item, int R)
+{
+    if (a.tile_of_rank) { const int nzg = a.nsplit / NW; return (item % (R * nzg)) / nzg; }
+    return (item / (a.ncl >> 3)) % R;
+}
+
+__device__ __forceinline__ void sci_item_done(unsigned int* done, int r)
+{
+    asm volatile("s_waitcnt vmcnt(0)" ::: "memory");
+    __syncthreads();
+    if (threadIdx.x == 0) __hip_atomic_fetch_add(done + 16 * r, 1u, __ATOMIC_RELAXED, __HIP_MEMORY_SCOPE_AGENT);
+}
+
 template <int METHOD_A, int METHOD_B, bool ENERGY, bool ALCH, int NW, bool TABLE>
 __global__ __launch_bounds__(64 * NW)
 __attribute__((amdgpu_waves_per_eu((SCI_RELAXED(METHOD_A) || SCI_RELAXED(METHOD_B)) ? 2 : 4, (SCI_RELAXED(METHOD_A) || SCI_RELAXED(METHOD_B)) ? 3 : 4)))
 void nonbonded_sci2_kernel(nb_params p, sci_args a, sci_args b, int n_items_a, int n_items, unsigned int* queue, const float* __restrict__ box,
-                           const float* __restrict__ rep_lam, double* __restrict__ epart, int n_epart, int R, const float4* __restrict__ ctab_g)
+                           const float* __restrict__ rep_lam, double* __restrict__ epart, int n_epart, int R, const float4* __restrict__ ctab_g,
+                           unsigned int* done)
 {
     constexpr bool TAB = TABLE && !ENERGY && SCI_EWALD(METHOD_A);
     if (p.prio) __builtin_amdgcn_s_setprio(3);
@@ -861,8 +891,11 @@
         if ((int)blockIdx.x < n_items_a) {
             if (TAB) stage_coulomb_table(p, ctab_g, 64 * NW);
             nonbonded_sci_body<METHOD_A, ENERGY, ALCH, NW, TAB>(p, a, blockIdx.x, box, rep_lam, epart, n_epart, R, s_ctab - p.ctab_key0);
-        }
-        else nonbonded_sci_body<METHOD_B, ENERGY, ALCH, NW, false, true>(p, b, blockIdx.x - n_items_a, box, rep_lam, epart, n_epart, R);
+            if (done) sci_item_done(done, sci_item_replica<NW>(a, blockIdx.x, R));
+        } else {
+            nonbonded_sci_body<METHOD_B, ENERGY, ALCH, NW, false, true>(p, b, blockIdx.x - n_items_a, box, rep_lam, epart, n_epart, R);
+            if (done) sci_item_done(done, sci_item_replica<NW>(b, blockIdx.x - n_items_a, R));
+        }
         return;
     }
     if (TAB) stage_coulomb_table(p, ctab_g, 64 * NW);
@@ -873,6 +906,7 @@
         const int item = s_item;
         if (item >= n_items_a) break;
         nonbonded_sci_body<METHOD_A, ENERGY, ALCH, NW, TAB>(p, a, item, box, rep_lam, epart, n_epart, R, s_ctab - p.ctab_key0);
+        if (done) sci_item_done(done, sci_item_replica<NW>(a, item, R));
         __syncthreads();
     }
     __syncthreads();
@@ -882,6 +916,7 @@
         const int item = s_item;
         if (item >= n_items - n_items_a) break;
         nonbonded_sci_body<METHOD_B, ENERGY, ALCH, NW, false, true>(p, b, item, box, rep_lam, epart, n_epart, R);
+        if (done) sci_item_done(done, sci_item_replica<NW>(b, item, R));
         __syncthreads();
     }
     if (threadIdx.x == 0 && atomicAdd(&queue[2], 1u) == gridDim.x - 1) { queue[0] = 0u; queue[1] = 0u; queue[2] = 0u; }
@@ -1474,6 +1509,8 @@
         t.d_order.reset(); t.d_spos.reset(); t.d_sparam.reset(); t.d_smask.reset(); t.d_tile_c.reset(); t.d_tile_h.reset();
         const size_t n = (size_t)h->R * h->Npad;
         REMD_TRY(t.d_order.alloc(h, n));
+        t.d_slot_of.reset();
+        REMD_TRY(t.d_slot_of.alloc(h, n));
         REMD_TRY(t.d_spos.alloc(h, n));
         t.d_sposi.reset();
         REMD_TRY(t.d_sposi.alloc(h, n));
@@ -1513,6 +1550,8 @@
             const int ncl_lj = t.NLpad / 8;
             t.lj_cap = std::min(ncl_lj, 4096);
             REMD_TRY(t.d_lj_order.alloc(h, nl));
+            t.d_lj_slot_of.reset();
+            REMD_TRY(t.d_lj_slot_of.alloc(h, n));
             REMD_TRY(t.d_lj_spos.alloc(h, nl));
             t.d_lj_sposi.reset();
             REMD_TRY(t.d_lj_sposi.alloc(h, nl));
@@ -1550,10 +1589,10 @@
                                t.d_grp_size, h->d_pos, h->d_box, t.d_order, t.d_sort_scratch, t.sort_hbits);
         }
         hipLaunchKernelGGL(gather_params_kernel, dim3((h->Npad + 255) / 256, h->R), dim3(256), 0, h->stream, h->Npad, t.p.excl_words,
-                           t.d_order, t.d_param, t.d_mask, t.d_sparam, t.d_smask);
+                           t.d_order, t.d_param, t.d_mask, t.d_sparam, t.d_smask, t.d_slot_of);
         if (split)
             hipLaunchKernelGGL(compact_lj_kernel, dim3(h->R), dim3(1024), 0, h->stream, h->N, h->Npad, t.NL, t.NLpad, t.lj_words, t.d_order,
-                               t.d_lj_ord, t.d_param, t.d_lj_mask, t.d_lj_order, t.d_lj_sparam, t.d_lj_smask);
+                               t.d_lj_ord, t.d_param, t.d_lj_mask, t.d_lj_order, t.d_lj_sparam, t.d_lj_smask, t.d_lj_slot_of);
         if (cl) {
             hipLaunchKernelGGL(build_excl_kernel, dim3(ntile * 8, h->R), dim3(64), 0, h->stream, h->Npad, ntile * 8, t.excl_W, t.p.excl_words,
                                t.d_smask, t.d_excl);
@@ -1620,23 +1659,25 @@
             const int items = items_a + (t.NLpad / 64) * h->R * (ssplit / SCI_NW);
             const int persist_grid = h->sw.nb_persist_grid >= 0 ? h->sw.nb_persist_grid : t.nb_grid;
             const int grid = (h->pme_concurrent && persist_grid > 0) ? std::min(items, persist_grid) : items;
-            const bool fold = h->fold_pending && !ENERGY && t.d_pair_done;
+            const bool fold = h->fold_pending && !ENERGY && t.d_pair_done && t.d_slot_of && t.d_lj_slot_of;
             if (h->fold_pending && !fold) h->fold_pending = false;
             const bool tab = t.use_table && !ENERGY && SCI_EWALD(MAIN);
             const size_t tab_lds = tab ? sizeof(float4) * (size_t)t.p.ctab_n : 0;
 #define LAUNCH_SCI2(ALCHF, TABF) hipLaunchKernelGGL((nonbonded_sci2_kernel<MAIN, NB_LJ_ONLY, ENERGY, ALCHF, SCI_NW, TABF>), dim3(grid), dim3(64 * SCI_NW), \
             tab_lds, h->stream, t.p, sa, sb, items_a, items, grid < items ? t.d_queue : (unsigned int*)nullptr, h->d_box, rl, h->d_epart, h->n_epart, h->R, \
-            (const float4*)t.d_ctab)
+            (const float4*)t.d_ctab, fold ? t.d_pair_done.get() : (unsigned int*)nullptr)
             if (t.has_alch) { if (tab) LAUNCH_SCI2(true, true); else LAUNCH_SCI2(true, false); }
             else { if (tab) LAUNCH_SCI2(false, true); else LAUNCH_SCI2(false, false); }
 #undef LAUNCH_SCI2
-            const dim3 sgrid((h->Npad + t.NLpad + 255) / 256, h->R);
             if (fold) {
-                t.pair_done_target += sgrid.x;
+                t.pair_done_target += (unsigned int)(items / h->R);
                 h->fold.done = t.d_pair_done; h->fold.target = t.pair_done_target;
+                h->fold.slot_of = t.d_slot_of; h->fold.sforce = t.d_sforce;
+                h->fold.lj_slot_of = t.d_lj_slot_of; h->fold.lj_sforce = t.d_lj_sforce; h->fold.NLpad = t.NLpad;
+                return 0;
             }
-            hipLaunchKernelGGL(scatter_sorted_forces_kernel, sgrid, dim3(256), 0, h->stream, h->Npad,
-                               t.d_order, t.d_sforce, t.NLpad, t.d_lj_order, t.d_lj_sforce, h->d_force, h->Npad, fold ? t.d_pair_done : (unsigned int*)nullptr);
+            hipLaunchKernelGGL(scatter_sorted_forces_kernel, dim3((h->Npad + t.NLpad + 255) / 256, h->R), dim3(256), 0, h->stream, h->Npad,
+                               t.d_order, t.d_sforce, t.NLpad, t.d_lj_order, t.d_lj_sforce, h->d_force, h->Npad);
             return 0;
         }
         const bool tab1 = t.use_table && !ENERGY && SCI_EWALD(METHOD);
@@ -1672,7 +1713,8 @@
 void remd_nb_reset_accumulators(remd_ctx* h)
 {
     nb_tables* t = h->nb.get();
-    h->fold_pending = false;
+    h->fold_pending = false; h->mesh_fold = false;
+    remd_pme_reset_fbin(h);
     if (!t || h->R <= 0) return;
     if (t->d_sforce) hipMemsetAsync(t->d_sforce, 0, sizeof(long long) * 3 * (size_t)h->R * h->Npad, h->stream);
     if (t->d_lj_sforce) hipMemsetAsync(t->d_lj_sforce, 0, sizeof(long long) * 3 * (size_t)h->R * t->NLpad, h->stream);
@@ -1789,6 +1831,7 @@
     const bool do_angle = (class_mask >> REMD_FG_ANGLE) & 1u, do_torsion = (class_mask >> REMD_FG_TORSION) & 1u;
     const bool do_nb = (class_mask >> REMD_FG_NONBONDED) & 1u, do_recip = (class_mask >> REMD_FG_RECIPROCAL) & 1u;
     const bool do_rst = h->n_restraints > 0 && ((class_mask >> REMD_FG_RESTRAINT) & 1u);
+    h->mesh_fold = false;
     if (!h->force_zeroed)
         REMD_CHECK(h, hipMemsetAsync(h->d_force, 0, sizeof(long long) * 3 * (size_t)h->Npad * h->R, h->stream));
     h->force_zeroed = false;
@@ -1847,6 +1890,8 @@
                 h->mesh_listed_total = total;
                 listed_rode = total > 0;
             }
+            h->mesh_fold = h->sw.nb_fold && h->sw.listed_main && !with_energy && !h->sync_events && t0.p.prio != 0 && h->defer_join_ok &&
+                           (class_mask & 63u) == 63u && t0.sorting && t0.lj_split && h->profiling != 2;
             rc0 = remd_pme_forces(h, with_energy, h->stream, 1);
             if (rc0) return rc0;
             std::swap(h->stream, h->stream2);
@@ -1894,7 +1939,7 @@
         if (merged && listed_main) launch_listed(h->stream2);
         h->fold_pending = h->sw.nb_fold && listed_main && merged && h->defer_join_ok && do_nb && (class_mask & 63u) == 63u && t.sorting && t.clusters &&
                           t.lj_split && t.d_lj_sci_list && t.d_sci_list && h->profiling != 2;
-        h->fold.done = nullptr;
+        h->fold = remd_fold_args();
         if (do_nb) {
             remd_prof_scope ps(h, "nonbonded");
             if (with_energy) {
@@ -1935,6 +1980,11 @@
                     hipEventRecord(h->ev_join, h->stream);
                     std::swap(h->stream, h->stream2); swapped = false;
                     hipStreamWaitEvent(h->stream, h->ev_join, 0);
+                }
+                if (h->mesh_fold) {
+                    if (h->fold_pending) remd_pme_fold_take(h, h->fold);
+                    else remd_pme_unbin_pending(h, h->stream);
+                    h->mesh_fold = false;
                 }
                 rc = remd_pme_forces(h, with_energy, h->stream, 2); if (rc) return rc;
             }
diff --git a/openmmtools_amd/csrc/integrate.hip b/openmmtools_amd/csrc/integrate.hip
--- a/openmmtools_amd/csrc/integrate.hip
+++ b/openmmtools_amd/csrc/integrate.hip
@@ -349,6 +349,7 @@
                 bins.atoms[e] = make_float4(x[k].x, x[k].y, x[k].z, __int_as_float(idx[k]));
                 if (bins.q) bins.q[e] = bins.param[idx[k]].x;
             } else atomicCAS(bins.err, 0u, 2u);
+            if (bins.pos_of) bins.pos_of[(size_t)r * Npad + idx[k]] = slot < bins.cap ? kx * bins.cap + slot : -1;
         }
 #ifdef CHAIN_STAMPS
         if (S.stamps) { asm volatile("s_waitcnt vmcnt(0) lgkmcnt(0)" ::: "memory"); const unsigned long long now = wall_clock64(); atomicAdd(&S.stamps[1 + 24 + k], now - S.t_last); S.t_last = now; }
@@ -358,6 +359,44 @@
     if (S.stamps) { const unsigned long long now = wall_clock64(); atomicAdd(&S.stamps[35], now - S.t_last); S.t_last = now; }
 #endif
     return mom;
+}
+
+__device__ __attribute__((noinline)) void chain_take_handovers(const remd_fold_args& fold, int Npad, int r, int4 a4, long long* force)
+{
+    const int e_idx[4] = { a4.x, a4.y, a4.z, a4.w };
+    int f_slot[4], f_lj[4], f_bin[4];
+#pragma unroll
+    for (int k = 0; k < 4; ++k) {
+        const int i = e_idx[k] >= 0 ? e_idx[k] : 0;
+        f_slot[k] = fold.slot_of[(size_t)r * Npad + i];
+        f_lj[k] = fold.lj_slot_of[(size_t)r * Npad + i];
+        f_bin[k] = fold.bin_pos ? fold.bin_pos[(size_t)r * Npad + i] : -1;
+    }
+    unsigned long long* Fu = reinterpret_cast<unsigned long long*>(force + (size_t)r * 3 * Npad);
+    unsigned long long* Sm = reinterpret_cast<unsigned long long*>(fold.sforce + (size_t)r * 3 * Npad);
+    unsigned long long* Sl = reinterpret_cast<unsigned long long*>(fold.lj_sforce + (size_t)r * 3 * fold.NLpad);
+    unsigned long long* Fb = fold.fbin ? fold.fbin + (size_t)r * 3 * fold.fbin_P : nullptr;
+#pragma unroll
+    for (int k = 0; k < 4; ++k) {
+        if (e_idx[k] < 0) continue;
+        const int i = e_idx[k];
+        unsigned long long t[3], a[3], b[3], c[3];
+#pragma unroll
+        for (int d = 0; d < 3; ++d) {
+            t[d] = Fu[(size_t)d * Npad + i];
+            a[d] = f_slot[k] >= 0 ? Sm[(size_t)d * Npad + f_slot[k]] : 0ull;
+            b[d] = f_lj[k] >= 0 ? Sl[(size_t)d * fold.NLpad + f_lj[k]] : 0ull;
+            c[d] = f_bin[k] >= 0 ? Fb[(size_t)d * fold.fbin_P + f_bin[k]] : 0ull;
+        }
+#pragma unroll
+        for (int d = 0; d < 3; ++d) {
+            t[d] += a[d] + b[d] + c[d];
+            if (f_slot[k] >= 0) Sm[(size_t)d * Npad + f_slot[k]] = 0ull;
+            if (f_lj[k] >= 0) Sl[(size_t)d * fold.NLpad + f_lj[k]] = 0ull;
+            if (f_bin[k] >= 0) Fb[(size_t)d * fold.fbin_P + f_bin[k]] = 0ull;
+            Fu[(size_t)d * Npad + i] = t[d];
+        }
+    }
 }
 
 __device__ __forceinline__ void integrate_chain_body(chain_prog prog, int n_units, const int4* __restrict__ unit_atoms,
@@ -425,6 +464,7 @@
         __builtin_amdgcn_fence(__ATOMIC_ACQUIRE, "agent");
     }
     const unsigned long long own_t0 = own_time ? wall_clock64() : 0ull;
+    if (fold.done) chain_take_handovers(fold, Npad, r, a4, force);
     float3 mom = f3(0, 0, 0);
     const int cmm_r_eff = prog.cmm_r, cmm_w_eff = prog.cmm_w;
     if (uidx == 0 && cmm_r_eff >= 0) {
@@ -546,6 +586,7 @@
                         bins.atoms[e] = make_float4(S.x[k].x, S.x[k].y, S.x[k].z, __int_as_float(idx[k]));
                         if (bins.q) bins.q[e] = bins.param[idx[k]].x;
                     } else atomicCAS(bins.err, 0u, 2u);
+                    if (bins.pos_of) bins.pos_of[(size_t)r * Npad + idx[k]] = slot < bins.cap ? col[k] * bins.cap + slot : -1;
                 }
             }
         }
@@ -791,6 +832,7 @@
 }
 
 remd_chain_bins remd_pme_chain_bins(remd_ctx* h);
+void remd_pme_fold_done(remd_ctx* h);
 static void launch_chain(remd_ctx* h, const unit_tables& ut, const chain_prog& prog, bool bin_for_pme = false)
 {
     const bool chain_bins = h->sw.pme_chainbin >= 0 ? h->sw.pme_chainbin != 0
@@ -805,6 +847,7 @@
                        h->join_deferred ? h->d_sync + 1 : (unsigned int*)nullptr, h->join_deferred, bins, h->d_chain_sync, h->d_sync + 2,
                        (h->profiling == 2 || (h->profiling == 1 && h->prof_filter.find("integrate_chain") != std::string::npos)) ? h->d_chain_own : (unsigned long long*)nullptr,
                        h->d_work, h->d_xold, h->d_vold, h->fold_pending ? h->fold : remd_fold_args(), h->d_noise_id);
+    if (h->fold_pending && h->fold.fbin) remd_pme_fold_done(h);
     h->join_deferred = 0; h->fold_pending = false;
     if (bins.count) h->cbins_ready = true;
 }
diff --git a/openmmtools_amd/csrc/pme.hip b/openmmtools_amd/csrc/pme.hip
--- a/openmmtools_amd/csrc/pme.hip
+++ b/openmmtools_amd/csrc/pme.hip
@@ -41,6 +41,8 @@
     int sch_nl = 0, sch_zt = 0;
     dev_array<float> d_cbin_q;
     dev_array<unsigned long long> d_fbin; size_t fbin_P = 0;
+    dev_array<int> d_bin_pos;
+    bool unbin_pending = false; const int* unbin_cs = nullptr; const int* unbin_ca = nullptr; int unbin_cap = 0;
     dev_array<int> d_cbin_count; dev_array<float4> d_cbin_atoms; int cbin_cap = 0, cbin_parity = 0; bool cbin_use = false;
 };
 
@@ -286,7 +288,7 @@
 __global__ __launch_bounds__(1024)
 void pme_bin_kernel(int N, int Npad, int nx, int ny, int nz, const float4* __restrict__ pos, const float* __restrict__ box,
                     int* __restrict__ bin_start , int* __restrict__ bin_atoms ,
-                    unsigned int* fork_flag, unsigned int fork_seq)
+                    unsigned int* fork_flag, unsigned int fork_seq, int* __restrict__ bin_pos )
 {
     if (fork_flag && blockIdx.x == 0 && threadIdx.x == 0) __hip_atomic_store(fork_flag, fork_seq, __ATOMIC_RELEASE, __HIP_MEMORY_SCOPE_AGENT);
     __builtin_amdgcn_s_setprio(PME_PRIO);
@@ -313,6 +315,7 @@
         if (kx >= nx) kx -= nx;
         const int slot = atomicAdd(&s_cur[kx], 1);
         bin_atoms[(size_t)r * Npad + slot] = i;
+        bin_pos[(size_t)r * Npad + i] = slot;
     }
     for (int k = tid; k <= nx; k += 1024) bin_start[(size_t)r * (nx + 1) + k] = s_start[k];
 }
@@ -1094,6 +1097,7 @@
         REMD_TRY(s->d_grid.alloc(h, s->nspec * s->R));
         REMD_TRY(s->d_col_start.alloc(h, (size_t)(s->n[0] + 1) * s->R));
         REMD_TRY(s->d_col_atoms.alloc(h, (size_t)h->Npad * s->R));
+        REMD_TRY(s->d_bin_pos.alloc(h, (size_t)h->Npad * s->R));
         if (!full_complex && h->sw.pme_chainbin != 0) {
             s->cbin_cap = std::min(h->Npad, std::max(64, 4 * ((h->N + s->n[0] - 1) / s->n[0])));
             if (h->sw.pme_cbin_cap) s->cbin_cap = h->sw.pme_cbin_cap;
@@ -1229,7 +1233,7 @@
     {
         remd_prof_scope ps(h, "pme_bin", st);
         hipLaunchKernelGGL(pme_bin_kernel, dim3(h->R), dim3(1024), 0, st, h->N, h->Npad, nx, ny, nz, h->d_pos, h->d_box,
-                           s->d_col_start, s->d_col_atoms, h->fork_seq_pending ? h->d_sync : (unsigned int*)nullptr, h->fork_seq_pending);
+                           s->d_col_start, s->d_col_atoms, h->fork_seq_pending ? h->d_sync : (unsigned int*)nullptr, h->fork_seq_pending, s->d_bin_pos);
         h->fork_seq_pending = 0;
     }
     {
@@ -1339,7 +1343,10 @@
         } else
         DISPATCH_Z(pme_zinv_gather_kernel, s->d_grid, s->d_tw[2], s->d_tw[3], h->Npad, h->d_pos, param, h->d_box, rep_lam,
                    bin_cs, bin_ca, h->d_force, bin_cap, (s->cbin_use && !rep_lam) ? s->d_cbin_q : (const float*)nullptr, fbin, s->fbin_P);
-        if (fbin) {
+        s->unbin_pending = false;
+        if (fbin && h->mesh_fold) {
+            s->unbin_pending = true; s->unbin_cs = bin_cs; s->unbin_ca = bin_ca; s->unbin_cap = bin_cap;
+        } else if (fbin) {
             const int npos = bin_cap > 0 ? nx * bin_cap : h->N;
             hipLaunchKernelGGL(pme_unbin_forces_kernel, dim3((npos + 255) / 256, s->R), dim3(256), 0, st, nx, bin_cap, h->N, h->Npad, s->fbin_P,
                                bin_cs, bin_ca, fbin, h->d_force);
@@ -1358,13 +1365,42 @@
     return 0;
 }
 
+void remd_pme_fold_take(remd_ctx* h, remd_fold_args& fold)
+{
+    pme_state* s = h->pme.get();
+    fold.fbin = nullptr; fold.fbin_P = 0; fold.bin_pos = nullptr;
+    if (!s || !s->unbin_pending) return;
+    fold.fbin = s->d_fbin; fold.fbin_P = (long long)s->fbin_P; fold.bin_pos = s->d_bin_pos;
+}
+void remd_pme_fold_done(remd_ctx* h)
+{
+    pme_state* s = h->pme.get();
+    if (s) s->unbin_pending = false;
+}
+void remd_pme_unbin_pending(remd_ctx* h, hipStream_t st)
+{
+    pme_state* s = h->pme.get();
+    if (!s || !s->unbin_pending) return;
+    const int npos = s->unbin_cap > 0 ? s->n[0] * s->unbin_cap : h->N;
+    hipLaunchKernelGGL(pme_unbin_forces_kernel, dim3((npos + 255) / 256, s->R), dim3(256), 0, st, s->n[0], s->unbin_cap, h->N, h->Npad, s->fbin_P,
+                       s->unbin_cs, s->unbin_ca, s->d_fbin, h->d_force);
+    s->unbin_pending = false;
+}
+void remd_pme_reset_fbin(remd_ctx* h)
+{
+    pme_state* s = h->pme.get();
+    if (!s) return;
+    s->unbin_pending = false;
+    if (s->d_fbin) hipMemsetAsync(s->d_fbin, 0, sizeof(unsigned long long) * 3 * s->fbin_P * s->R, h->stream);
+}
+
 remd_chain_bins remd_pme_chain_bins(remd_ctx* h)
 {
     remd_chain_bins b;
     const pme_state* s = h->pme.get();
     if (!s || !s->d_cbin_count || s->R != h->R || !h->pme_concurrent || h->no_chain_bins) return b;
     b.nx = s->n[0]; b.cap = s->cbin_cap; b.count = s->d_cbin_count + (size_t)s->cbin_parity * s->R * s->n[0]; b.atoms = s->d_cbin_atoms;
-    b.box = h->d_box; b.err = h->d_sync + 2;
+    b.box = h->d_box; b.err = h->d_sync + 2; b.pos_of = s->d_bin_pos;
     b.param = remd_nb_param(h);
     b.q = (b.param && !remd_nb_rep_lam(h)) ? s->d_cbin_q : nullptr;
     return b;
diff --git a/openmmtools_amd/csrc/remd_internal.h b/openmmtools_amd/csrc/remd_internal.h
--- a/openmmtools_amd/csrc/remd_internal.h
+++ b/openmmtools_amd/csrc/remd_internal.h
@@ -74,7 +74,9 @@
     k = (int)u;
 }
 struct remd_chain_bins { int nx = 0, cap = 0; int* count = nullptr; float4* atoms = nullptr; const float* box = nullptr; unsigned int* err = nullptr;
-                         float* q = nullptr; const float4* param = nullptr; const float* rep_lam = nullptr; };
+                         float* q = nullptr; const float4* param = nullptr; const float* rep_lam = nullptr;
+                         int* pos_of = nullptr;
+};
 
 __device__ __forceinline__ unsigned long long remd_f2fix(float f)
 {
@@ -88,6 +90,10 @@
 
 struct remd_fold_args {
     const unsigned int* done = nullptr; unsigned int target = 0;
+    const int* slot_of = nullptr; long long* sforce = nullptr;
+    const int* lj_slot_of = nullptr; long long* lj_sforce = nullptr;
+    int NLpad = 0;
+    const int* bin_pos = nullptr; unsigned long long* fbin = nullptr; long long fbin_P = 0;
 };
 
 struct listed_tables {
@@ -269,6 +275,7 @@
     bool defer_join_ok = false; unsigned int join_deferred = 0;
     listed_tables mesh_listed{}; int mesh_listed_total = 0;
     remd_fold_args fold; bool fold_pending = false;
+    bool mesh_fold = false;
     bool mesh_prio_hi = true;
     bool no_device_waits = false, no_chain_bins = false, no_resident = false, no_chain_merge = false;
     bool lean_waits = false, no_chain_barrier = false;
```

After: 14.91, median of 6. 1.02x the previous value.
